# douban/dpark

Hardware: NVIDIA H100
Metric: shuffled rows/sec (reduceByKey end-to-end) (higher is better)
Workload: dtype int64

## Files before the change

### dpark_b200/_native.py

```python
import ctypes as C
import os

import torch

_HERE = os.path.dirname(os.path.abspath(__file__))
LIB_PATH = os.path.join(_HERE, "libdpark_b200.so")

OK, ERR_INVALID, ERR_UNSUPPORTED, ERR_WORKSPACE, ERR_CUDA = 0, -1, -2, -3, -4
K_HASHED = -1
K_I64, K_I32, K_F64, K_U64, K_F32, K_ROWID = 0, 1, 2, 3, 4, 5
V_I64, V_F64, V_I32, V_F32 = 0, 1, 2, 3
OPS = {"sum": 0, "min": 1, "max": 2, "prod": 3, "and": 4, "or": 5, "xor": 6}
BYTES_SIGNED, STR_UTF8 = 0, 1
MAX_PARTITIONS = 4096

_KEY_KIND = {torch.int64: K_I64, torch.int32: K_I32, torch.float64: K_F64, torch.float32: K_F32}
if hasattr(torch, "uint64"):
    _KEY_KIND[torch.uint64] = K_U64
_VAL_KIND = {torch.int64: V_I64, torch.float64: V_F64, torch.int32: V_I32, torch.float32: V_F32}

EXPORTS = [
    "dpk_abi_version", "dpk_last_error", "dpk_device_info", "dpk_hash_keys", "dpk_hash_bytes",
    "dpk_partition_ids", "dpk_partition_workspace_bytes", "dpk_partition_count",
    "dpk_partition_scatter", "dpk_partition", "dpk_combine_workspace_bytes", "dpk_combine",
# ... 99 lines not shown
def _stream():
    return C.c_void_p(torch.cuda.current_stream().cuda_stream)


def _need_cuda(*ts):
    for t in ts:
        if t is not None and not t.is_cuda:
            raise NativeError("dpark_b200 shuffle kernels need CUDA tensors (no CPU fallback); got %s" % t.device)
        if t is not None and not t.is_contiguous():
            raise ValueError("columns must be contiguous")


def key_kind(t, prehashed=False):
    if prehashed:
        if t.dtype != torch.int64:
            raise TypeError("prehashed keys must be int64")
        return K_HASHED
    try:
        return _KEY_KIND[t.dtype]
    except KeyError:
        raise TypeError("%s is unhashable by portable_hash" % t.dtype)


def val_kind(t):
    try:
        return _VAL_KIND[t.dtype]
    except KeyError:
        raise TypeError("unsupported value dtype %s" % t.dtype)


def _thr(thresholds, device):
    if thresholds is None:
        return None, 0
    if not torch.is_tensor(thresholds):
        thresholds = torch.tensor(list(thresholds), dtype=torch.int64, device=device)
    thresholds = thresholds.to(device=device, dtype=torch.int64).contiguous()
    return thresholds, int(thresholds.numel())


def device_info():
    import numpy as np
    info = np.zeros(4, dtype=np.int32)
    _check(lib().dpk_device_info(info.ctypes.data_as(C.c_void_p)))
    return {"sm_count": int(info[0]), "cc": (int(info[1]), int(info[2])), "l2_mb": int(info[3])}


def hash_keys(keys):
    _need_cuda(keys)
    out = torch.empty(keys.numel(), dtype=torch.int64, device=keys.device)
    _check(lib().dpk_hash_keys(_ptr(keys), key_kind(keys), keys.numel(), _ptr(out), _stream()))
    return out


def hash_bytes(data, offsets, mode):
    _need_cuda(data, offsets)
    n = offsets.numel() - 1
    out = torch.empty(n, dtype=torch.int64, device=offsets.device)
    _check(lib().dpk_hash_bytes(_ptr(data), _ptr(offsets), n, mode, _ptr(out), _stream()))
    return out


def hash_tuple(item_hashes):
    _need_cuda(item_hashes)
    arity, n = int(item_hashes.shape[0]), int(item_hashes.shape[1])
    out = torch.empty(n, dtype=torch.int64, device=item_hashes.device)
    _check(lib().dpk_hash_tuple(_ptr(item_hashes), n, arity, _ptr(out), _stream()))
    return out


def partition_ids(hashes, P, thresholds=None):
    _need_cuda(hashes)
    thr, nthr = _thr(thresholds, hashes.device)
    out = torch.empty(hashes.numel(), dtype=torch.int32, device=hashes.device)
    _check(lib().dpk_partition_ids(_ptr(hashes), hashes.numel(), P, _ptr(thr), nthr, _ptr(out), _stream()))
    return out


def partition_workspace(nbuckets, device):
    nbytes = lib().dpk_partition_workspace_bytes(0, nbuckets)
    return torch.empty(nbytes, dtype=torch.uint8, device=device)


K_UNORDERED = 0x100


def _kk(keys, prehashed, row_hash, unordered=False):
    kk = K_ROWID if row_hash is not None else key_kind(keys, prehashed)
    return kk | K_UNORDERED if (unordered and kk >= 0) else kk


def partition_count(keys, P, thresholds=None, prehashed=False, sub_bits=0, ws=None, row_hash=None, unordered=False):
    _need_cuda(keys, row_hash)
    F = P << sub_bits
    thr, nthr = _thr(thresholds, keys.device)
    if ws is None:
        ws = partition_workspace(F, keys.device)
    counts = torch.empty(F, dtype=torch.int64, device=keys.device)
    _check(lib().dpk_partition_count(_ptr(keys), _kk(keys, prehashed, row_hash, unordered), _ptr(row_hash), keys.numel(), P,
                                     _ptr(thr), nthr,
                                     sub_bits, _ptr(counts), _ptr(ws), ws.numel(), _stream()))
    return counts, ws


def partition_scatter(keys, vals, P, bucket_base, out_keys, out_vals, ws, thresholds=None, prehashed=False,
                      sub_bits=0, row_hash=None, unordered=False):
    _need_cuda(keys, vals, bucket_base, out_keys, out_vals, ws, row_hash)
    thr, nthr = _thr(thresholds, keys.device)
    vb = 0 if vals is None else vals.element_size()
    _check(lib().dpk_partition_scatter(_ptr(keys), _kk(keys, prehashed, row_hash, unordered), _ptr(row_hash), _ptr(vals), vb,
                                       keys.numel(), P,
                                       _ptr(thr), nthr, sub_bits, _ptr(bucket_base), _ptr(out_keys),
                                       _ptr(out_vals), _ptr(ws), ws.numel(), _stream()))


def partition_scatter_ptrs(keys, vals, P, key_ptrs, val_ptrs, ws, thresholds=None, prehashed=False, sub_bits=0,
                           row_hash=None, unordered=False):
    _need_cuda(keys, vals, key_ptrs, val_ptrs, ws, row_hash)
    thr, nthr = _thr(thresholds, keys.device)
    vb = 0 if vals is None else vals.element_size()
    _check(lib().dpk_partition_scatter_ptrs(_ptr(keys), _kk(keys, prehashed, row_hash, unordered), _ptr(row_hash), _ptr(vals),
                                            vb, keys.numel(), P, _ptr(thr), nthr, sub_bits, _ptr(key_ptrs),
                                            _ptr(val_ptrs), _ptr(ws), ws.numel(), _stream()))


def copy_segments(src_ptrs, dst_ptrs, nbytes, sms=0):
    _need_cuda(src_ptrs, dst_ptrs, nbytes)
    if not (src_ptrs.numel() == dst_ptrs.numel() == nbytes.numel()):
        raise ValueError("segment table columns differ in length")
    if sms:
        set_option("copy_sms", int(sms))
    try:
        _check(lib().dpk_copy_segments(_ptr(src_ptrs), _ptr(dst_ptrs), _ptr(nbytes), nbytes.numel(), _stream()))
    finally:
        if sms:
            set_option("copy_sms", 0)


def memcpy_batch(dst_ptrs, src_ptrs, nbytes):
    n = len(nbytes)
    if not (len(dst_ptrs) == len(src_ptrs) == n):
        raise ValueError("segment table columns differ in length")
    if n == 0:
        return
    U, I = C.c_uint64 * n, C.c_int64 * n
    _check(lib().dpk_memcpy_batch(U(*dst_ptrs), U(*src_ptrs), I(*nbytes), n, _stream()))


def push_plan(all_counts, nranks, per_block, my_src, my_rank, keys, vals, dst_base, capacity, need_over, want_seg=True,
              part=None, dst_row0=0):
    _need_cuda(all_counts, dst_base, need_over)
    nsrc, F = int(all_counts.shape[0]), int(all_counts.shape[1])
    ncols = 1 if vals is None else 2
    dev = all_counts.device
    lo, hi = (0, per_block) if part is None else part
    src = torch.empty(ncols * nranks, dtype=torch.int64, device=dev)
    dst = torch.empty(ncols * nranks, dtype=torch.int64, device=dev)
    nby = torch.empty(ncols * nranks, dtype=torch.int64, device=dev)
    b0, b1 = min(F, my_rank * per_block + lo), min(F, (my_rank + 1) * per_block, my_rank * per_block + hi)
    seg = torch.empty((nsrc, max(0, b1 - b0)), dtype=torch.int64, device=dev) if want_seg else None
    _check(lib().dpk_push_plan_part(_ptr(all_counts), nsrc, nranks, F, per_block, lo, hi, dst_row0, my_src, my_rank, ncols,
                                    C.c_uint64(keys.data_ptr()), C.c_uint64(0 if vals is None else vals.data_ptr()),
                                    _ptr(dst_base), keys.element_size(), 0 if vals is None else vals.element_size(),
                                    capacity, _ptr(src), _ptr(dst), _ptr(nby), _ptr(need_over), _ptr(seg), _stream()))
    return src, dst, nby, seg


def pipe_plan(all_counts, nranks, per_block, nparts, region_rows, my_src, my_rank, keys, vals, dst_base, need_over,
              want_seg=True):
    _need_cuda(all_counts, dst_base, need_over, keys, vals)
    nsrc, F = int(all_counts.shape[0]), int(all_counts.shape[1])
    ncols = 1 if vals is None else 2
    dev = all_counts.device
    base = torch.empty(F, dtype=torch.int64, device=dev)
    src = torch.empty((nparts, ncols * nranks), dtype=torch.int64, device=dev)
    dst = torch.empty((nparts, ncols * nranks), dtype=torch.int64, device=dev)
    nby = torch.empty((nparts, ncols * nranks), dtype=torch.int64, device=dev)
    seg = torch.empty((nparts, nsrc, per_block // nparts), dtype=torch.int64, device=dev) if want_seg else None
    _check(lib().dpk_pipe_plan(_ptr(all_counts), nsrc, nranks, F, per_block, nparts, region_rows, my_src, my_rank, ncols,
                               C.c_uint64(keys.data_ptr()), C.c_uint64(0 if vals is None else vals.data_ptr()),
                               _ptr(dst_base), keys.element_size(), 0 if vals is None else vals.element_size(),
                               _ptr(base), _ptr(src), _ptr(dst), _ptr(nby), _ptr(need_over), _ptr(seg), _stream()))
    return base, src, dst, nby, seg


def pipe_pad_rows(nranks, nparts, key_bytes, val_bytes=None):
    return nranks * nparts * (16 // min(key_bytes, val_bytes or key_bytes))


def fused_plan(all_counts, nranks, per_block, my_rank, dst_base, key_bytes, val_bytes, capacity, dump_keys, dump_vals,
               need_over, want_seg=True):
    _need_cuda(all_counts, dst_base, need_over, dump_keys, dump_vals)
    G, F = int(all_counts.shape[0]), int(all_counts.shape[1])
    if G != nranks:
        raise ValueError("all_counts has %d source rows for %d ranks" % (G, nranks))
    ncols = 1 if dump_vals is None else 2
    dev = all_counts.device
    kp = torch.empty(F, dtype=torch.int64, device=dev)
    vp_ = torch.empty(F, dtype=torch.int64, device=dev) if ncols == 2 else None
    b0, b1 = min(F, my_rank * per_block), min(F, (my_rank + 1) * per_block)
    seg = torch.empty((G, b1 - b0), dtype=torch.int64, device=dev) if want_seg else None
    _check(lib().dpk_fused_plan(_ptr(all_counts), nranks, F, per_block, my_rank, ncols, _ptr(dst_base), key_bytes,
                                val_bytes if ncols == 2 else 0, capacity, C.c_uint64(dump_keys.data_ptr()),
                                C.c_uint64(0 if dump_vals is None else dump_vals.data_ptr()), _ptr(kp), _ptr(vp_),
                                _ptr(need_over), _ptr(seg), _stream()))
    return kp, vp_, seg


def partition(keys, vals, P, thresholds=None, prehashed=False, sub_bits=0, row_hash=None, unordered=False):
    _need_cuda(keys, vals, row_hash)
    if vals is not None and vals.numel() != keys.numel():
        from .errors import DparkUserFatalError
        raise DparkUserFatalError("ragged pair columns: %d keys, %d values" % (keys.numel(), vals.numel()))
    F = P << sub_bits
    thr, nthr = _thr(thresholds, keys.device)
    ws = partition_workspace(F, keys.device)
    out_keys = torch.empty_like(keys)
    out_vals = None if vals is None else torch.empty_like(vals)
    offsets = torch.empty(F + 1, dtype=torch.int64, device=keys.device)
    vb = 0 if vals is None else vals.element_size()
    _check(lib().dpk_partition(_ptr(keys), _kk(keys, prehashed, row_hash, unordered), _ptr(row_hash), _ptr(vals), vb,
                               keys.numel(), P,
                               _ptr(thr), nthr, sub_bits, _ptr(out_keys), _ptr(out_vals), _ptr(offsets),
                               _ptr(ws), ws.numel(), _stream()))
    return out_keys, out_vals, offsets


def acc_dtype(vals_dtype):
    return torch.float64 if vals_dtype in (torch.float32, torch.float64) else torch.int64


def combine(keys, vals, op, P, seg_rows, part_first=0, nparts=None, thresholds=None, sub_bits=0,
            row_hash=None):
    _need_cuda(keys, vals, seg_rows, row_hash)
    if nparts is None:
        nparts = P
    n = keys.numel()
    F = nparts << sub_bits
    if seg_rows.dim() == 1:
        seg_rows = seg_rows.unsqueeze(0)
    nsrc = int(seg_rows.shape[0])
    if seg_rows.shape[1] != F or seg_rows.dtype != torch.int64:
        raise ValueError("seg_rows must be int64[nsrc, %d]" % F)
    bucket_rows = seg_rows
    thr, nthr = _thr(thresholds, keys.device)
    ws_bytes = lib().dpk_combine_workspace_bytes(n, F, nsrc)
    ws = torch.empty(ws_bytes, dtype=torch.uint8, device=keys.device)
    out_keys = torch.empty_like(keys)
    out_vals = torch.empty(n, dtype=acc_dtype(vals.dtype), device=keys.device)
    out_offsets = torch.empty(nparts + 1, dtype=torch.int64, device=keys.device)
    out_counts = torch.empty(nparts, dtype=torch.int64, device=keys.device)
    kk = key_kind(keys) if row_hash is None else K_ROWID
    _check(lib().dpk_combine(_ptr(keys), kk, _ptr(row_hash), _ptr(vals), val_kind(vals), n, OPS[op], P,
                             _ptr(thr), nthr, sub_bits, part_first, nparts, nsrc, _ptr(bucket_rows), _ptr(out_keys),
                             _ptr(out_vals), _ptr(out_offsets), _ptr(out_counts), _ptr(ws), ws_bytes,
                             _stream()))
    return out_keys, out_vals, out_offsets, out_counts


def dict_encode(data, offsets, hashes):
    _need_cuda(data, offsets, hashes)
    n = offsets.numel() - 1
    ws_bytes = lib().dpk_dict_encode_workspace_bytes(n)
    ws = torch.empty(ws_bytes, dtype=torch.uint8, device=offsets.device)
    rep = torch.empty(n, dtype=torch.int64, device=offsets.device)
    _check(lib().dpk_dict_encode(_ptr(data), _ptr(offsets), _ptr(hashes), n, _ptr(rep), _ptr(ws), ws_bytes,
                                 _stream()))
    return rep


def tokenize(data):
    _need_cuda(data)
    n = int(data.numel())
    dev = data.device
    if n == 0:
        z = torch.zeros(0, dtype=torch.int64, device=dev)
        return z, z.clone(), True
    nb = int(lib().dpk_tokenize_blocks(n))
    counts = torch.empty(nb + 1, dtype=torch.int64, device=dev)
    counts[nb] = 0
    _check(lib().dpk_tokenize_count(_ptr(data), n, _ptr(counts), C.c_void_p(counts.data_ptr() + 8 * nb), _stream()))
    incl = torch.cumsum(counts[:nb], 0)
    total, flag = int(incl[-1].item()), int(counts[nb].item())
    if flag & 1:
        return None, None, False
    base = (incl - counts[:nb]).contiguous()
    starts = torch.empty(total, dtype=torch.int64, device=dev)
    lens = torch.empty(total, dtype=torch.int64, device=dev)
    if total:
        _check(lib().dpk_tokenize_emit(_ptr(data), n, _ptr(base), _ptr(starts), _ptr(lens), _stream()))
    return starts, lens, True


def gather_bytes(data, starts, lens, idx=None):
    _need_cuda(data, starts, lens, idx)
    sel = lens if idx is None else lens[idx]
    m = int(sel.numel())
    off = torch.zeros(m + 1, dtype=torch.int64, device=data.device)
    if m:
        torch.cumsum(sel, 0, out=off[1:])
    out = torch.empty(int(off[-1].item()) if m else 0, dtype=torch.uint8, device=data.device)
    if m and out.numel():
        _check(lib().dpk_gather_bytes(_ptr(data), _ptr(starts), _ptr(lens), _ptr(idx), m, _ptr(off), _ptr(out), _stream()))
    return out, off


def key_or(keys):
    _need_cuda(keys)
    out = torch.empty(1, dtype=torch.int64, device=keys.device)
    _check(lib().dpk_key_or(_ptr(keys), keys.numel(), _ptr(out), _stream()))
    return out


def gather_i64(src, idx):
    _need_cuda(src, idx)
    out = torch.empty(idx.numel(), dtype=torch.int64, device=idx.device)
    _check(lib().dpk_gather_i64(_ptr(src), _ptr(idx), idx.numel(), _ptr(out), _stream()))
    return out


def radix_pass(keys, vals, shift, bits, out_keys=None, out_vals=None, ws=None):
    _need_cuda(keys, vals)
    if keys.dtype != torch.int64:
        raise TypeError("radix_pass sorts int64 key bits")
    if out_keys is None:
        out_keys = torch.empty_like(keys)
    if out_vals is None and vals is not None:
        out_vals = torch.empty_like(vals)
    if ws is None:
        ws = partition_workspace(1 << bits, keys.device)
    vb = 0 if vals is None else vals.element_size()
    _check(lib().dpk_radix_pass(_ptr(keys), _ptr(vals), vb, keys.numel(), shift, bits, _ptr(out_keys),
                                _ptr(out_vals), _ptr(ws), ws.numel(), _stream()))
    return out_keys, out_vals


# ... 96 lines not shown
```

### dpark_b200/csrc/dpk_aggregate2.cuh

```cuda
#pragma once

constexpr int AG2_THREADS = 256;
constexpr int AG2_WARPS = AG2_THREADS / 32;
constexpr int AG2_TAGS = 4096;
constexpr int AG2_CAP = 2048;
constexpr int AG2_ITEMS = AG2_CAP / AG2_THREADS;
constexpr int AG2_GEN_ITEMS = 4;
constexpr uint32_t AG2_IDX_MASK = 0xfffu;
constexpr int AG2_MINW = 256;
constexpr int AG2_MAX_M = 1 << 16;
constexpr int AG2_STACK = 40;

struct Ag2Shared {
    int fb, sp, overflow, nres;
    unsigned long long excl;
    int next_fb[2];
    long long next_r0[2], next_r1[2];
    int wcnt[AG2_ITEMS * AG2_WARPS];
    int total;
    int stack_m[AG2_STACK], stack_r[AG2_STACK];
};

__device__ __forceinline__ uint32_t sm_ld_u32(uint32_t a) {
    uint32_t v;
// ... 74 lines not shown
    unsigned mine = 0;
    const int lane = threadIdx.x & 31;
    const unsigned lt = (1u << lane) - 1u;
    offs[0] = offs[1] = 0;
    int lc = 0;
#pragma unroll
    for (int g = 0; g < NI; g += 4) {
        long long k[4];
        uint32_t h[4], t[4];
        bool claimed[4];
#pragma unroll
        for (int u = 0; u < 4; u++) {
            const int idx = (g + u) * AG2_THREADS + (int)threadIdx.x;
            k[u] = idx < n ? sm_ld_s64(key_base + (uint32_t)idx * 8u) : 0ll;
        }
        uint32_t fpb[4];
#pragma unroll
        for (int u = 0; u < 4; u++) {
            const uint32_t hs = slot_hash32((uint64_t)k[u]);
            h[u] = hs & (AG2_TAGS - 1);
            fpb[u] = hs & ~(uint32_t)AG2_IDX_MASK;
        }
#pragma unroll
        for (int u = 0; u < 4; u++) {
            const int idx = (g + u) * AG2_THREADS + (int)threadIdx.x;
            t[u] = idx < n ? sm_ld_u32(tag_base + h[u] * 4u) : 0xffffffffu;
        }
#pragma unroll
        for (int u = 0; u < 4; u++) {
            const int idx = (g + u) * AG2_THREADS + (int)threadIdx.x;
            claimed[u] = false;
            if (t[u] == 0u) {
                t[u] = sm_cas_u32(tag_base + h[u] * 4u, 0u, fpb[u] | ((uint32_t)idx + 1u));
                claimed[u] = t[u] == 0u;
            }
        }
#pragma unroll
        for (int u = 0; u < 4; u++) {
            const int idx = (g + u) * AG2_THREADS + (int)threadIdx.x;
            if (idx < n && !claimed[u]) {
                uint32_t hh = h[u], tt = t[u];
                for (;;) {
                    if (tt == 0u) {
                        tt = sm_cas_u32(tag_base + hh * 4u, 0u, fpb[u] | ((uint32_t)idx + 1u));
                        if (tt == 0u) { claimed[u] = true; break; }
                    }
                    if ((tt & ~(uint32_t)AG2_IDX_MASK) == fpb[u]) {
                        const uint32_t o = (tt & AG2_IDX_MASK) - 1u;
                        if (sm_ld_s64(key_base + o * 8u) == k[u]) {
                            const long long mv = sm_ld_s64(acc_base + (uint32_t)idx * 8u);
                            if constexpr (std::is_same<AccT, double>::value)
                                sm_apply<double>(op, acc_base + o * 8u, s_acc + o, __longlong_as_double(mv));
                            else
                                sm_apply<int64_t>(op, acc_base + o * 8u, s_acc + o, (int64_t)mv);
                            break;
                        }
                    }
                    hh = (hh + 1u) & (AG2_TAGS - 1);
                    tt = sm_ld_u32(tag_base + hh * 4u);
                }
            }
        }
#pragma unroll
        for (int u = 0; u < 4; u++) {
            const int j = g + u;
            const unsigned cmj = __ballot_sync(0xffffffffu, claimed[u]);
            if (lane == j) lc = __popc(cmj);
            offs[j >> 2] |= (uint32_t)__popc(cmj & lt) << (8 * (j & 3));
            if (claimed[u]) mine |= 1u << j;
        }
    }
    *lane_cnt = lc;
    return mine;
}

__device__ __forceinline__ int ag2_off(const uint32_t (&offs)[2], int j) { return (int)((offs[j >> 2] >> (8 * (j & 3))) & 0xffu); }
__device__ __forceinline__ uint32_t ag2_slot(const uint32_t (&slots)[3], int j) {
    const int bit = 12 * j;
    uint32_t v = slots[bit >> 5] >> (bit & 31);
    if ((bit & 31) > 20) v |= slots[(bit >> 5) + 1] << (32 - (bit & 31));
    return v & 0xfffu;
}

template <typename KeyT, typename ValT, typename AccT, int MINB, bool CURSOR, bool BATCHED, bool FAST_ONLY = false>
__global__ void __launch_bounds__(AG2_THREADS, MINB)
k_smem_aggregate2(const KeyT *__restrict__ keys, const ValT *__restrict__ vals, int op,
                  const int64_t *__restrict__ fine_off, int32_t nfine, int32_t fine_per_part,
                  const int64_t *__restrict__ part_offsets, KeyT *__restrict__ out_keys,
                  int64_t *__restrict__ out_vals, long long *__restrict__ out_counts,
                  unsigned long long *__restrict__ fb_state, int *__restrict__ work_counter,
                  int *__restrict__ part_err, const int *__restrict__ bucket_list, const int *__restrict__ bucket_count,
                  long long *__restrict__ phase_cycles, int *__restrict__ big_list = nullptr, int *__restrict__ big_count = nullptr) {
    long long tstamp = 0;
    auto stamp = [&](int k) {
        if (phase_cycles != nullptr && threadIdx.x == 0) {
            const long long now = clock64();
            if (k >= 0) atomicAdd(reinterpret_cast<unsigned long long *>(&phase_cycles[k]), (unsigned long long)(now - tstamp));
            tstamp = now;
        }
    };
    const int nwork = bucket_list ? *bucket_count : nfine;
    auto bucket_of_ticket = [&](int t) { return bucket_list ? bucket_list[t] : t; };
    extern __shared__ __align__(16) long long s_dyn2[];
    uint32_t *s_tag = reinterpret_cast<uint32_t *>(s_dyn2);
    long long *s_key = s_dyn2 + AG2_TAGS / 2;
    long long *s_acc = s_key + AG2_CAP;
    const uint32_t tag_base = (uint32_t)__cvta_generic_to_shared(s_tag);
    const uint32_t key_base = (uint32_t)__cvta_generic_to_shared(s_key);
    const uint32_t acc_base = (uint32_t)__cvta_generic_to_shared(s_acc);
    __shared__ Ag2Shared sh;
    const int lane = threadIdx.x & 31, warp = threadIdx.x >> 5;
    auto clear_tags = [&]() {
        uint4 *t4 = reinterpret_cast<uint4 *>(s_tag);
#pragma unroll
        for (int i = 0; i < AG2_TAGS / 4 / AG2_THREADS; i++) t4[i * AG2_THREADS + threadIdx.x] = make_uint4(0, 0, 0, 0);
    };
    auto stage = [&](int64_t g0, int w, int at, auto ni_tag, auto between) {
        constexpr int NI = decltype(ni_tag)::value;
        KeyT kr[NI];
        ValT vr[NI];
#pragma unroll
        for (int j = 0; j < NI; j++) {
            const int i = j * AG2_THREADS + (int)threadIdx.x;
            if (i < w) { kr[j] = keys[g0 + i]; vr[j] = vals[g0 + i]; }
        }
        between();
#pragma unroll
        for (int j = 0; j < NI; j++) {
            const int i = j * AG2_THREADS + (int)threadIdx.x;
            if (i < w) {
                s_key[at + i] = key_bits<KeyT>(kr[j]);
                if constexpr (std::is_same<AccT, double>::value) s_acc[at + i] = __double_as_longlong((double)vr[j]);
                else s_acc[at + i] = (long long)vr[j];
            }
        }
    };
    auto nothing = []() {};
    auto scan_claims = [&]() {
        constexpr int N = AG2_ITEMS * AG2_WARPS;
        int a = sh.wcnt[lane], b = sh.wcnt[lane + 32];
        int ia = a, ib = b;
#pragma unroll
        for (int d = 1; d < 32; d <<= 1) {
            int ta = __shfl_up_sync(0xffffffffu, ia, d), tb = __shfl_up_sync(0xffffffffu, ib, d);
            if (lane >= d) { ia += ta; ib += tb; }
        }
        const int suma = __shfl_sync(0xffffffffu, ia, 31);
        sh.wcnt[lane] = ia - a;
        sh.wcnt[lane + 32] = suma + ib - b;
        if (lane == 31) sh.total = suma + ib;
        static_assert(N == 64, "scan_claims handles 64 counters");
    };

    clear_tags();
    if (threadIdx.x == 0) {
        const int t = atomicAdd(work_counter, 1);
        sh.next_fb[0] = t < nwork ? bucket_of_ticket(t) : nfine;
        if (t < nwork) { const int b = bucket_of_ticket(t); sh.next_r0[0] = fine_off[b]; sh.next_r1[0] = fine_off[b + 1]; }
    }
    for (int it = 0;; it++) {
        __syncthreads();
        stamp(it ? 4 : -1);
        const int fb = sh.next_fb[it & 1];
        if (fb >= nfine) break;
        const int64_t r0 = sh.next_r0[it & 1], r1 = sh.next_r1[it & 1];
        const int p = fb / fine_per_part;
        const int first_fb = p * fine_per_part;
        const bool last_fb = fb == first_fb + fine_per_part - 1;
        const int64_t pbase = part_offsets[p];
        uint32_t offs[2], slots[3];
        int lane_cnt;
        int nt = 0;
        long long nr0 = 0, nr1 = 0;
        auto prefetch_ticket = [&]() {
            if (CURSOR && threadIdx.x == 0) nt = atomicAdd(work_counter, 1);
        };
        auto prefetch_range = [&]() {
            if (CURSOR && threadIdx.x == 0) {
                const int b = nt < nwork ? bucket_of_ticket(nt) : nfine;
                sh.next_fb[(it + 1) & 1] = b;
                if (b < nfine) { nr0 = fine_off[b]; nr1 = fine_off[b + 1]; }
            }
        };
        auto publish_range = [&]() {
            if (threadIdx.x == 0) {
                if (!CURSOR) {
                    nt = atomicAdd(work_counter, 1);
                    sh.next_fb[(it + 1) & 1] = nt;
                    if (nt < nfine) { nr0 = fine_off[nt]; nr1 = fine_off[nt + 1]; }
                }
                sh.next_r0[(it + 1) & 1] = nr0;
                sh.next_r1[(it + 1) & 1] = nr1;
            }
        };

        if (r1 - r0 <= AG2_CAP) {
            const int n = (int)(r1 - r0);
            stage(r0, n, 0, std::integral_constant<int, AG2_ITEMS>(), prefetch_ticket);
            prefetch_range();
            __syncthreads();
            stamp(0);
            const unsigned mine = BATCHED ? ag2_insert_batched<AccT, AG2_ITEMS>(n, op, tag_base, key_base, acc_base, s_acc, offs, &lane_cnt)
                                          : ag2_insert<AccT, false, AG2_ITEMS>(0, n, 1, 0, op, tag_base, key_base, acc_base, s_acc, offs, &lane_cnt, slots);
            if (lane < AG2_ITEMS) sh.wcnt[lane * AG2_WARPS + warp] = lane_cnt;
            if (CURSOR) publish_range();
            __syncthreads();
            stamp(1);
// ... 148 lines not shown
```

### dpark_b200/csrc/dpk_combine.cu

```cuda
#include "dpk_common.cuh"
#include <cooperative_groups.h>
#include <type_traits>

namespace cg = cooperative_groups;

namespace dpk {

constexpr int CB_THREADS = 256;
constexpr int64_t kEmpty = INT64_MIN;

struct __align__(16) Slot {
    int64_t key;
    int64_t acc;
};

template <typename KeyT> __device__ __forceinline__ int64_t key_bits(KeyT k);
template <> __device__ __forceinline__ int64_t key_bits<int64_t>(int64_t k) { return k; }
template <> __device__ __forceinline__ int64_t key_bits<int32_t>(int32_t k) { return (int64_t)k; }
template <> __device__ __forceinline__ int64_t key_bits<uint64_t>(uint64_t k) { return (int64_t)k; }
template <> __device__ __forceinline__ int64_t key_bits<double>(double k) {
    if (k == 0.0) k = 0.0;
    return __double_as_longlong(k);
}
template <> __device__ __forceinline__ int64_t key_bits<float>(float k) {
// ... 79 lines not shown

__global__ void __launch_bounds__(CB_THREADS)
k_tbl_plan(const int64_t *__restrict__ seg_rows, int32_t nsrc, int32_t F, int32_t sub_bits, int32_t nparts,
           int64_t *__restrict__ tbl_off, int64_t *__restrict__ part_off, int64_t *__restrict__ seg_start) {
    __shared__ long long s_slots[CB_THREADS], s_rows[CB_THREADS], s_carry;
    const int E = (F + CB_THREADS - 1) / CB_THREADS;
    const int b0 = threadIdx.x * E, b1 = min(b0 + E, F);
    long long slots = 0, rows = 0;
    for (int b = b0; b < b1; b++) {
        long long r = 0;
        for (int s = 0; s < nsrc; s++) r += seg_rows[(int64_t)s * F + b];
        slots += ((r + (r >> 1) + 32 + 7) >> 3) << 3;
        rows += r;
    }
    s_slots[threadIdx.x] = slots;
    s_rows[threadIdx.x] = rows;
    __syncthreads();
    long long sbase = 0, rbase = 0;
    for (int t = 0; t < (int)threadIdx.x; t++) { sbase += s_slots[t]; rbase += s_rows[t]; }
    const int S = 1 << sub_bits;
    for (int b = b0; b < b1; b++) {
        long long r = 0;
        for (int s = 0; s < nsrc; s++) r += seg_rows[(int64_t)s * F + b];
        tbl_off[b] = sbase;
        if ((b & (S - 1)) == 0) part_off[b >> sub_bits] = rbase;
        sbase += ((r + (r >> 1) + 32 + 7) >> 3) << 3;
        rbase += r;
    }
    if (b0 < F && b1 == F) { tbl_off[F] = sbase; part_off[nparts] = rbase; }
    if (F == 0 && threadIdx.x == 0) { tbl_off[0] = 0; part_off[0] = 0; }
    if (threadIdx.x == 0) s_carry = 0;
    __syncthreads();
    for (int s = 0; s < nsrc; s++) {
        long long mine = 0;
        for (int b = b0; b < b1; b++) mine += seg_rows[(int64_t)s * F + b];
        s_rows[threadIdx.x] = mine;
        __syncthreads();
        long long base = s_carry;
        for (int t = 0; t < (int)threadIdx.x; t++) base += s_rows[t];
        for (int b = b0; b < b1; b++) {
            seg_start[(int64_t)s * F + b] = base;
            base += seg_rows[(int64_t)s * F + b];
        }
        __syncthreads();
        if (threadIdx.x == CB_THREADS - 1) s_carry = base;
        __syncthreads();
    }
}

__device__ __forceinline__ int4 slot_fill(int64_t ident) {
    return make_int4((int)(uint32_t)((uint64_t)kEmpty & 0xffffffffu), (int)(uint32_t)((uint64_t)kEmpty >> 32),
                     (int)(uint32_t)((uint64_t)ident & 0xffffffffu), (int)(uint32_t)((uint64_t)ident >> 32));
}

__device__ __forceinline__ Slot *probe_slot(Slot *region, uint32_t size, int64_t kb) {
    uint32_t h = (uint32_t)(((mix64((uint64_t)kb) & 0xffffffffull) * (uint64_t)size) >> 32);
    for (;;) {
        int64_t cur = __ldcg(&region[h].key);
        if (cur == kb) break;
        if (cur == kEmpty) {
            unsigned long long prev = atomicCAS((unsigned long long *)&region[h].key, (unsigned long long)kEmpty,
                                                (unsigned long long)kb);
            if (prev == (unsigned long long)kEmpty || prev == (unsigned long long)kb) break;
        }
        h = h + 1 == size ? 0 : h + 1;
    }
    return &region[h];
}

__global__ void __launch_bounds__(CB_THREADS)
k_tbl_init(Slot *__restrict__ table, const int64_t *__restrict__ tbl_total, int64_t ident) {
    const int64_t slots = *tbl_total;
    int64_t i = (int64_t)blockIdx.x * blockDim.x + threadIdx.x;
    int64_t stride = (int64_t)gridDim.x * blockDim.x;
    const int4 fill = slot_fill(ident);
    for (; i < slots; i += stride) reinterpret_cast<int4 *>(table)[i] = fill;
}

template <typename KeyT, typename ValT, typename AccT>
__global__ void __launch_bounds__(CB_THREADS)
k_tbl_insert(const KeyT *__restrict__ keys, const int64_t *__restrict__ aux, const ValT *__restrict__ vals,
             int64_t n, const int64_t *__restrict__ rows_total, int op, PartFn f, int32_t bucket_first, int32_t F,
             const int64_t *__restrict__ tbl_off, Slot *__restrict__ table, Slot *__restrict__ side,
             int32_t *__restrict__ side_used) {
    int64_t i = (int64_t)blockIdx.x * blockDim.x + threadIdx.x;
    int64_t stride = (int64_t)gridDim.x * blockDim.x;
    const int64_t rows = min(n, *rows_total);
    for (; i < rows; i += stride) {
        const KeyT key = keys[i];
        const int64_t kb = key_bits<KeyT>(key);
        const AccT v = (AccT)vals[i];
        Slot *s;
        if (kb == kEmpty) {
            s = side;
            *side_used = 1;
        } else {
            int b = f.bucket(hash_of<KeyT>(key, aux)) - bucket_first;
            b = min(max(b, 0), F - 1);
            const int64_t base = __ldg(&tbl_off[b]);
            s = probe_slot(table + base, (uint32_t)(__ldg(&tbl_off[b + 1]) - base), kb);
        }
        Acc<AccT>::apply(op, &s->acc, v);
    }
}

template <typename KeyT>
__global__ void __launch_bounds__(CB_THREADS)
k_tbl_compact(const Slot *__restrict__ table, const int64_t *__restrict__ tbl_total,
              const int64_t *__restrict__ aux, PartFn f, int32_t part_first, int32_t nparts,
              const int64_t *__restrict__ part_offsets, KeyT *__restrict__ out_keys,
              int64_t *__restrict__ out_vals, unsigned long long *__restrict__ out_counts) {
    extern __shared__ __align__(16) int32_t s_mem[];
    int32_t *s_cnt = s_mem;
    long long *s_base = reinterpret_cast<long long *>(s_mem + ((nparts + 1) & ~1));
    const int lane = threadIdx.x & 31;
    constexpr int ITEMS = 4;
    const int64_t total = *tbl_total;
    const int64_t tile = (int64_t)CB_THREADS * ITEMS;
    for (int64_t t0 = (int64_t)blockIdx.x * tile; t0 < total; t0 += (int64_t)gridDim.x * tile) {
        for (int p = threadIdx.x; p < nparts; p += CB_THREADS) s_cnt[p] = 0;
        __syncthreads();
        int64_t kb[ITEMS], acc[ITEMS];
        int lp[ITEMS], rk[ITEMS];
#pragma unroll
        for (int j = 0; j < ITEMS; j++) {
            int64_t i = t0 + (int64_t)j * CB_THREADS + threadIdx.x;
            lp[j] = -1;
            if (i < total) {
                int4 raw = __ldcs(reinterpret_cast<const int4 *>(table) + i);
                kb[j] = (int64_t)(((uint64_t)(uint32_t)raw.y << 32) | (uint32_t)raw.x);
                acc[j] = (int64_t)(((uint64_t)(uint32_t)raw.w << 32) | (uint32_t)raw.z);
                if (kb[j] != kEmpty) lp[j] = f(hash_of<KeyT>(key_from_bits<KeyT>(kb[j]), aux)) - part_first;
            }
        }
#pragma unroll
        for (int j = 0; j < ITEMS; j++) {
            unsigned m = __match_any_sync(0xffffffffu, lp[j]);
            int base = 0;
            const bool ok = lp[j] >= 0 && lp[j] < nparts;
            if (ok && lane == __ffs(m) - 1) base = atomicAdd(&s_cnt[lp[j]], __popc(m));
            base = __shfl_sync(0xffffffffu, base, __ffs(m) - 1);
            rk[j] = base + __popc(m & ((1u << lane) - 1u));
        }
        __syncthreads();
        for (int p = threadIdx.x; p < nparts; p += CB_THREADS) {
            int c = s_cnt[p];
            s_base[p] = c ? (long long)atomicAdd(&out_counts[p], (unsigned long long)c) : 0;
        }
        __syncthreads();
#pragma unroll
        for (int j = 0; j < ITEMS; j++) {
            if (lp[j] >= 0 && lp[j] < nparts) {
                int64_t dst = part_offsets[lp[j]] + s_base[lp[j]] + rk[j];
                out_keys[dst] = key_from_bits<KeyT>(kb[j]);
                out_vals[dst] = acc[j];
            }
        }
        __syncthreads();
    }
}

constexpr int BR_THREADS = 1024;
constexpr int BR_CLUSTER = 8;

template <typename KeyT, typename ValT, typename AccT>
__global__ void __cluster_dims__(BR_CLUSTER, 1, 1) __launch_bounds__(BR_THREADS, 1)
k_bucket_reduce(const KeyT *__restrict__ keys, const int64_t *__restrict__ aux, const ValT *__restrict__ vals,
                int op, int64_t ident, int32_t sub_bits, int32_t F, int32_t nsrc,
                const int64_t *__restrict__ seg_start, const int64_t *__restrict__ seg_rows,
                const int64_t *__restrict__ tbl_off, Slot *__restrict__ table, Slot *__restrict__ side,
                int32_t *__restrict__ side_used, const int64_t *__restrict__ part_offsets,
                KeyT *__restrict__ out_keys, int64_t *__restrict__ out_vals,
                unsigned long long *__restrict__ out_counts, int *__restrict__ bucket_counter) {
    cg::cluster_group cluster = cg::this_cluster();
    const unsigned crank = cluster.block_rank();
    __shared__ int s_bucket;
    __shared__ int s_wsum[BR_THREADS / 32];
    __shared__ long long s_base;
    const int lane = threadIdx.x & 31, warp = threadIdx.x >> 5;
    const int64_t tid_c = (int64_t)crank * BR_THREADS + threadIdx.x;
    const int64_t nth_c = (int64_t)BR_CLUSTER * BR_THREADS;
    const int4 fill = slot_fill(ident);
    for (;;) {
        if (crank == 0 && threadIdx.x == 0) s_bucket = atomicAdd(bucket_counter, 1);
        cluster.sync();
        const int b = *cluster.map_shared_rank(&s_bucket, 0);
        cluster.sync();
        if (b >= F) break;
        const int64_t base = tbl_off[b];
        const uint32_t size = (uint32_t)(tbl_off[b + 1] - base);
        Slot *region = table + base;
        for (int64_t i = tid_c; i < size; i += nth_c) reinterpret_cast<int4 *>(region)[i] = fill;
        cluster.sync();
        for (int s = 0; s < nsrc; s++) {
            const int64_t r0 = seg_start[(int64_t)s * F + b];
            const int64_t rn = seg_rows[(int64_t)s * F + b];
            for (int64_t i = tid_c; i < rn; i += nth_c) {
                const int64_t kb = key_bits<KeyT>(keys[r0 + i]);
                const AccT v = (AccT)vals[r0 + i];
                Slot *sl;
                if (kb == kEmpty) {
                    sl = side;
                    *side_used = 1;
                } else {
                    sl = probe_slot(region, size, kb);
                }
                Acc<AccT>::apply(op, &sl->acc, v);
            }
        }
        cluster.sync();
        const int p = b >> sub_bits;
        const int64_t pbase = part_offsets[p];
        constexpr int ITEMS = 4;
        const int64_t tile = (int64_t)BR_THREADS * ITEMS;
        for (int64_t t0 = (int64_t)crank * tile; t0 < size; t0 += (int64_t)BR_CLUSTER * tile) {
            int64_t kb[ITEMS], acc[ITEMS];
            int c = 0;
#pragma unroll
            for (int j = 0; j < ITEMS; j++) {
                const int64_t i = t0 + (int64_t)threadIdx.x * ITEMS + j;
                kb[j] = kEmpty;
                if (i < size) {
                    int4 raw = __ldcg(reinterpret_cast<const int4 *>(region) + i);
                    kb[j] = (int64_t)(((uint64_t)(uint32_t)raw.y << 32) | (uint32_t)raw.x);
                    acc[j] = (int64_t)(((uint64_t)(uint32_t)raw.w << 32) | (uint32_t)raw.z);
                }
                c += kb[j] != kEmpty;
            }
            int inc = c;
#pragma unroll
            for (int d = 1; d < 32; d <<= 1) {
                int t = __shfl_up_sync(0xffffffffu, inc, d);
                if (lane >= d) inc += t;
            }
            if (lane == 31) s_wsum[warp] = inc;
            __syncthreads();
            if (warp == 0) {
                int w = s_wsum[lane];
                int winc = w;
#pragma unroll
                for (int d = 1; d < 32; d <<= 1) {
                    int t = __shfl_up_sync(0xffffffffu, winc, d);
                    if (lane >= d) winc += t;
                }
                s_wsum[lane] = winc - w;
                if (lane == 31) s_base = winc ? (long long)atomicAdd(&out_counts[p], (unsigned long long)winc) : 0;
            }
            __syncthreads();
            int64_t dst = pbase + s_base + s_wsum[warp] + (inc - c);
#pragma unroll
            for (int j = 0; j < ITEMS; j++) {
                if (kb[j] != kEmpty) {
                    out_keys[dst] = key_from_bits<KeyT>(kb[j]);
                    out_vals[dst] = acc[j];
                    dst++;
                }
            }
            __syncthreads();
        }
    }
}

#include "dpk_aggregate.cuh"
#include "dpk_aggregate2.cuh"
#include "dpk_aggregate3.cuh"

template <typename KeyT>
__global__ void k_side_flush(const Slot *__restrict__ side, const int32_t *__restrict__ side_used,
                             const int64_t *__restrict__ aux, PartFn f, int32_t part_first, int32_t nparts,
                             const int64_t *__restrict__ part_offsets, KeyT *__restrict__ out_keys,
                             int64_t *__restrict__ out_vals, unsigned long long *__restrict__ out_counts) {
    if (threadIdx.x != 0 || blockIdx.x != 0 || *side_used == 0) return;
    const KeyT key = key_from_bits<KeyT>(kEmpty);
    const int p = f(hash_of<KeyT>(key, aux)) - part_first;
    if (p < 0 || p >= nparts) return;
    const int64_t dst = part_offsets[p] + (int64_t)atomicAdd(&out_counts[p], 1ull);
    out_keys[dst] = key;
    out_vals[dst] = side->acc;
}

static inline int64_t max_slots_for(int64_t n, int32_t F) { return n + (n >> 1) + (int64_t)F * 40 + 64; }

static inline int grid_cap(int64_t items, int per_cta, int waves) {
    int64_t g = (items + per_cta - 1) / per_cta;
    int64_t cap = (int64_t)sm_count() * waves;
    if (g > cap) g = cap;
    if (g < 1) g = 1;
    return (int)g;
}

int g_reduce_impl = 2;

int g_agg_wide = 1;
int g_agg_ctas = 4;
int g_agg_timing = 0;
int g_agg_split = 1;
int g_agg_cursor = 1;
int g_agg_pipe = 0;
int g_agg_batched = 0;
int g_agg_impl = 1;
int g_agg_target_rows = 2048;

struct Ctx {
    int key_kind, val_bytes;
    int64_t *fine_off;
    unsigned long long *fb_state;
    int *part_err;
    void *seg_ws;
    int64_t seg_ws_bytes;
    const void *keys, *vals;
    const int64_t *aux;
    int64_t n;
    int op;
    PartFn f;
    int32_t part_first, nparts, F, nsrc;
    const int64_t *seg_rows, *seg_start, *tbl_off, *part_off;
    Slot *table, *side;
    int64_t max_slots;
    int32_t *side_used;
    int *bucket_counter;
    void *out_keys;
    int64_t *out_vals;
    unsigned long long *out_counts;
    cudaStream_t st;
};

template <typename KeyT, typename ValT, typename AccT>
static int dispatch_op(const Ctx &c) {
    if (!Acc<AccT>::supports(c.op)) return fail(DPK_ERR_UNSUPPORTED, "op %d unsupported for this value kind", c.op);
    const int64_t ident = Acc<AccT>::identity(c.op);
    if (g_reduce_impl == 2) {
        const int sb2 = choose_sb2(c.n, c.F, g_agg_target_rows);
        const int32_t S2 = 1 << sb2;
        PartFn fine = fine_partfn(c.f, sb2);
        fine.row_hash = c.aux;
        KeyT *rekeys = (KeyT *)c.table;
        ValT *revals = (ValT *)((char *)c.table + (size_t)c.n * 8);
        int rc = seg_multisplit(c.keys, c.key_kind, c.vals, (int32_t)sizeof(ValT), c.n, fine, c.F, c.nsrc, c.seg_start,
                                c.seg_rows, rekeys, revals, c.fine_off, c.seg_ws, c.seg_ws_bytes, c.st);
        if (rc) return rc;
        const int32_t nfine = c.F * S2;
        int grid = sm_count() * 8;
        if (grid > nfine) grid = nfine;
        auto agg = g_agg_wide ? k_smem_aggregate<KeyT, ValT, AccT, true> : k_smem_aggregate<KeyT, ValT, AccT, false>;
        const int agg_smem = AG_CAP * 16 + AG_CAP * 2;
        DPK_CUDA_TRY(cudaFuncSetAttribute(agg, cudaFuncAttributeMaxDynamicSharedMemorySize, agg_smem));
        DPK_CUDA_TRY(cudaMemsetAsync(c.fb_state, 0, (size_t)nfine * 8, c.st));
        if (g_agg_impl == 1) {
            auto agg2 = k_smem_aggregate2<KeyT, ValT, AccT, 3, true, true>;
            if (g_agg_cursor && g_agg_batched) agg2 = g_agg_ctas == 4 ? k_smem_aggregate2<KeyT, ValT, AccT, 4, true, true> : k_smem_aggregate2<KeyT, ValT, AccT, 3, true, true>;
            else if (g_agg_cursor) agg2 = g_agg_ctas == 4 ? k_smem_aggregate2<KeyT, ValT, AccT, 4, true, false> : k_smem_aggregate2<KeyT, ValT, AccT, 3, true, false>;
            else agg2 = k_smem_aggregate2<KeyT, ValT, AccT, 3, false, false>;
            const int smem2 = AG2_TAGS * 4 + AG2_CAP * 16;
            DPK_CUDA_TRY(cudaFuncSetAttribute(agg2, cudaFuncAttributeMaxDynamicSharedMemorySize, smem2));
            DPK_CUDA_TRY(cudaMemsetAsync(c.part_err, 0, (size_t)(c.nparts + 2) * 4, c.st));
            long long *timing = nullptr;
            if (g_agg_timing) {
                static long long *d_timing = nullptr;
                if (!d_timing) DPK_CUDA_TRY(cudaMalloc(&d_timing, 64));
                DPK_CUDA_TRY(cudaMemsetAsync(d_timing, 0, 64, c.st));
                timing = d_timing;
            }
            if (g_agg_pipe && g_agg_cursor) {
                auto agg3 = g_agg_pipe == 2 ? k_smem_aggregate3<KeyT, ValT, AccT, 2, false>
                          : (g_agg_batched ? k_smem_aggregate3<KeyT, ValT, AccT, 3, true> : k_smem_aggregate3<KeyT, ValT, AccT, 3, false>);
                const int smem3 = AG2_TAGS * 4 + AG2_CAP * 8;
                DPK_CUDA_TRY(cudaFuncSetAttribute(agg3, cudaFuncAttributeMaxDynamicSharedMemorySize, smem3));
                int *big_count = c.part_err + c.nparts, *list_counter = c.part_err + c.nparts + 1;
                int *big_list = reinterpret_cast<int *>(c.fb_state);
                int g3 = sm_count() * (g_agg_pipe == 2 ? 2 : 3);
                if (g3 > nfine) g3 = nfine;
                DPK_LAUNCH("smem_aggregate", c.st, agg3<<<g3, AG2_THREADS, smem3, c.st>>>(
                    rekeys, revals, c.op, ident, c.fine_off, nfine, (1 << c.f.sub_bits) * S2, c.part_off,
                    (KeyT *)c.out_keys, c.out_vals, (long long *)c.out_counts, c.bucket_counter, big_list, big_count));
                auto aggb = k_smem_aggregate2<KeyT, ValT, AccT, 3, true, false>;
                DPK_CUDA_TRY(cudaFuncSetAttribute(aggb, cudaFuncAttributeMaxDynamicSharedMemorySize, smem2));
                DPK_LAUNCH("smem_aggregate_big", c.st, aggb<<<sm_count(), AG2_THREADS, smem2, c.st>>>(
                    rekeys, revals, c.op, c.fine_off, nfine, (1 << c.f.sub_bits) * S2, c.part_off,
                    (KeyT *)c.out_keys, c.out_vals, (long long *)c.out_counts, c.fb_state, list_counter, c.part_err,
                    big_list, big_count, nullptr, nullptr, nullptr));
            } else if (g_agg_cursor && !g_agg_batched && g_agg_split) {
                auto fast = g_agg_ctas == 4 ? k_smem_aggregate2<KeyT, ValT, AccT, 4, true, false, true>
                                            : k_smem_aggregate2<KeyT, ValT, AccT, 3, true, false, true>;
                DPK_CUDA_TRY(cudaFuncSetAttribute(fast, cudaFuncAttributeMaxDynamicSharedMemorySize, smem2));
                int *big_count = c.part_err + c.nparts, *list_counter = c.part_err + c.nparts + 1;
                int *big_list = reinterpret_cast<int *>(c.fb_state);
                DPK_LAUNCH("smem_aggregate", c.st, fast<<<grid, AG2_THREADS, smem2, c.st>>>(
                    rekeys, revals, c.op, c.fine_off, nfine, (1 << c.f.sub_bits) * S2, c.part_off,
                    (KeyT *)c.out_keys, c.out_vals, (long long *)c.out_counts, c.fb_state, c.bucket_counter, c.part_err,
                    nullptr, nullptr, timing, big_list, big_count));
                auto aggb = k_smem_aggregate2<KeyT, ValT, AccT, 3, true, false>;
                DPK_CUDA_TRY(cudaFuncSetAttribute(aggb, cudaFuncAttributeMaxDynamicSharedMemorySize, smem2));
                DPK_LAUNCH("smem_aggregate_big", c.st, aggb<<<sm_count() * 2, AG2_THREADS, smem2, c.st>>>(
                    rekeys, revals, c.op, c.fine_off, nfine, (1 << c.f.sub_bits) * S2, c.part_off,
                    (KeyT *)c.out_keys, c.out_vals, (long long *)c.out_counts, c.fb_state, list_counter, c.part_err,
                    big_list, big_count, nullptr, nullptr, nullptr));
            } else {
            DPK_LAUNCH("smem_aggregate", c.st, agg2<<<grid, AG2_THREADS, smem2, c.st>>>(
                rekeys, revals, c.op, c.fine_off, nfine, (1 << c.f.sub_bits) * S2, c.part_off,
                (KeyT *)c.out_keys, c.out_vals, (long long *)c.out_counts, c.fb_state, c.bucket_counter, c.part_err,
                nullptr, nullptr, timing, nullptr, nullptr));
            if (timing) {
                long long h[8];
                DPK_CUDA_TRY(cudaMemcpyAsync(h, timing, sizeof(h), cudaMemcpyDeviceToHost, c.st));
                DPK_CUDA_TRY(cudaStreamSynchronize(c.st));
                const double nb = h[5] ? (double)h[5] : 1.0;
                fprintf(stderr, "agg_timing: %lld buckets; cycles per bucket: load+stage %.0f | insert %.0f | reserve %.0f | write-out %.0f | "
                        "to next top %.0f | total %.0f\n", h[5], h[0] / nb, h[1] / nb, h[2] / nb, h[3] / nb, h[4] / nb,
                        (h[0] + h[1] + h[2] + h[3] + h[4]) / nb);
            }
            }
            if (g_agg_cursor)
                DPK_LAUNCH("agg_finalize", c.st, k_agg_finalize<<<1, 256, 0, c.st>>>(c.part_err, (long long *)c.out_counts, c.nparts));
            return DPK_OK;
        }
        DPK_LAUNCH("smem_aggregate", c.st, agg<<<grid, AG_THREADS, agg_smem, c.st>>>(
            rekeys, revals, c.op, ident, c.fine_off, nfine, (1 << c.f.sub_bits) * S2, c.part_off,
            (KeyT *)c.out_keys, c.out_vals, c.out_counts, c.fb_state, c.bucket_counter));
        return DPK_OK;
    }
    if (g_reduce_impl == 1) {
        auto kern = k_bucket_reduce<KeyT, ValT, AccT>;
        int nclusters = sm_count() / BR_CLUSTER;
        if (nclusters > c.F) nclusters = c.F;
        if (nclusters < 1) nclusters = 1;
        DPK_LAUNCH("bucket_reduce", c.st, kern<<<nclusters * BR_CLUSTER, BR_THREADS, 0, c.st>>>(
            (const KeyT *)c.keys, c.aux, (const ValT *)c.vals, c.op, ident, c.f.sub_bits, c.F, c.nsrc,
            c.seg_start, c.seg_rows, c.tbl_off, c.table, c.side, c.side_used, c.part_off, (KeyT *)c.out_keys,
            c.out_vals, c.out_counts, c.bucket_counter));
    } else {
        DPK_LAUNCH("tbl_init", c.st, k_tbl_init<<<grid_cap(c.max_slots, CB_THREADS, 16), CB_THREADS, 0, c.st>>>(
            c.table, c.tbl_off + c.F, ident));
        if (c.n > 0) {
            DPK_LAUNCH("tbl_insert", c.st, k_tbl_insert<KeyT, ValT, AccT><<<grid_cap(c.n, CB_THREADS, 16), CB_THREADS, 0, c.st>>>(
                (const KeyT *)c.keys, c.aux, (const ValT *)c.vals, c.n, c.part_off + c.nparts, c.op, c.f,
                c.part_first << c.f.sub_bits,
                c.F, c.tbl_off, c.table, c.side, c.side_used));
        }
        size_t sh = (size_t)((c.nparts + 1) & ~1) * 4 + (size_t)c.nparts * 8;
        DPK_LAUNCH("tbl_compact", c.st, k_tbl_compact<KeyT><<<grid_cap(c.max_slots, CB_THREADS * 4, 8), CB_THREADS, sh, c.st>>>(
            c.table, c.tbl_off + c.F, c.aux, c.f, c.part_first, c.nparts, c.part_off, (KeyT *)c.out_keys,
            c.out_vals, c.out_counts));
    }
    DPK_LAUNCH("side_flush", c.st, k_side_flush<KeyT><<<1, 32, 0, c.st>>>(
        c.side, c.side_used, c.aux, c.f, c.part_first, c.nparts, c.part_off, (KeyT *)c.out_keys, c.out_vals,
        c.out_counts));
    return DPK_OK;
}

template <typename KeyT>
static int dispatch_valkind(int val_kind, const Ctx &c) {
    switch (val_kind) {
    case DPK_V_I64: return dispatch_op<KeyT, int64_t, int64_t>(c);
    case DPK_V_I32: return dispatch_op<KeyT, int32_t, int64_t>(c);
    case DPK_V_F64: return dispatch_op<KeyT, double, double>(c);
    case DPK_V_F32: return dispatch_op<KeyT, float, double>(c);
    }
    return fail(DPK_ERR_UNSUPPORTED, "value kind %d unsupported", val_kind);
}

template <typename KeyT>
static int run_combine(Ctx &c, int val_kind, int64_t *out_offsets, void *ws) {
    c.table = (Slot *)ws;
    c.side = c.table + c.max_slots;
    c.side_used = (int32_t *)(c.side + 1);
    c.bucket_counter = (int *)(c.side_used + 2);
    int64_t *tbl_off = (int64_t *)(c.side_used + 4);
    int64_t *seg_start = tbl_off + c.F + 2;
    c.tbl_off = tbl_off;
    c.seg_start = seg_start;
    c.part_off = out_offsets;
    c.fine_off = seg_start + (int64_t)c.nsrc * c.F + 2;
    const int sb2 = choose_sb2(c.n, c.F, g_agg_target_rows);
    c.fb_state = (unsigned long long *)(c.fine_off + ((int64_t)c.F << sb2) + 2);
    c.part_err = (int *)(c.fb_state + ((int64_t)c.F << sb2) + 2);
    c.seg_ws = (void *)(((uintptr_t)(c.part_err + c.F + 2) + 255) & ~(uintptr_t)255);
    c.seg_ws_bytes = seg_multisplit_ws_bytes(c.n, c.F, 1 << sb2, c.nsrc);
    DPK_CUDA_TRY(cudaMemsetAsync(c.side_used, 0, 16, c.st));
    DPK_CUDA_TRY(cudaMemsetAsync(c.out_counts, 0, (size_t)c.nparts * 8, c.st));
    DPK_LAUNCH("tbl_plan", c.st, k_tbl_plan<<<1, CB_THREADS, 0, c.st>>>(c.seg_rows, c.nsrc, c.F, c.f.sub_bits, c.nparts,
                                                                       tbl_off, out_offsets, seg_start));
    return dispatch_valkind<KeyT>(val_kind, c);
}

__global__ void k_side_init(Slot *side, int64_t ident) {
    if (threadIdx.x == 0 && blockIdx.x == 0) { side->key = kEmpty; side->acc = ident; }
}

}

using namespace dpk;

extern "C" {

int dpk_set_option(const char *name, int64_t value) {
    if (!name) return fail(DPK_ERR_INVALID, "name is NULL");
    if (strcmp(name, "reduce_impl") == 0) {
        if (value < 0 || value > 2) return fail(DPK_ERR_INVALID, "reduce_impl must be 0, 1 or 2");
        g_reduce_impl = (int)value;
        return DPK_OK;
    }
    if (strcmp(name, "agg_impl") == 0) {
        if (value != 0 && value != 1) return fail(DPK_ERR_INVALID, "agg_impl must be 0 or 1");
        g_agg_impl = (int)value;
        return DPK_OK;
    }
    if (strcmp(name, "agg_batched") == 0) {
        if (value != 0 && value != 1) return fail(DPK_ERR_INVALID, "agg_batched must be 0 or 1");
        g_agg_batched = (int)value;
        return DPK_OK;
    }
    if (strcmp(name, "agg_split") == 0) {
        g_agg_split = value != 0;
        return DPK_OK;
    }
    if (strcmp(name, "agg_timing") == 0) {
        g_agg_timing = value != 0;
        return DPK_OK;
    }
    if (strcmp(name, "agg_pipe") == 0) {
// ... 12 lines not shown
        return DPK_OK;
    }
    if (strcmp(name, "agg_wide") == 0) {
        if (value != 0 && value != 1) return fail(DPK_ERR_INVALID, "agg_wide must be 0 or 1");
        g_agg_wide = (int)value;
        return DPK_OK;
    }
    if (strcmp(name, "scatter_items") == 0) {
        if (value != 8 && value != 16) return fail(DPK_ERR_INVALID, "scatter_items must be 8 or 16");
        g_scatter_items = (int)value;
        return DPK_OK;
    }
    if (strcmp(name, "scatter_threads") == 0) {
        if (value != 256 && value != 512 && value != 1024) return fail(DPK_ERR_INVALID, "scatter_threads must be 256, 512 or 1024");
        g_scatter_threads = (int)value;
        return DPK_OK;
    }
    if (strcmp(name, "scatter_seg_wide") == 0) {
        g_scatter_seg_wide = value != 0;
        return DPK_OK;
    }
    if (strcmp(name, "scatter_wide_from") == 0) {
        if (value < 0 || value > DPK_MAX_PARTITIONS) return fail(DPK_ERR_INVALID, "scatter_wide_from out of range");
        g_scatter_wide_from = (int)value;
        return DPK_OK;
    }
    if (strcmp(name, "copy_tma") == 0) {
        if (value != 0 && value != 1) return fail(DPK_ERR_INVALID, "copy_tma must be 0 or 1");
        g_copy_tma = (int)value;
        return DPK_OK;
    }
    if (strcmp(name, "copy_sms") == 0) {
        if (value < 0 || value > 1024) return fail(DPK_ERR_INVALID, "copy_sms out of range");
        g_copy_sms = (int)value;
        return DPK_OK;
    }
    if (strcmp(name, "scatter_ptr_bulk") == 0) {
        if (value != 0 && value != 1) return fail(DPK_ERR_INVALID, "scatter_ptr_bulk must be 0 or 1");
        g_scatter_ptr_bulk = (int)value;
        return DPK_OK;
    }
    if (strcmp(name, "scatter_ptr_threads") == 0) {
        if (value != 512 && value != 1024) return fail(DPK_ERR_INVALID, "scatter_ptr_threads must be 512 or 1024");
        g_scatter_ptr_threads = (int)value;
        return DPK_OK;
    }
    if (strcmp(name, "scatter_bulk") == 0) {
        if (value != 0 && value != 1) return fail(DPK_ERR_INVALID, "scatter_bulk must be 0 or 1");
        g_scatter_bulk = (int)value;
        return DPK_OK;
    }
    if (strcmp(name, "count_mode") == 0) {
        if (value != 0 && value != 1) return fail(DPK_ERR_INVALID, "count_mode must be 0 or 1");
        g_count_mode = (int)value;
        return DPK_OK;
    }
    if (strcmp(name, "agg_target_rows") == 0) {
        if (value < 64 || value > AG_LIMIT) return fail(DPK_ERR_INVALID, "agg_target_rows must be in [64, %d]", AG_LIMIT);
        g_agg_target_rows = (int)value;
        return DPK_OK;
    }
    return fail(DPK_ERR_INVALID, "unknown option %s", name);
}

int64_t dpk_combine_workspace_bytes(int64_t n, int32_t nbuckets, int32_t nsrc) {
    if (n < 0) n = 0;
    if (nbuckets < 1) nbuckets = 1;
    if (nsrc < 1) nsrc = 1;
    return (max_slots_for(n, nbuckets) + 2) * (int64_t)sizeof(Slot) +
           ((int64_t)nbuckets + 4 + (int64_t)nbuckets * nsrc) * 8 + 64 +
           (((int64_t)nbuckets << choose_sb2(n, nbuckets, g_agg_target_rows)) + 4) * 16 + 512 + ((int64_t)nbuckets + 2) * 4 +
           seg_multisplit_ws_bytes(n, nbuckets, 1 << choose_sb2(n, nbuckets, g_agg_target_rows), nsrc);
}

int dpk_combine(const void *keys, int key_kind, const int64_t *key_aux, const void *vals, int val_kind, int64_t n,
                int op, int32_t P, const int64_t *thresholds, int32_t nthr, int32_t sub_bits, int32_t part_first,
                int32_t nparts, int32_t nsrc, const int64_t *seg_rows, void *out_keys, void *out_vals,
                int64_t *out_offsets, int64_t *out_counts, void *ws, int64_t ws_bytes, dpk_stream_t stream) {
    if (n < 0 || n >= ((int64_t)1 << 31)) return fail(DPK_ERR_INVALID, "n=%lld out of range [0, 2^31)", (long long)n);
    if (nparts < 1 || part_first < 0 || part_first + nparts > P)
        return fail(DPK_ERR_INVALID, "bad partition range first=%d n=%d P=%d", part_first, nparts, P);
    if (nsrc < 1) return fail(DPK_ERR_INVALID, "nsrc must be >= 1");
    if (!seg_rows || !out_counts || !out_offsets || !ws) return fail(DPK_ERR_INVALID, "NULL pointer");
    if (n > 0 && (!keys || !vals || !out_keys || !out_vals)) return fail(DPK_ERR_INVALID, "NULL pointer");
    Ctx c;
    int rc = make_partfn(P, thresholds, nthr, sub_bits, &c.f);
    if (rc) return rc;
    c.F = nparts << sub_bits;
    if (c.F > DPK_MAX_PARTITIONS)
        return fail(DPK_ERR_UNSUPPORTED, "%d local buckets exceed %d", c.F, DPK_MAX_PARTITIONS);
    if (ws_bytes < dpk_combine_workspace_bytes(n, c.F, nsrc))
        return fail(DPK_ERR_WORKSPACE, "workspace needs %lld B, got %lld", (long long)dpk_combine_workspace_bytes(n, c.F, nsrc), (long long)ws_bytes);
    c.keys = keys; c.vals = vals; c.n = n; c.op = op; c.aux = key_aux; c.key_kind = key_kind; c.val_bytes = 0;
    if (key_kind == DPK_K_ROWID && n > 0 && !key_aux) return fail(DPK_ERR_INVALID, "DPK_K_ROWID needs key_aux (the per-row hash column)");
    c.part_first = part_first; c.nparts = nparts; c.nsrc = nsrc; c.seg_rows = seg_rows;
    c.max_slots = max_slots_for(n, c.F);
    c.out_keys = out_keys; c.out_vals = (int64_t *)out_vals; c.out_counts = (unsigned long long *)out_counts;
    c.st = (cudaStream_t)stream;
    {
        int64_t ident = (val_kind == DPK_V_F64 || val_kind == DPK_V_F32) ? Acc<double>::identity(op) : Acc<int64_t>::identity(op);
        Slot *side = (Slot *)ws + c.max_slots;
        DPK_LAUNCH("side_init", c.st, k_side_init<<<1, 32, 0, c.st>>>(side, ident));
    }
    switch (key_kind) {
    case DPK_K_I64: return run_combine<int64_t>(c, val_kind, out_offsets, ws);
    case DPK_K_I32: return run_combine<int32_t>(c, val_kind, out_offsets, ws);
    case DPK_K_F64: return run_combine<double>(c, val_kind, out_offsets, ws);
    case DPK_K_U64: return run_combine<uint64_t>(c, val_kind, out_offsets, ws);
    case DPK_K_F32: return run_combine<float>(c, val_kind, out_offsets, ws);
    case DPK_K_ROWID: return run_combine<RowId>(c, val_kind, out_offsets, ws);
    }
    return fail(DPK_ERR_UNSUPPORTED, "key kind %d is unhashable by portable_hash", key_kind);
}

}
```

### dpark_b200/csrc/dpk_common.cuh

```cuda
#pragma once
#include <cuda_runtime.h>
#include <stdint.h>
#include <stdio.h>
#include <stdarg.h>
#include <string.h>
#include <math.h>

#include "dpark_b200.h"

#define DPK_HD __host__ __device__ __forceinline__

namespace dpk {

extern thread_local char g_err[512];
int fail(int code, const char *fmt, ...);
#define DPK_CUDA_TRY(expr)                                                        \
    do {                                                                          \
        cudaError_t _e = (expr);                                                  \
        if (_e != cudaSuccess)                                                    \
            return dpk::fail(DPK_ERR_CUDA, "%s failed: %s (%s:%d)", #expr,        \
                             cudaGetErrorString(_e), __FILE__, __LINE__);         \
    } while (0)
#define DPK_LAUNCH_CHECK() DPK_CUDA_TRY(cudaGetLastError())

// ... 84 lines not shown
        if (c < 0x80) { cp = c; extra = 0; }
        else if (c < 0xE0) { cp = c & 0x1F; extra = 1; }
        else if (c < 0xF0) { cp = c & 0x0F; extra = 2; }
        else { cp = c & 0x07; extra = 3; }
        for (int j = 1; j <= extra && i + j < nbytes; j++) cp = (cp << 6) | (s[i + j] & 0x3F);
        i += extra + 1;
        if (ncp == 0) value = (uint64_t)cp << 7;
        value = (1000003ull * value) ^ (uint64_t)cp;
        ncp++;
    }
    value ^= (uint64_t)ncp;
    return (int64_t)value == -1 ? -2 : (int64_t)value;
}

DPK_HD int64_t hash_tuple_items(const int64_t *item_hash, int64_t stride, int64_t i, int32_t arity) {
    uint64_t mul = 1000003ull, value = 0x345678ull;
    int64_t l = arity;
    for (int32_t a = 0; a < arity; a++) {
        l -= 1;
        value = (value ^ (uint64_t)item_hash[(int64_t)a * stride + i]) * mul;
        mul += (uint64_t)(82520 + l * 2);
    }
    value += 97531ull;
    return (int64_t)value == -1 ? -2 : (int64_t)value;
}

struct PartFn {
    int32_t P;
    int32_t mode;
    uint64_t magic;
    int32_t shift;
    int32_t nthr;
    const int64_t *thresholds;
    int32_t sub_bits;
    const int64_t *row_hash;

    DPK_HD int32_t nbuckets() const { return P << sub_bits; }
    DPK_HD int32_t bucket(int64_t h) const {
        if (mode == 4) return (int32_t)(((uint64_t)h >> shift) & (uint64_t)(P - 1));
        if (mode == 5) return P == 1 ? 0 : (int32_t)((mixed(h) >> shift) & (uint32_t)(P - 1));
        int32_t p = (*this)(h);
        if (sub_bits == 0) return p;
        return (p << sub_bits) | (int32_t)(mixed(h) >> (32 - sub_bits));
    }
    static DPK_HD uint32_t mixed(int64_t h) {
        uint32_t x = (uint32_t)(uint64_t)h * 0x9E3779B1u + (uint32_t)((uint64_t)h >> 32) * 0x85EBCA77u;
        x ^= x >> 16; x *= 0x21F0AAADu;
        x ^= x >> 15; x *= 0x735A2D97u;
        x ^= x >> 15;
        return x;
    }

    DPK_HD int32_t operator()(int64_t h) const {
        if (mode == 1) return (int32_t)((uint64_t)h & (uint64_t)(P - 1));
        if (mode == 2) {
            uint64_t a = h < 0 ? 0ull - (uint64_t)h : (uint64_t)h;
#ifdef __CUDA_ARCH__
            uint64_t q = __umul64hi(magic, a);
#else
            uint64_t q = (uint64_t)(((unsigned __int128)magic * a) >> 64);
#endif
            uint64_t t = ((a - q) >> 1) + q;
            q = t >> shift;
            uint32_t r = (uint32_t)(a - q * (uint64_t)P);
            return h < 0 ? (r ? P - (int32_t)r : 0) : (int32_t)r;
        }
        if (mode == 3) {
            int32_t lo = 0, hi = nthr;
            while (lo < hi) {
                int32_t mid = (lo + hi) >> 1;
                if (h < thresholds[mid]) hi = mid; else lo = mid + 1;
            }
            return lo;
        }
        return 0;
    }
};
int make_partfn(int32_t P, const int64_t *thresholds, int32_t nthr, int32_t sub_bits, PartFn *out);

int64_t seg_multisplit_ws_bytes(int64_t n, int32_t F1, int32_t S2, int32_t nsrc);
int seg_multisplit(const void *keys, int key_kind, const void *vals, int32_t val_bytes, int64_t n,
                   const PartFn &fine, int32_t F1, int32_t nsrc, const int64_t *seg_start,
                   const int64_t *seg_rows, void *out_keys, void *out_vals, int64_t *fine_off, void *ws,
                   int64_t ws_bytes, cudaStream_t st, bool stable = false);

DPK_HD uint64_t mix64(uint64_t x) {
    x ^= x >> 33; x *= 0xff51afd7ed558ccdull; x ^= x >> 33; x *= 0xc4ceb9fe1a85ec53ull;
    return x ^ (x >> 33);
}
DPK_HD uint32_t slot_hash32(uint64_t kb) {
    uint32_t x = (uint32_t)kb * 0xCC9E2D51u + (uint32_t)(kb >> 32) * 0x1B873593u + 0x7F4A7C15u;
    x ^= x >> 16; x *= 0x85EBCA6Bu;
    x ^= x >> 13; x *= 0xC2B2AE35u;
    x ^= x >> 16;
    return x;
}

constexpr int AG_MAX_SB2 = 10;
DPK_HD int choose_sb2(int64_t n, int32_t F, int target_rows) {
    int sb2 = 0;
    while (sb2 < AG_MAX_SB2 && n / ((int64_t)F << sb2) > target_rows) sb2++;
    return sb2;
}
DPK_HD PartFn fine_partfn(const PartFn &first, int sb2) {
    PartFn fine = first;
    fine.mode = 5; fine.P = 1 << sb2; fine.shift = 32 - first.sub_bits - sb2; fine.sub_bits = 0;
    return fine;
}

DPK_HD int64_t join_left_rows(const int64_t *run, int64_t len, int64_t nL) {
    int64_t lo = 0, hi = len;
    while (lo < hi) {
        const int64_t mid = (lo + hi) >> 1;
        if (run[mid] < nL) lo = mid + 1; else hi = mid;
    }
    return lo;
}
DPK_HD int64_t join_side(int64_t n, bool keep_other) { return n > 0 ? n : (keep_other ? 1 : 0); }
DPK_HD int64_t join_count(int64_t nl, int64_t nr, bool keep_left, bool keep_right) {
    return join_side(nl, keep_right) * join_side(nr, keep_left);
}
DPK_HD void join_pair(int64_t i, int64_t nr, bool keep_left, int64_t *a, int64_t *b) {
    const int64_t R = join_side(nr, keep_left);
    *a = i / R;
    *b = i - *a * R;
}
DPK_HD int64_t group_of(const int64_t *off, int64_t lo, int64_t hi, int64_t i) {
    while (hi - lo > 1) {
        const int64_t mid = (lo + hi) >> 1;
        if (off[mid] <= i) lo = mid; else hi = mid;
    }
    return lo;
}

DPK_HD void cogroup_split(const int64_t *ids, int64_t s, int64_t len, const int64_t *bounds, int32_t ninputs,
                          int64_t *first, int64_t *count, int64_t stride) {
    int64_t lo = join_left_rows(ids + s, len, bounds[0]);
    for (int32_t t = 0; t < ninputs; t++) {
        const int64_t hi = join_left_rows(ids + s, len, bounds[t + 1]);
        first[t * stride] = s + lo;
        count[t * stride] = hi - lo;
        lo = hi;
    }
}
DPK_HD int64_t cogroup_source(const int64_t *ids, int64_t first, int64_t base, int64_t r, int64_t id_base) {
    return ids[first + r - base] - id_base;
}

constexpr int TK_BYTES = 16;
__host__ __device__ __forceinline__ bool tok_ws(uint8_t c) { return c == 0x20 || (c >= 0x09 && c <= 0x0d) || (c >= 0x1c && c <= 0x1f); }

__host__ __device__ __forceinline__ uint32_t tok_starts16(const uint8_t *__restrict__ data, int64_t n, int64_t i0, bool *hi) {
    uint8_t c[TK_BYTES];
    if (i0 + TK_BYTES <= n && (((uintptr_t)(data + i0)) & 15u) == 0) {
        const uint4 q = *reinterpret_cast<const uint4 *>(data + i0);
        const uint32_t w[4] = {q.x, q.y, q.z, q.w};
#pragma unroll
        for (int j = 0; j < TK_BYTES; j++) c[j] = (uint8_t)(w[j >> 2] >> ((j & 3) * 8));
    } else {
#pragma unroll
        for (int j = 0; j < TK_BYTES; j++) c[j] = i0 + j < n ? data[i0 + j] : (uint8_t)0x20;
    }
    bool prev_ws = i0 == 0 ? true : tok_ws(data[i0 - 1]);
    uint32_t m = 0;
    bool h = false;
#pragma unroll
    for (int j = 0; j < TK_BYTES; j++) {
// ... 12 lines not shown
```

### dpark_b200/csrc/dpk_partition.cu

```cuda
#include "dpk_common.cuh"

namespace dpk {

constexpr int PT_THREADS = 256;
constexpr int PT_WARPS = PT_THREADS / 32;
constexpr int PT_ITEMS = 16;
constexpr int PT_TILE = PT_THREADS * PT_ITEMS;
constexpr int PT_COUNT_PRIV = 1024;

struct NoVal {};

int g_count_mode = 1;
int g_scatter_items = 16;
int g_scatter_bulk = 1;
int g_scatter_threads = 512;
int g_scatter_seg_wide = 1;
int g_scatter_wide_from = 512;
int g_scatter_ptr_bulk = 1;
int g_scatter_ptr_threads = 1024;

struct SegTab {
    const int64_t *cbeg, *cend;
    const int32_t *ctotal;
    int32_t *chunk_counts;
    const int64_t *chunk_off;
    const uint64_t *key_ptrs, *val_ptrs;
    int unordered;
};

struct Plan {
    int32_t T;
    int64_t L;
    SegTab seg;
    const char *label_count = nullptr, *label_scatter = nullptr;
};

static Plan make_plan(int64_t n) {
    Plan pl;
    pl.seg = SegTab{nullptr, nullptr, nullptr, nullptr, nullptr, nullptr, nullptr, 0};
    int64_t tiles = (n + PT_TILE - 1) / PT_TILE;
    if (tiles < 1) tiles = 1;
    int64_t maxT = (int64_t)sm_count() * 8;
    pl.T = (int32_t)(tiles < maxT ? tiles : maxT);
    pl.L = tiles;
    return pl;
}

static inline int64_t align_up(int64_t x, int64_t a) { return (x + a - 1) / a * a; }

static int64_t ws_counts_bytes(int32_t P) { return align_up((int64_t)P * sm_count() * 8 * 4, 256); }
static int64_t ws_total_bytes(int32_t P) {
    return ws_counts_bytes(P) + align_up((int64_t)P * 8, 256) + align_up((int64_t)(P + 1) * 8, 256);
}

template <typename KeyT, int PRE>
__device__ __forceinline__ int64_t key_hash(KeyT k, const PartFn &f) {
    if constexpr (PRE == 1) return (int64_t)k;
    else if constexpr (PRE == 2) return __ldg(&f.row_hash[(int64_t)k]);
    else return KeyHash<KeyT>::of(k);
}

__device__ __forceinline__ unsigned warp_peers(int id, int nbits) {
    unsigned peers = 0xffffffffu;
#pragma unroll
    for (int b = 0; b < 13; b++) {
        if (b < nbits) {
            const unsigned set = __ballot_sync(0xffffffffu, (id >> b) & 1);
            peers &= ((id >> b) & 1) ? set : ~set;
        }
    }
    return peers;
}

template <int NW = PT_WARPS>
__device__ __forceinline__ int block_excl_scan(int v, int *s_warp, int *total) {
    const int lane = threadIdx.x & 31, warp = threadIdx.x >> 5;
    int inc = v;
#pragma unroll
    for (int d = 1; d < 32; d <<= 1) {
        int t = __shfl_up_sync(0xffffffffu, inc, d);
        if (lane >= d) inc += t;
    }
    if (lane == 31) s_warp[warp] = inc;
    __syncthreads();
    int base = 0, tot = 0;
#pragma unroll
    for (int w = 0; w < NW; w++) {
        int t = s_warp[w];
        if (w < warp) base += t;
        tot += t;
    }
    __syncthreads();
    *total = tot;
    return base + inc - v;
}

template <typename KeyT, int PRE>
__global__ void __launch_bounds__(PT_THREADS)
k_part_count(const KeyT *__restrict__ keys, int64_t n, int64_t L, PartFn f,
             int32_t *__restrict__ tile_counts, int32_t T, SegTab seg, int count_mode) {
    extern __shared__ int32_t s_cnt[];
    const int P = f.nbuckets();
    if (seg.cbeg != nullptr && (int)blockIdx.x >= *seg.ctotal) return;
    const bool priv = P <= PT_COUNT_PRIV;
    const int nhist = priv ? PT_WARPS * P : P;
    for (int p = threadIdx.x; p < nhist; p += PT_THREADS) s_cnt[p] = 0;
    __syncthreads();
    const int64_t beg = seg.cbeg ? seg.cbeg[blockIdx.x] : ((int64_t)blockIdx.x * L / T) * PT_TILE;
    const int64_t end = seg.cbeg ? seg.cend[blockIdx.x] : min(n, ((int64_t)(blockIdx.x + 1) * L / T) * PT_TILE);
    const int lane = threadIdx.x & 31;
    int32_t *wh = s_cnt + (priv ? (threadIdx.x >> 5) * P : 0);
    constexpr int U = 8;
    int64_t i0 = beg;
    if (count_mode == 1) {
        for (; i0 + (int64_t)PT_THREADS * U <= end; i0 += (int64_t)PT_THREADS * U) {
            KeyT k[U];
#pragma unroll
            for (int u = 0; u < U; u++) k[u] = keys[i0 + (int64_t)u * PT_THREADS + threadIdx.x];
#pragma unroll
            for (int u = 0; u < U; u++) atomicAdd(&wh[f.bucket(key_hash<KeyT, PRE>(k[u], f))], 1);
        }
    }
    for (; i0 < end; i0 += (int64_t)PT_THREADS * U) {
        KeyT k[U];
        bool ok[U];
#pragma unroll
        for (int u = 0; u < U; u++) {
            int64_t i = i0 + (int64_t)u * PT_THREADS + threadIdx.x;
            ok[u] = i < end;
            k[u] = ok[u] ? keys[i] : KeyT(0);
        }
#pragma unroll
        for (int u = 0; u < U; u++) {
            int pid = ok[u] ? f.bucket(key_hash<KeyT, PRE>(k[u], f)) : -1;
            if (count_mode == 1) {
                if (ok[u]) atomicAdd(&wh[pid], 1);
                continue;
            }
            unsigned m = warp_peers(pid, 32 - __clz(P));
            if (priv) {
                if (ok[u] && lane == __ffs(m) - 1) wh[pid] += __popc(m);
                __syncwarp();
            } else {
                if (ok[u] && lane == __ffs(m) - 1) atomicAdd(&s_cnt[pid], __popc(m));
            }
        }
    }
    __syncthreads();
    if (priv) {
        for (int p = threadIdx.x; p < P; p += PT_THREADS) {
            int t = 0;
#pragma unroll
            for (int w = 0; w < PT_WARPS; w++) t += s_cnt[w * P + p];
            s_cnt[p] = t;
        }
        __syncthreads();
    }
    if (seg.cbeg) {
        for (int p = threadIdx.x; p < P; p += PT_THREADS) seg.chunk_counts[(int64_t)blockIdx.x * P + p] = s_cnt[p];
    } else {
        for (int p = threadIdx.x; p < P; p += PT_THREADS) tile_counts[(int64_t)p * T + blockIdx.x] = s_cnt[p];
    }
}

__global__ void __launch_bounds__(PT_THREADS)
k_part_scan(int32_t *__restrict__ tile_counts, int32_t T, int64_t *__restrict__ totals) {
    __shared__ int s_warp[PT_WARPS];
    int32_t *row = tile_counts + (int64_t)blockIdx.x * T;
    const int E = (T + PT_THREADS - 1) / PT_THREADS;
    const int b = threadIdx.x * E;
    int sum = 0;
    for (int i = b; i < min(b + E, T); i++) sum += row[i];
    int tot;
    int run = block_excl_scan(sum, s_warp, &tot);
    for (int i = b; i < min(b + E, T); i++) {
        int t = row[i];
        row[i] = run;
        run += t;
    }
    if (threadIdx.x == 0) totals[blockIdx.x] = (int64_t)tot;
}

__global__ void __launch_bounds__(PT_THREADS)
k_part_offsets(const int64_t *__restrict__ totals, int32_t P, int64_t *__restrict__ offsets) {
    __shared__ long long s_part[PT_THREADS];
    const int E = (P + PT_THREADS - 1) / PT_THREADS;
    const int b = threadIdx.x * E;
    long long sum = 0;
    for (int i = b; i < min(b + E, P); i++) sum += totals[i];
    s_part[threadIdx.x] = sum;
    __syncthreads();
    long long base = 0;
    for (int t = 0; t < (int)threadIdx.x; t++) base += s_part[t];
    for (int i = b; i < min(b + E, P); i++) {
        offsets[i] = base;
        base += totals[i];
    }
    if (b < P && min(b + E, P) == P) offsets[P] = base;
    if (P == 0 && threadIdx.x == 0) offsets[0] = 0;
}

struct ScatterSmem {
    int64_t key_off, val_off, pid_off, gpos_off, tstart_off, tcount_off, whist_off, kptr_off, vptr_off, total;
};
static ScatterSmem scatter_smem(int kb, int vb, int32_t P, bool ptr_mode, int tile) {
    ScatterSmem s;
    int64_t o = 0;
    s.key_off = o; o += align_up((int64_t)tile * kb, 16);
    s.val_off = o; o += align_up((int64_t)tile * vb, 16);
    s.gpos_off = o; o += align_up((int64_t)P * 8, 16);
    s.tstart_off = o; o += align_up((int64_t)P * 4, 16);
    s.tcount_off = o; o += align_up((int64_t)P * 4, 16);
    s.pid_off = o; o += align_up((int64_t)tile * 2, 16);
    s.whist_off = o; o += align_up((int64_t)PT_WARPS * P * 2, 16);
    s.kptr_off = o; if (ptr_mode) o += align_up((int64_t)P * 8, 16);
    s.vptr_off = o; if (ptr_mode) o += align_up((int64_t)P * 8, 16);
    s.total = o;
    return s;
}

template <typename KeyT, typename ValT, int PRE, int ITEMS>
__global__ void __launch_bounds__(PT_THREADS, ITEMS == 16 ? 2 : 4)
k_part_scatter(const KeyT *__restrict__ keys, const ValT *__restrict__ vals, int64_t n, int64_t L,
               PartFn f, const int32_t *__restrict__ tile_off, int32_t T,
               const int64_t *__restrict__ bucket_base, KeyT *__restrict__ out_keys,
               ValT *__restrict__ out_vals, ScatterSmem lay, SegTab seg) {
    constexpr bool HAS_VAL = !std::is_same<ValT, NoVal>::value;
    constexpr int TILE = PT_THREADS * ITEMS;
    extern __shared__ __align__(16) unsigned char smem[];
    __shared__ int s_warp[PT_WARPS];
    KeyT *s_key = reinterpret_cast<KeyT *>(smem + lay.key_off);
    ValT *s_val = reinterpret_cast<ValT *>(smem + lay.val_off);
    int64_t *s_gpos = reinterpret_cast<int64_t *>(smem + lay.gpos_off);
    int32_t *s_tstart = reinterpret_cast<int32_t *>(smem + lay.tstart_off);
    int32_t *s_tcount = reinterpret_cast<int32_t *>(smem + lay.tcount_off);
    uint16_t *s_pid = reinterpret_cast<uint16_t *>(smem + lay.pid_off);
    uint16_t *s_whist = reinterpret_cast<uint16_t *>(smem + lay.whist_off);

    const int P = f.nbuckets();
    const int lane = threadIdx.x & 31, warp = threadIdx.x >> 5;
    const unsigned lt_mask = (1u << lane) - 1u;
    if (seg.cbeg != nullptr && (int)blockIdx.x >= *seg.ctotal) return;
    const int64_t beg = seg.cbeg ? seg.cbeg[blockIdx.x] : ((int64_t)blockIdx.x * L / T) * PT_TILE;
    const int64_t end = seg.cbeg ? seg.cend[blockIdx.x] : min(n, ((int64_t)(blockIdx.x + 1) * L / T) * PT_TILE);

    uint64_t *s_kptr = reinterpret_cast<uint64_t *>(smem + lay.kptr_off);
    uint64_t *s_vptr = reinterpret_cast<uint64_t *>(smem + lay.vptr_off);
    if (seg.key_ptrs) {
        for (int p = threadIdx.x; p < P; p += PT_THREADS) {
            s_gpos[p] = (int64_t)tile_off[(int64_t)p * T + blockIdx.x];
            s_kptr[p] = seg.key_ptrs[p];
            if constexpr (HAS_VAL) s_vptr[p] = seg.val_ptrs[p];
        }
    } else if (seg.cbeg) {
        for (int p = threadIdx.x; p < P; p += PT_THREADS) s_gpos[p] = seg.chunk_off[(int64_t)blockIdx.x * P + p];
    } else {
        for (int p = threadIdx.x; p < P; p += PT_THREADS)
            s_gpos[p] = bucket_base[p] + (int64_t)tile_off[(int64_t)p * T + blockIdx.x];
    }

    const int E = (P + PT_THREADS - 1) / PT_THREADS;

    for (int64_t tile = beg; tile < end; tile += TILE) {
        const int rows = (int)min((int64_t)TILE, end - tile);
        for (int i = threadIdx.x; i < PT_WARPS * P; i += PT_THREADS) s_whist[i] = 0;

        KeyT k[ITEMS];
        ValT v[ITEMS];
        const int64_t wbase = tile + (int64_t)warp * (32 * ITEMS) + lane;
#pragma unroll
        for (int j = 0; j < ITEMS; j++) {
            int64_t idx = wbase + j * 32;
            k[j] = idx < end ? keys[idx] : KeyT(0);
        }
        if constexpr (HAS_VAL) {
#pragma unroll
            for (int j = 0; j < ITEMS; j++) {
                int64_t idx = wbase + j * 32;
                if (idx < end) v[j] = vals[idx];
            }
        }
        __syncthreads();

        uint16_t pid[ITEMS], rank[ITEMS];
        uint16_t *wh = s_whist + warp * P;
#pragma unroll
        for (int j = 0; j < ITEMS; j++) {
            const bool ok = (wbase + j * 32) < end;
            const int p = ok ? f.bucket(key_hash<KeyT, PRE>(k[j], f)) : P;
            if (seg.unordered) {
                pid[j] = (uint16_t)p;
                if (ok) {
                    const unsigned old = atomicAdd(reinterpret_cast<unsigned *>(wh) + (p >> 1), (p & 1) ? 0x10000u : 1u);
                    rank[j] = (uint16_t)((p & 1) ? (old >> 16) : (old & 0xffffu));
                }
                continue;
            }
            const unsigned m = __match_any_sync(0xffffffffu, p);
            int base = 0;
            if (ok) base = wh[p];
            __syncwarp();
            pid[j] = (uint16_t)p;
            rank[j] = (uint16_t)(base + __popc(m & lt_mask));
            if (ok && lane == __ffs(m) - 1) wh[p] = (uint16_t)(base + __popc(m));
            __syncwarp();
        }
        __syncthreads();

        for (int p = threadIdx.x; p < P; p += PT_THREADS) {
            int run = 0;
#pragma unroll
            for (int w = 0; w < PT_WARPS; w++) {
                int t = s_whist[w * P + p];
                s_whist[w * P + p] = (uint16_t)run;
                run += t;
            }
            s_tcount[p] = run;
        }
        __syncthreads();
        {
            const int b = threadIdx.x * E;
            int sum = 0;
            for (int i = b; i < min(b + E, P); i++) sum += s_tcount[i];
            int tot;
            int run = block_excl_scan(sum, s_warp, &tot);
            for (int i = b; i < min(b + E, P); i++) {
                s_tstart[i] = run;
                run += s_tcount[i];
            }
        }
        __syncthreads();

#pragma unroll
        for (int j = 0; j < ITEMS; j++) {
            const int p = pid[j];
            if (p < P) {
                const int pos = s_tstart[p] + s_whist[warp * P + p] + rank[j];
                s_key[pos] = k[j];
                if constexpr (HAS_VAL) s_val[pos] = v[j];
                s_pid[pos] = (uint16_t)p;
            }
        }
        __syncthreads();

        for (int i = threadIdx.x; i < rows; i += PT_THREADS) {
            const int p = s_pid[i];
            const int64_t dst = s_gpos[p] + (int64_t)(i - s_tstart[p]);
            if (seg.key_ptrs) {
                reinterpret_cast<KeyT *>(s_kptr[p])[dst] = s_key[i];
                if constexpr (HAS_VAL) reinterpret_cast<ValT *>(s_vptr[p])[dst] = s_val[i];
            } else {
                out_keys[dst] = s_key[i];
                if constexpr (HAS_VAL) out_vals[dst] = s_val[i];
            }
        }
        __syncthreads();
        for (int p = threadIdx.x; p < P; p += PT_THREADS) s_gpos[p] += s_tcount[p];
    }
}


struct BulkSmem {
    int64_t key_off, val_off, gpos_off, cnt_off, sk_off, sv_off, vd_off, total;
    int32_t key_slots, val_slots;
};
static BulkSmem bulk_smem(int kb, int vb, int32_t P, int tile, bool ptr_mode = false) {
    BulkSmem s;
    int64_t o = 0;
    const int padk = 16 / kb - 1, padv = vb ? 16 / vb - 1 : 0;
    s.key_slots = tile + P * padk;
    s.val_slots = vb ? tile + P * padv : 0;
    s.key_off = o; o += align_up((int64_t)s.key_slots * kb, 128);
    s.val_off = o; o += align_up((int64_t)s.val_slots * vb, 128);
    s.gpos_off = o; o += align_up((int64_t)P * 8, 16);
    s.cnt_off = o; o += align_up((int64_t)P * 4 * 2, 16);
    s.sk_off = o; o += align_up((int64_t)P * 4, 16);
    s.sv_off = o; o += align_up((int64_t)P * 4, 16);
    s.vd_off = o; if (ptr_mode && vb) o += align_up((int64_t)P * 8, 16);
    s.total = o;
    return s;
}

__device__ __forceinline__ void bulk_store_s2g(void *gdst, uint32_t ssrc, uint32_t bytes) {
    asm volatile("cp.async.bulk.global.shared::cta.bulk_group [%0], [%1], %2;" ::"l"(gdst), "r"(ssrc), "r"(bytes) : "memory");
}

template <typename T>
__device__ __forceinline__ void flush_run(T *__restrict__ out, int64_t g, const T *s_col, uint32_t s_col_addr, int s0, int cnt) {
    constexpr int A = 16 / (int)sizeof(T);
    T *dst = out + g;
    int head = (int)(((16u - (uint32_t)((uintptr_t)dst & 15u)) & 15u) / (uint32_t)sizeof(T));
    if (head > cnt) head = cnt;
    const int mid = ((cnt - head) / A) * A;
    for (int i = 0; i < head; i++) dst[i] = s_col[s0 + i];
    if (mid) bulk_store_s2g(dst + head, s_col_addr + (uint32_t)(s0 + head) * (uint32_t)sizeof(T), (uint32_t)mid * (uint32_t)sizeof(T));
    for (int i = head + mid; i < cnt; i++) dst[i] = s_col[s0 + i];
}

template <int FMODE>
__device__ __forceinline__ int bucket_of(const PartFn &f, int64_t h) {
    if constexpr (FMODE == 1) {
        const uint32_t sub = (uint32_t)(((uint64_t)PartFn::mixed(h) << f.sub_bits) >> 32);
        return (int)((((uint32_t)h & (uint32_t)(f.P - 1)) << f.sub_bits) | sub);
    } else if constexpr (FMODE == 2) {
        return (int)((PartFn::mixed(h) >> f.shift) & (uint32_t)(f.P - 1));
    } else {
        return f.bucket(h);
    }
}

template <typename KeyT, typename ValT, int PRE, int NT, int FMODE, bool PTRS = false>
__global__ void __launch_bounds__(NT, NT == 1024 ? 1 : 2)
k_part_scatter_bulk(const KeyT *__restrict__ keys, const ValT *__restrict__ vals, int64_t n, int64_t L,
                    PartFn f, const int32_t *__restrict__ tile_off, int32_t T,
                    const int64_t *__restrict__ bucket_base, KeyT *__restrict__ out_keys,
                    ValT *__restrict__ out_vals, BulkSmem lay, SegTab seg) {
    constexpr bool HAS_VAL = !std::is_same<ValT, NoVal>::value;
    constexpr int ITEMS = NT == 256 ? 16 : 8;
    constexpr int TILE = NT * ITEMS;
    constexpr int NW = NT / 32;
    constexpr int AK = 16 / (int)sizeof(KeyT);
    constexpr int AV = HAS_VAL ? 16 / (int)sizeof(typename std::conditional<HAS_VAL, ValT, int64_t>::type) : 1;
    extern __shared__ __align__(128) unsigned char smem_bulk[];
    unsigned char *smem = smem_bulk;
    __shared__ int s_warp[NW];
    KeyT *s_key = reinterpret_cast<KeyT *>(smem + lay.key_off);
    ValT *s_val = reinterpret_cast<ValT *>(smem + lay.val_off);
    int64_t *s_gpos = reinterpret_cast<int64_t *>(smem + lay.gpos_off);
    uint32_t *s_cnt = reinterpret_cast<uint32_t *>(smem + lay.cnt_off);
    int32_t *s_sk = reinterpret_cast<int32_t *>(smem + lay.sk_off);
    int32_t *s_sv = reinterpret_cast<int32_t *>(smem + lay.sv_off);
    constexpr bool ptrs = PTRS;
    int64_t *s_vd = reinterpret_cast<int64_t *>(smem + lay.vd_off);
    const uint32_t key_addr = (uint32_t)__cvta_generic_to_shared(s_key);
    const uint32_t val_addr = (uint32_t)__cvta_generic_to_shared(s_val);

    const int P = f.nbuckets();
    const int lane = threadIdx.x & 31, warp = threadIdx.x >> 5;
    if (seg.cbeg != nullptr && (int)blockIdx.x >= *seg.ctotal) return;
    const int64_t beg = seg.cbeg ? seg.cbeg[blockIdx.x] : ((int64_t)blockIdx.x * L / T) * PT_TILE;
    const int64_t end = seg.cbeg ? seg.cend[blockIdx.x] : min(n, ((int64_t)(blockIdx.x + 1) * L / T) * PT_TILE);
    if (seg.cbeg) {
        for (int p = threadIdx.x; p < P; p += NT) s_gpos[p] = seg.chunk_off[(int64_t)blockIdx.x * P + p];
    } else if constexpr (PTRS) {
        for (int p = threadIdx.x; p < P; p += NT) {
            const int64_t ke = (int64_t)(seg.key_ptrs[p] / sizeof(KeyT));
            s_gpos[p] = ke + (int64_t)tile_off[(int64_t)p * T + blockIdx.x];
            if constexpr (HAS_VAL) s_vd[p] = (int64_t)(seg.val_ptrs[p] / sizeof(ValT)) - ke;
        }
    } else {
        for (int p = threadIdx.x; p < P; p += NT)
            s_gpos[p] = bucket_base[p] + (int64_t)tile_off[(int64_t)p * T + blockIdx.x];
    }
    for (int p = threadIdx.x; p < 2 * P; p += NT) s_cnt[p] = 0;
    const int E = (P + NT - 1) / NT;

    KeyT k[ITEMS];
    ValT v[ITEMS];
    auto load_tile = [&](int64_t tile) {
        const KeyT *kp = keys + tile + warp * (32 * ITEMS) + lane;
        if (tile + TILE <= end) {
#pragma unroll
            for (int j = 0; j < ITEMS; j++) k[j] = kp[j * 32];
            if constexpr (HAS_VAL) {
                const ValT *vp = vals + tile + warp * (32 * ITEMS) + lane;
#pragma unroll
                for (int j = 0; j < ITEMS; j++) v[j] = vp[j * 32];
            }
        } else {
            const int left = (int)(end - tile) - warp * (32 * ITEMS) - lane;
#pragma unroll
            for (int j = 0; j < ITEMS; j++) k[j] = j * 32 < left ? kp[j * 32] : KeyT(0);
            if constexpr (HAS_VAL) {
                const ValT *vp = vals + tile + warp * (32 * ITEMS) + lane;
#pragma unroll
                for (int j = 0; j < ITEMS; j++)
                    if (j * 32 < left) v[j] = vp[j * 32];
            }
        }
    };
    if (beg < end) load_tile(beg);
    __syncthreads();

    int par = 0;
    for (int64_t tile = beg; tile < end; tile += TILE, par ^= 1) {
        uint32_t *cnt = s_cnt + par * P;
        uint32_t pr[ITEMS];
        if (tile + TILE <= end) {
#pragma unroll
            for (int j = 0; j < ITEMS; j++) {
                const int p = bucket_of<FMODE>(f, key_hash<KeyT, PRE>(k[j], f));
                pr[j] = ((uint32_t)p << 16) | atomicAdd(&cnt[p], 1u);
            }
        } else {
            const int left = (int)(end - tile) - warp * (32 * ITEMS) - lane;
#pragma unroll
            for (int j = 0; j < ITEMS; j++) {
                pr[j] = 0xffffffffu;
                if (j * 32 < left) {
                    const int p = bucket_of<FMODE>(f, key_hash<KeyT, PRE>(k[j], f));
                    pr[j] = ((uint32_t)p << 16) | atomicAdd(&cnt[p], 1u);
                }
            }
        }
        asm volatile("cp.async.bulk.wait_group.read 0;" ::: "memory");
        __syncthreads();

        {
            const int b = threadIdx.x * E;
            int sum = 0;
            for (int i = b; i < min(b + E, P); i++) sum += (int)cnt[i];
            int tot;
            int run = block_excl_scan<NW>(sum, s_warp, &tot);
            for (int i = b; i < min(b + E, P); i++) {
                const int64_t g = s_gpos[i];
                const uint32_t gk = (uint32_t)(((uintptr_t)(out_keys + g)) / sizeof(KeyT));
                const int basek = run + i * (AK - 1);
                s_sk[i] = basek + (int)((gk - (uint32_t)basek) & (uint32_t)(AK - 1));
                if constexpr (HAS_VAL) {
                    const uint32_t gv = (uint32_t)(((uintptr_t)(out_vals + (ptrs ? g + s_vd[i] : g))) / sizeof(ValT));
                    const int basev = run + i * (AV - 1);
                    s_sv[i] = basev + (int)((gv - (uint32_t)basev) & (uint32_t)(AV - 1));
                }
                run += (int)cnt[i];
            }
        }
        __syncthreads();

#pragma unroll
        for (int j = 0; j < ITEMS; j++) {
            const int p = (int)(pr[j] >> 16), r = (int)(pr[j] & 0xffffu);
            if (p != 0xffff) {
                s_key[s_sk[p] + r] = k[j];
                if constexpr (HAS_VAL) s_val[s_sv[p] + r] = v[j];
            }
        }
        if (tile + TILE < end) load_tile(tile + TILE);
        asm volatile("fence.proxy.async.shared::cta;" ::: "memory");
        __syncthreads();

        if constexpr (HAS_VAL) {
            for (int q0 = 0; q0 < 2 * P; q0 += NT) {
                const int q = q0 + (int)threadIdx.x;
                const int p = q >> 1;
                const bool on = q < 2 * P;
                const int c = on ? (int)cnt[p] : 0;
                const int64_t g = on ? s_gpos[p] : 0;
                if (c) {
                    if (q & 1) flush_run<ValT>(out_vals, ptrs ? g + s_vd[p] : g, s_val, val_addr, s_sv[p], c);
                    else flush_run<KeyT>(out_keys, g, s_key, key_addr, s_sk[p], c);
                }
                __syncwarp();
                if (c && !(q & 1)) {
                    s_gpos[p] = g + c;
                    cnt[p] = 0;
                }
            }
        } else {
            for (int p = threadIdx.x; p < P; p += NT) {
                const int c = (int)cnt[p];
                if (c) {
                    const int64_t g = s_gpos[p];
                    flush_run<KeyT>(out_keys, g, s_key, key_addr, s_sk[p], c);
                    s_gpos[p] = g + c;
                    cnt[p] = 0;
                }
            }
        }
        asm volatile("cp.async.bulk.commit_group;" ::: "memory");
    }
    asm volatile("cp.async.bulk.wait_group 0;" ::: "memory");
}

template <typename KeyT, int PRE>
static int launch_count(const void *keys, int64_t n, const Plan &pl, const PartFn &f,
                        int32_t *tile_counts, cudaStream_t st) {
    size_t sh = (size_t)f.nbuckets() * sizeof(int32_t) * (f.nbuckets() <= PT_COUNT_PRIV ? PT_WARPS : 1);
    DPK_LAUNCH(pl.label_count ? pl.label_count : (pl.seg.cbeg ? "seg_count" : "part_count"), st, k_part_count<KeyT, PRE><<<pl.T, PT_THREADS, sh, st>>>((const KeyT *)keys, n, pl.L, f, tile_counts, pl.T, pl.seg, g_count_mode));
    return DPK_OK;
}

static int dispatch_count(const void *keys, int key_kind, int64_t n, const Plan &pl, const PartFn &f,
                          int32_t *tile_counts, cudaStream_t st) {
    if (key_kind >= DPK_K_UNORDERED) key_kind -= DPK_K_UNORDERED;
    switch (key_kind) {
    case -1: return launch_count<int64_t, true>(keys, n, pl, f, tile_counts, st);
    case DPK_K_I64: return launch_count<int64_t, false>(keys, n, pl, f, tile_counts, st);
    case DPK_K_I32: return launch_count<int32_t, false>(keys, n, pl, f, tile_counts, st);
    case DPK_K_F64: return launch_count<double, false>(keys, n, pl, f, tile_counts, st);
    case DPK_K_U64: return launch_count<uint64_t, false>(keys, n, pl, f, tile_counts, st);
    case DPK_K_F32: return launch_count<float, false>(keys, n, pl, f, tile_counts, st);
    case DPK_K_ROWID:
        if (!f.row_hash) return fail(DPK_ERR_INVALID, "DPK_K_ROWID needs key_aux (the per-row hash column)");
        return launch_count<int64_t, 2>(keys, n, pl, f, tile_counts, st);
    }
    return fail(DPK_ERR_UNSUPPORTED, "key kind %d is unhashable by portable_hash", key_kind);
}

template <typename KeyT, typename ValT, int PRE, int ITEMS>
static int launch_scatter_items(const void *keys, const void *vals, int64_t n, const Plan &pl, const PartFn &f,
                                const int32_t *tile_off, const int64_t *bucket_base, void *out_keys,
                                void *out_vals, cudaStream_t st) {
    constexpr int vb = std::is_same<ValT, NoVal>::value ? 0 : (int)sizeof(ValT);
    ScatterSmem lay = scatter_smem((int)sizeof(KeyT), vb, f.nbuckets(), pl.seg.key_ptrs != nullptr, PT_THREADS * ITEMS);
    auto kern = k_part_scatter<KeyT, ValT, PRE, ITEMS>;
    if (lay.total > 227 * 1024)
        return fail(DPK_ERR_UNSUPPORTED, "%d buckets need %lld B of shared memory", f.nbuckets(), (long long)lay.total);
    DPK_CUDA_TRY(cudaFuncSetAttribute(kern, cudaFuncAttributeMaxDynamicSharedMemorySize, (int)lay.total));
    DPK_LAUNCH(pl.label_scatter ? pl.label_scatter : (pl.seg.cbeg ? "seg_scatter" : "part_scatter"), st,
               kern<<<pl.T, PT_THREADS, (size_t)lay.total, st>>>((const KeyT *)keys, (const ValT *)vals, n, pl.L, f,
                                                                tile_off, pl.T, bucket_base, (KeyT *)out_keys,
                                                                (ValT *)out_vals, lay, pl.seg));
    return DPK_OK;
}

template <typename KeyT, typename ValT, int PRE>
static int launch_scatter_bulk(const void *keys, const void *vals, int64_t n, const Plan &pl, const PartFn &f,
                               const int32_t *tile_off, const int64_t *bucket_base, void *out_keys,
                               void *out_vals, cudaStream_t st) {
    constexpr int vb = std::is_same<ValT, NoVal>::value ? 0 : (int)sizeof(ValT);
    int nt = g_scatter_threads;
    if (nt == 512 && pl.seg.cbeg != nullptr && g_scatter_seg_wide) nt = 1024;
    if (nt == 512 && g_scatter_seg_wide && sizeof(KeyT) <= 4 && (vb == 0 || vb <= 4)) nt = 1024;
    if (nt == 512 && g_scatter_wide_from > 0 && f.nbuckets() >= g_scatter_wide_from) nt = 1024;
    const bool ptr_mode = pl.seg.key_ptrs != nullptr;
    if (ptr_mode && nt == 512 && g_scatter_ptr_threads == 1024) nt = 1024;
    if (nt == 1024 && bulk_smem((int)sizeof(KeyT), vb, f.nbuckets(), 8192, ptr_mode).total > 220 * 1024) nt = 512;
    BulkSmem lay = bulk_smem((int)sizeof(KeyT), vb, f.nbuckets(), nt == 1024 ? 8192 : PT_TILE, ptr_mode);
    const int fmode = f.mode == 5 ? 2 : ((f.mode == 0 || f.mode == 1) ? 1 : 0);
    if (ptr_mode) {
        auto kp = nt == 1024 ? (fmode == 1 ? k_part_scatter_bulk<KeyT, ValT, PRE, 1024, 1, true> : k_part_scatter_bulk<KeyT, ValT, PRE, 1024, 0, true>)
                             : (fmode == 1 ? k_part_scatter_bulk<KeyT, ValT, PRE, 512, 1, true> : k_part_scatter_bulk<KeyT, ValT, PRE, 512, 0, true>);
        if (nt != 512 && nt != 1024) return fail(DPK_ERR_UNSUPPORTED, "pointer mode needs 512- or 1024-thread CTAs");
        DPK_CUDA_TRY(cudaFuncSetAttribute(kp, cudaFuncAttributeMaxDynamicSharedMemorySize, (int)lay.total));
        DPK_LAUNCH(pl.label_scatter ? pl.label_scatter : "part_scatter", st,
                   kp<<<pl.T, nt, (size_t)lay.total, st>>>((const KeyT *)keys, (const ValT *)vals, n, pl.L, f, tile_off, pl.T,
                                                          bucket_base, (KeyT *)out_keys, (ValT *)out_vals, lay, pl.seg));
        return DPK_OK;
    }
    auto kern = nt == 1024 ? (fmode == 2 ? k_part_scatter_bulk<KeyT, ValT, PRE, 1024, 2> :
                              fmode == 1 ? k_part_scatter_bulk<KeyT, ValT, PRE, 1024, 1> : k_part_scatter_bulk<KeyT, ValT, PRE, 1024, 0>)
              : nt == 512 ? (fmode == 2 ? k_part_scatter_bulk<KeyT, ValT, PRE, 512, 2> :
                             fmode == 1 ? k_part_scatter_bulk<KeyT, ValT, PRE, 512, 1> : k_part_scatter_bulk<KeyT, ValT, PRE, 512, 0>)
                          : k_part_scatter_bulk<KeyT, ValT, PRE, 256, 0>;
    DPK_CUDA_TRY(cudaFuncSetAttribute(kern, cudaFuncAttributeMaxDynamicSharedMemorySize, (int)lay.total));
    DPK_LAUNCH(pl.label_scatter ? pl.label_scatter : (pl.seg.cbeg ? "seg_scatter" : "part_scatter"), st,
               kern<<<pl.T, nt, (size_t)lay.total, st>>>((const KeyT *)keys, (const ValT *)vals, n, pl.L, f,
                                                                tile_off, pl.T, bucket_base, (KeyT *)out_keys,
                                                                (ValT *)out_vals, lay, pl.seg));
    return DPK_OK;
}

template <typename KeyT, typename ValT, int PRE>
static int launch_scatter(const void *keys, const void *vals, int64_t n, const Plan &pl_in, const PartFn &f,
                          const int32_t *tile_off, const int64_t *bucket_base, void *out_keys,
                          void *out_vals, cudaStream_t st) {
    Plan pl = pl_in;
    if (pl.seg.unordered == 2) {
        constexpr int vb = std::is_same<ValT, NoVal>::value ? 0 : (int)sizeof(ValT);
        if (bulk_smem((int)sizeof(KeyT), vb, f.nbuckets(), PT_TILE, pl.seg.key_ptrs != nullptr).total <= 110 * 1024)
            return launch_scatter_bulk<KeyT, ValT, PRE>(keys, vals, n, pl, f, tile_off, bucket_base, out_keys, out_vals, st);
        pl.seg.unordered = (f.nbuckets() % 2 == 0) ? 1 : 0;
    }
    if (g_scatter_items == 8)
        return launch_scatter_items<KeyT, ValT, PRE, 8>(keys, vals, n, pl, f, tile_off, bucket_base, out_keys, out_vals, st);
    return launch_scatter_items<KeyT, ValT, PRE, 16>(keys, vals, n, pl, f, tile_off, bucket_base, out_keys, out_vals, st);
}

template <typename KeyT, int PRE>
static int dispatch_val(const void *keys, const void *vals, int32_t val_bytes, int64_t n, const Plan &pl,
                        const PartFn &f, const int32_t *tile_off, const int64_t *bucket_base,
                        void *out_keys, void *out_vals, cudaStream_t st) {
    if (vals == nullptr || val_bytes == 0)
        return launch_scatter<KeyT, NoVal, PRE>(keys, nullptr, n, pl, f, tile_off, bucket_base, out_keys, nullptr, st);
    if (val_bytes == 8)
        return launch_scatter<KeyT, int64_t, PRE>(keys, vals, n, pl, f, tile_off, bucket_base, out_keys, out_vals, st);
    if (val_bytes == 4)
        return launch_scatter<KeyT, int32_t, PRE>(keys, vals, n, pl, f, tile_off, bucket_base, out_keys, out_vals, st);
    return fail(DPK_ERR_UNSUPPORTED, "val_bytes must be 0, 4 or 8, got %d", val_bytes);
}

static int dispatch_scatter(const void *keys, int key_kind, const void *vals, int32_t val_bytes, int64_t n,
                            const Plan &pl_in, const PartFn &f, const int32_t *tile_off,
                            const int64_t *bucket_base, void *out_keys, void *out_vals, cudaStream_t st) {
    Plan pl = pl_in;
    if (key_kind >= DPK_K_UNORDERED) {
        key_kind -= DPK_K_UNORDERED;
        if (f.nbuckets() % 2 == 0) pl.seg.unordered = 1;
        if (g_scatter_bulk && (pl.seg.key_ptrs == nullptr || g_scatter_ptr_bulk)) pl.seg.unordered = 2;
    } else if (pl.seg.unordered && g_scatter_bulk && pl.seg.key_ptrs == nullptr) {
        pl.seg.unordered = 2;
    }
    switch (key_kind) {
    case -1: return dispatch_val<int64_t, true>(keys, vals, val_bytes, n, pl, f, tile_off, bucket_base, out_keys, out_vals, st);
    case DPK_K_I64: return dispatch_val<int64_t, false>(keys, vals, val_bytes, n, pl, f, tile_off, bucket_base, out_keys, out_vals, st);
    case DPK_K_I32: return dispatch_val<int32_t, false>(keys, vals, val_bytes, n, pl, f, tile_off, bucket_base, out_keys, out_vals, st);
    case DPK_K_F64: return dispatch_val<double, false>(keys, vals, val_bytes, n, pl, f, tile_off, bucket_base, out_keys, out_vals, st);
    case DPK_K_U64: return dispatch_val<uint64_t, false>(keys, vals, val_bytes, n, pl, f, tile_off, bucket_base, out_keys, out_vals, st);
    case DPK_K_F32: return dispatch_val<float, false>(keys, vals, val_bytes, n, pl, f, tile_off, bucket_base, out_keys, out_vals, st);
    case DPK_K_ROWID:
        if (!f.row_hash) return fail(DPK_ERR_INVALID, "DPK_K_ROWID needs key_aux (the per-row hash column)");
        return dispatch_val<int64_t, 2>(keys, vals, val_bytes, n, pl, f, tile_off, bucket_base, out_keys, out_vals, st);
    }
    return fail(DPK_ERR_UNSUPPORTED, "key kind %d is unhashable by portable_hash", key_kind);
}

static int check_common(const void *keys, int64_t n, int32_t P, int32_t sub_bits, void *ws, int64_t ws_bytes) {
    if (n < 0 || n >= ((int64_t)1 << 31)) return fail(DPK_ERR_INVALID, "n=%lld out of range [0, 2^31)", (long long)n);
    if (P < 1 || sub_bits < 0 || sub_bits > 12 || ((int64_t)P << sub_bits) > DPK_MAX_PARTITIONS)
        return fail(DPK_ERR_UNSUPPORTED, "P=%d (x 2^%d sub-buckets) out of range [1, %d]", P, sub_bits, DPK_MAX_PARTITIONS);
    P <<= sub_bits;
    if (n > 0 && !keys) return fail(DPK_ERR_INVALID, "keys is NULL");
    if (!ws || ws_bytes < ws_total_bytes(P)) return fail(DPK_ERR_WORKSPACE, "workspace needs %lld B, got %lld", (long long)ws_total_bytes(P), (long long)ws_bytes);
    return DPK_OK;
}

constexpr int SEG_CHUNK_TILES = 4;
constexpr int64_t SEG_CHUNK = (int64_t)SEG_CHUNK_TILES * PT_TILE;

static inline int64_t seg_max_chunks(int64_t n, int32_t F1, int32_t nsrc) {
    return n / SEG_CHUNK + (int64_t)F1 * nsrc + 1;
}

__global__ void __launch_bounds__(PT_THREADS)
k_seg_plan(const int64_t *__restrict__ seg_start, const int64_t *__restrict__ seg_rows, int32_t nsrc, int32_t F1,
           int64_t *__restrict__ brow_off, int64_t *__restrict__ cfirst, int64_t *__restrict__ cbeg,
           int64_t *__restrict__ cend, int32_t *__restrict__ ctotal) {
    __shared__ long long s_rows[PT_THREADS], s_chunks[PT_THREADS];
    const int E = (F1 + PT_THREADS - 1) / PT_THREADS;
    const int b0 = threadIdx.x * E, b1 = min(b0 + E, F1);
    long long rows = 0, chunks = 0;
    for (int b = b0; b < b1; b++)
        for (int s = 0; s < nsrc; s++) {
            long long r = seg_rows[(int64_t)s * F1 + b];
            rows += r;
            chunks += (r + SEG_CHUNK - 1) / SEG_CHUNK;
        }
    s_rows[threadIdx.x] = rows;
    s_chunks[threadIdx.x] = chunks;
    __syncthreads();
    long long rbase = 0, cbase = 0;
    for (int t = 0; t < (int)threadIdx.x; t++) { rbase += s_rows[t]; cbase += s_chunks[t]; }
    for (int b = b0; b < b1; b++) {
        brow_off[b] = rbase;
        cfirst[b] = cbase;
        for (int s = 0; s < nsrc; s++) {
            const long long r0 = seg_start[(int64_t)s * F1 + b], r = seg_rows[(int64_t)s * F1 + b];
            for (long long o = 0; o < r; o += SEG_CHUNK) {
                cbeg[cbase] = r0 + o;
                cend[cbase] = r0 + min(r, o + SEG_CHUNK);
                cbase++;
            }
            rbase += r;
        }
    }
    if (b0 < F1 && b1 == F1) { brow_off[F1] = rbase; cfirst[F1] = cbase; *ctotal = (int32_t)cbase; }
    if (F1 == 0 && threadIdx.x == 0) { brow_off[0] = 0; cfirst[0] = 0; *ctotal = 0; }
}

__global__ void __launch_bounds__(PT_THREADS)
k_seg_scan(const int32_t *__restrict__ chunk_counts, const int64_t *__restrict__ cfirst,
           const int64_t *__restrict__ brow_off, int32_t F1, int32_t S2, int64_t *__restrict__ chunk_off,
           int64_t *__restrict__ fine_off) {
    extern __shared__ int32_t s_tot[];
    __shared__ int s_warp[PT_WARPS];
    const int b = blockIdx.x;
    const int64_t c0 = cfirst[b], c1 = cfirst[b + 1];
    for (int p = threadIdx.x; p < S2; p += PT_THREADS) {
        int t = 0;
        for (int64_t c = c0; c < c1; c++) t += chunk_counts[c * S2 + p];
        s_tot[p] = t;
    }
    __syncthreads();
    const int E = (S2 + PT_THREADS - 1) / PT_THREADS;
    const int p0 = threadIdx.x * E, p1 = min(p0 + E, S2);
    int sum = 0;
    for (int p = p0; p < p1; p++) sum += s_tot[p];
    int tot;
    int run = block_excl_scan(sum, s_warp, &tot);
    for (int p = p0; p < p1; p++) {
        int t = s_tot[p];
        s_tot[p] = run;
        run += t;
    }
    __syncthreads();
    const int64_t base = brow_off[b];
    for (int p = threadIdx.x; p < S2; p += PT_THREADS) {
        int64_t pos = base + s_tot[p];
        fine_off[(int64_t)b * S2 + p] = pos;
        for (int64_t c = c0; c < c1; c++) {
            chunk_off[c * S2 + p] = pos;
            pos += chunk_counts[c * S2 + p];
        }
    }
    if (b == F1 - 1 && threadIdx.x == 0) fine_off[(int64_t)F1 * S2] = brow_off[F1];
}

int64_t seg_multisplit_ws_bytes(int64_t n, int32_t F1, int32_t S2, int32_t nsrc) {
    const int64_t maxc = seg_max_chunks(n, F1, nsrc);
    return align_up((int64_t)(F1 + 1) * 8, 256) * 2 + 256 + align_up(maxc * 8, 256) * 2 +
           align_up(maxc * S2 * 4, 256) + align_up(maxc * S2 * 8, 256);
}

int seg_multisplit(const void *keys, int key_kind, const void *vals, int32_t val_bytes, int64_t n,
                   const PartFn &fine, int32_t F1, int32_t nsrc, const int64_t *seg_start,
                   const int64_t *seg_rows, void *out_keys, void *out_vals, int64_t *fine_off, void *ws,
                   int64_t ws_bytes, cudaStream_t st, bool stable) {
    const int32_t S2 = fine.nbuckets();
    if (ws_bytes < seg_multisplit_ws_bytes(n, F1, S2, nsrc)) return fail(DPK_ERR_WORKSPACE, "segmented multisplit workspace too small");
    const int64_t maxc = seg_max_chunks(n, F1, nsrc);
    char *w = (char *)ws;
    int64_t *brow_off = (int64_t *)w; w += align_up((int64_t)(F1 + 1) * 8, 256);
    int64_t *cfirst = (int64_t *)w; w += align_up((int64_t)(F1 + 1) * 8, 256);
    int32_t *ctotal = (int32_t *)w; w += 256;
    int64_t *cbeg = (int64_t *)w; w += align_up(maxc * 8, 256);
    int64_t *cend = (int64_t *)w; w += align_up(maxc * 8, 256);
    int32_t *chunk_counts = (int32_t *)w; w += align_up(maxc * S2 * 4, 256);
    int64_t *chunk_off = (int64_t *)w;
    DPK_LAUNCH("seg_plan", st, k_seg_plan<<<1, PT_THREADS, 0, st>>>(seg_start, seg_rows, nsrc, F1, brow_off, cfirst, cbeg, cend, ctotal));
    Plan pl;
    pl.T = (int32_t)maxc;
    pl.L = 0;
    pl.seg = SegTab{cbeg, cend, ctotal, chunk_counts, chunk_off, nullptr, nullptr, (S2 % 2 == 0) ? 1 : (g_scatter_bulk ? 2 : 0)};
    if (stable) {
        pl.seg.unordered = 0;
        pl.label_count = "radix_count";
        pl.label_scatter = "radix_scatter";
    }
    int rc = DPK_OK;
    if (n > 0) {
        rc = dispatch_count(keys, key_kind, n, pl, fine, nullptr, st);
        if (rc) return rc;
    }
    DPK_LAUNCH("seg_scan", st, k_seg_scan<<<F1, PT_THREADS, (size_t)S2 * 4, st>>>(chunk_counts, cfirst, brow_off, F1, S2, chunk_off, fine_off));
    if (n > 0) rc = dispatch_scatter(keys, key_kind, vals, val_bytes, n, pl, fine, nullptr, nullptr, out_keys, out_vals, st);
    return rc;
}

}

using namespace dpk;

extern "C" {

int64_t dpk_partition_workspace_bytes(int64_t n, int32_t nbuckets) {
    (void)n;
    if (nbuckets < 1) nbuckets = 1;
    return ws_total_bytes(nbuckets);
}

int dpk_partition_count(const void *keys, int key_kind, const int64_t *key_aux, int64_t n, int32_t P,
                        const int64_t *thresholds, int32_t nthr, int32_t sub_bits, int64_t *out_counts,
                        void *ws, int64_t ws_bytes, dpk_stream_t stream) {
    int rc = check_common(keys, n, P, sub_bits, ws, ws_bytes);
    if (rc) return rc;
    if (!out_counts) return fail(DPK_ERR_INVALID, "out_counts is NULL");
    PartFn f;
    rc = make_partfn(P, thresholds, nthr, sub_bits, &f);
    if (rc) return rc;
    f.row_hash = key_aux;
    const int32_t F = f.nbuckets();
    cudaStream_t st = (cudaStream_t)stream;
    int32_t *tile_counts = (int32_t *)ws;
    Plan pl = make_plan(n);
    if (n == 0) {
        DPK_CUDA_TRY(cudaMemsetAsync(tile_counts, 0, (size_t)F * pl.T * 4, st));
    } else {
        rc = dispatch_count(keys, key_kind, n, pl, f, tile_counts, st);
        if (rc) return rc;
    }
    DPK_LAUNCH("part_scan", st, k_part_scan<<<F, PT_THREADS, 0, st>>>(tile_counts, pl.T, out_counts));
    return DPK_OK;
}

int dpk_partition_scatter(const void *keys, int key_kind, const int64_t *key_aux, const void *vals,
                          int32_t val_bytes, int64_t n, int32_t P, const int64_t *thresholds, int32_t nthr,
                          int32_t sub_bits,
                          const int64_t *bucket_base, void *out_keys, void *out_vals, void *ws,
                          int64_t ws_bytes, dpk_stream_t stream) {
    int rc = check_common(keys, n, P, sub_bits, ws, ws_bytes);
    if (rc) return rc;
    if (n == 0) return DPK_OK;
    if (!bucket_base || !out_keys) return fail(DPK_ERR_INVALID, "NULL pointer");
    PartFn f;
    rc = make_partfn(P, thresholds, nthr, sub_bits, &f);
    if (rc) return rc;
    f.row_hash = key_aux;
    Plan pl = make_plan(n);
    return dispatch_scatter(keys, key_kind, vals, val_bytes, n, pl, f, (const int32_t *)ws, bucket_base,
                            out_keys, out_vals, (cudaStream_t)stream);
}

int dpk_partition(const void *keys, int key_kind, const int64_t *key_aux, const void *vals, int32_t val_bytes,
                  int64_t n, int32_t P, const int64_t *thresholds, int32_t nthr, int32_t sub_bits, void *out_keys, void *out_vals,
                  int64_t *out_offsets, void *ws, int64_t ws_bytes, dpk_stream_t stream) {
    int rc = check_common(keys, n, P, sub_bits, ws, ws_bytes);
    if (rc) return rc;
    if (!out_offsets) return fail(DPK_ERR_INVALID, "out_offsets is NULL");
    const int32_t F = P << sub_bits;
    int64_t *totals = (int64_t *)((char *)ws + ws_counts_bytes(F));
    rc = dpk_partition_count(keys, key_kind, key_aux, n, P, thresholds, nthr, sub_bits, totals, ws, ws_bytes, stream);
    if (rc) return rc;
    cudaStream_t st = (cudaStream_t)stream;
    DPK_LAUNCH("part_offsets", st, k_part_offsets<<<1, PT_THREADS, 0, st>>>(totals, F, out_offsets));
    return dpk_partition_scatter(keys, key_kind, key_aux, vals, val_bytes, n, P, thresholds, nthr, sub_bits, out_offsets,
                                 out_keys, out_vals, ws, ws_bytes, stream);
// ... 104 lines not shown
```

### dpark_b200/peer.py

```python
import torch
import torch.distributed as dist

from . import _native as nv
from .shuffle import Received, owner_blocks


class PeerExchange(object):

    def __init__(self, capacity, key_dtype, val_dtype, device=None, group=None, mode="push", buffers=2):
        import torch.distributed._symmetric_memory as symm
        if mode not in ("push", "fused"):
            raise ValueError("mode must be 'push' (scatter locally, then block pushes) or 'fused' "
                             "(the scatter kernel stores into peer memory)")
        self.mode = mode
        self.group = group or dist.group.WORLD
        self.rank = dist.get_rank(self.group)
        self.world = dist.get_world_size(self.group)
        self.device = device or torch.device("cuda", torch.cuda.current_device())
        self.capacity = int(capacity)
        self.nbuf = max(1, int(buffers))
        name = self.group.group_name
        self._keys, self._vals, self._hk, self._hv, self._kb, self._vb, self._db = [], [], [], [], [], [], []
        self._pk, self._pv, self._kp, self._vp = [], [], [], []
        for _ in range(self.nbuf):
# ... 9 lines not shown
            self._db.append(torch.cat([self._kb[-1], self._vb[-1]]).contiguous())
            self._pk.append([hk.get_buffer(r, (self.capacity,), key_dtype) for r in range(self.world)])
            self._pv.append([hv.get_buffer(r, (self.capacity,), val_dtype) for r in range(self.world)])
            self._kp.append([int(p) for p in hk.buffer_ptrs])
            self._vp.append([int(p) for p in hv.buffer_ptrs])
        self.step = 0
        self.side = torch.cuda.Stream(device=self.device, priority=-1)
        self.err = torch.zeros(1, dtype=torch.int64, device=self.device)
        self._closed = False
        self._dump = None
        self.copy_sms = 16
        self.copy_engine = 2
        self.side2 = torch.cuda.Stream(device=self.device, priority=-1)
        self._tab_host = None

    @property
    def keys(self):
        return self._keys[self.step % self.nbuf]

    @property
    def vals(self):
        return self._vals[self.step % self.nbuf]

    @property
    def key_base(self):
        return self._kb[self.step % self.nbuf]

    @property
    def val_base(self):
        return self._vb[self.step % self.nbuf]

    @property
    def dst_base(self):
        return self._db[self.step % self.nbuf]

    def barrier(self):
        self._hk[self.step % self.nbuf].barrier()

    def advance(self):
        self.step += 1

    def note_need(self, need_rows):
        torch.maximum(self.err, (need_rows - self.capacity).reshape(1), out=self.err)

    def check(self):
        over = int(self.err.item())
        if over > 0:
            self.err.zero_()
            raise RuntimeError("peer receive buffer too small: a step needed %d rows, capacity %d (results of that "
                               "step are invalid)" % (self.capacity + over, self.capacity))

    def dump(self, rows, with_vals=True):
        if self._dump is None or self._dump[0].numel() < rows:
            self._dump = (torch.empty(max(rows, 1), dtype=self._keys[0].dtype, device=self.device),
                          torch.empty(max(rows, 1), dtype=self._vals[0].dtype, device=self.device))
        return self._dump[0], (self._dump[1] if with_vals else None)

    def close(self):
        if not self._closed:
            self._closed = True
            self._keys, self._vals, self._hk, self._hv, self._kb, self._vb, self._db = [], [], [], [], [], [], []
            self._pk, self._pv = [], []


def push_plan(all_counts, blocks, rank):
    G, F = all_counts.shape
    csum = torch.zeros(G, F + 1, dtype=torch.int64, device=all_counts.device)
    csum[:, 1:] = torch.cumsum(all_counts, 1)
    bidx = torch.tensor(blocks, dtype=torch.int64, device=all_counts.device)
    edge = csum[:, bidx]
    R = edge[:, 1:] - edge[:, :-1]
    src_base = torch.cumsum(R, 0) - R
    return edge[rank, :-1].contiguous(), src_base[rank].contiguous(), R[rank].contiguous(), R.sum(0)


def _landed(seg, capacity):
    flat = seg.reshape(-1)
    start = torch.cumsum(flat, 0) - flat
    return torch.minimum(flat, (capacity - start).clamp(min=0)).view(seg.shape).contiguous()


def exchange_push(px, mo, need_host_count=False):
    G, rank, dev = px.world, px.rank, px.device
    P, sb = mo.P, mo.sub_bits
    F = P << sb
    if mo.keys.dtype != px.keys.dtype or (mo.vals is not None and mo.vals.dtype != px.vals.dtype):
        raise TypeError("receive buffers are (%s, %s) but the map output is (%s, %s): allocate the PeerExchange "
                        "with the column dtypes that are exchanged (after a map-side combine the value column "
                        "is the accumulator type)" % (px.keys.dtype, px.vals.dtype, mo.keys.dtype,
                                                      None if mo.vals is None else mo.vals.dtype))
    counts = (mo.offsets[1:] - mo.offsets[:-1]).contiguous()
    all_counts = torch.empty(G * F, dtype=torch.int64, device=dev)
    dist.all_gather_into_tensor(all_counts, counts, group=px.group)
    all_counts = all_counts.view(G, F)
    blocks = [b << sb for b in owner_blocks(P, G)]
    per_block = ((P + G - 1) // G) << sb
    src, dst, nby, seg = nv.push_plan(all_counts, G, per_block, rank, rank, mo.keys, mo.vals,
                                      px.dst_base if mo.vals is not None else px.key_base, px.capacity, px.err)
    nv.copy_segments(src, dst, nby)
    px.barrier()
    b0, b1 = blocks[rank], blocks[rank + 1]
    keys, vals = px.keys, (px.vals if mo.vals is not None else None)
    px.advance()
    if need_host_count:
        nrecv = min(int(seg.sum().item()), px.capacity)
        return Received(keys[:nrecv], None if vals is None else vals[:nrecv], seg, b0 >> sb, (b1 - b0) >> sb, sb)
    return Received(keys, vals, seg, b0 >> sb, (b1 - b0) >> sb, sb, bound=True)


def map_exchange_overlapped(px, key_chunks, val_chunks, P, thresholds=None, sub_bits=0, unordered=True, halves=2):
    from . import shuffle as sh
    G, rank, dev = px.world, px.rank, px.device
    F = P << sub_bits
    M = len(key_chunks)
    H = max(1, min(halves, M))
    has_v = val_chunks[0] is not None
    bounds = [(M * h) // H for h in range(H + 1)]
    gk, gv = [], []
    for h in range(H):
        sel = slice(bounds[h], bounds[h + 1])
        k1 = sh._as_one(key_chunks[sel])
        v1 = sh._as_one(val_chunks[sel]) if has_v else None
        if k1 is None or (has_v and v1 is None) or k1.numel() >= (1 << 31):
            return _map_exchange_overlapped_splits(px, key_chunks, val_chunks, P, thresholds, sub_bits, unordered, H)
        gk.append(k1)
        gv.append(v1)
    counts, wss = [], []
    for k in gk:
        c, ws = nv.partition_count(k, P, thresholds, False, sub_bits, None, None, unordered)
        counts.append(c)
        wss.append(ws)
    gc = torch.stack(counts)
    all_counts = torch.empty(G * H * F, dtype=torch.int64, device=dev)
    dist.all_gather_into_tensor(all_counts, gc.reshape(-1), group=px.group)
    all_counts = all_counts.view(G * H, F)
    per_block = ((P + G - 1) // G) << sub_bits
    main = torch.cuda.current_stream()
    seg = None
    for h in range(H):
        offsets = torch.zeros(F + 1, dtype=torch.int64, device=dev)
        torch.cumsum(gc[h], 0, out=offsets[1:])
        out_k = torch.empty_like(gk[h])
        out_v = torch.empty_like(gv[h]) if has_v else None
        nv.partition_scatter(gk[h], gv[h], P, offsets, out_k, out_v, wss[h], thresholds, False, sub_bits, None, unordered)
        src, dst, nby, sg = nv.push_plan(all_counts, G, per_block, rank * H + h, rank, out_k, out_v,
                                         px.dst_base if has_v else px.key_base, px.capacity, px.err, want_seg=(h == 0))
        if h == 0:
            seg = sg
        ready = torch.cuda.Event()
        ready.record(main)
        with torch.cuda.stream(px.side):
            px.side.wait_event(ready)
            nv.copy_segments(src, dst, nby, sms=px.copy_sms if h + 1 < H else 0)
            for t in (out_k, out_v, src, dst, nby):
                if t is not None:
                    t.record_stream(px.side)
    main.wait_stream(px.side)
    px.barrier()
    blocks = [b << sub_bits for b in owner_blocks(P, G)]
    b0, b1 = blocks[rank], blocks[rank + 1]
    keys, vals = px.keys, (px.vals if has_v else None)
    px.advance()
    return Received(keys, vals, seg, b0 >> sub_bits, (b1 - b0) >> sub_bits, sub_bits, bound=True)


def shuffle_pipelined(px, key_chunks, val_chunks, P, op, thresholds=None, sub_bits=0, groups=2, parts=2):
# ... 257 lines not shown
```

### dpark_b200/shuffle.py

```python
import torch

from . import _native as nv

FINE_BUCKET_ROWS = 1536
MAX_SECOND_LEVEL = 1024
TARGET_BUCKET_ROWS = FINE_BUCKET_ROWS * MAX_SECOND_LEVEL
MAX_FIRST_LEVEL = 512


def owner_blocks(P, G):
    per = (P + G - 1) // G
    return [min(P, g * per) for g in range(G + 1)]


def choose_sub_bits(rows, P, world=1):
    total = float(rows) * max(1, world)
    nf = total / FINE_BUCKET_ROWS
    if nf <= P:
        return 0
    want = min(float(MAX_FIRST_LEVEL), 2.0 * nf ** 0.5)
    sb = 0
    while sb < 12 and (P << (sb + 1)) <= min(nv.MAX_PARTITIONS, MAX_FIRST_LEVEL) and (P << sb) < want:
        sb += 1
    while sb < 12 and (P << (sb + 1)) <= min(nv.MAX_PARTITIONS, 1024) and total / float(P << sb) > TARGET_BUCKET_ROWS:
        sb += 1
    return sb


def bind_to_gpu_numa_node(local_rank):
    import os
    try:
        props = torch.cuda.get_device_properties(local_rank)
        bus = "%04x:%02x:%02x.0" % (props.pci_domain_id, props.pci_bus_id, props.pci_device_id)
        with open("/sys/bus/pci/devices/%s/numa_node" % bus) as f:
            node = int(f.read().strip())
        if node < 0:
            return None
        with open("/sys/devices/system/node/node%d/cpulist" % node) as f:
            spec = f.read().strip()
        cpus = set()
        for part in spec.split(","):
            if "-" in part:
                lo, hi = part.split("-")
                cpus.update(range(int(lo), int(hi) + 1))
            elif part:
                cpus.add(int(part))
        allowed = cpus & set(os.sched_getaffinity(0))
        if not allowed:
            return None
        os.sched_setaffinity(0, allowed)
        return node
    except Exception:
        return None


class MapOutput(object):
    __slots__ = ("keys", "vals", "offsets", "P", "sub_bits")

    def __init__(self, keys, vals, offsets, P, sub_bits):
        self.keys, self.vals, self.offsets, self.P, self.sub_bits = keys, vals, offsets, P, sub_bits


def _as_one(chunks):
    first = chunks[0]
    if first is None or not first.is_contiguous():
        return None
    base = first.untyped_storage().data_ptr()
    at, total = first.storage_offset(), 0
    for c in chunks:
        if (c is None or c.dtype != first.dtype or c.dim() != 1 or not c.is_contiguous() or c.storage_offset() != at
                or c.untyped_storage().data_ptr() != base):
            return None
        at += c.numel()
        total += c.numel()
    return torch.empty(0, dtype=first.dtype, device=first.device).set_(first.untyped_storage(), first.storage_offset(), (total,))


def map_side(key_chunks, val_chunks, P, thresholds=None, prehashed=False, sub_bits=0, row_hash=None,
             unordered=False):
    F = P << sub_bits
    if len(key_chunks) > 1:
        whole_k, whole_v = _as_one(key_chunks), (_as_one(val_chunks) if val_chunks[0] is not None else None)
        if whole_k is not None and (val_chunks[0] is None or whole_v is not None) and whole_k.numel() < (1 << 31):
            key_chunks, val_chunks = [whole_k], [whole_v]
    if len(key_chunks) == 1:
        k, v, off = nv.partition(key_chunks[0], val_chunks[0], P, thresholds, prehashed, sub_bits, row_hash, unordered)
        return MapOutput(k, v, off, P, sub_bits)
    dev = key_chunks[0].device
    counts, wss = [], []
    for k in key_chunks:
        c, ws = nv.partition_count(k, P, thresholds, prehashed, sub_bits, None, row_hash, unordered)
        counts.append(c)
        wss.append(ws)
    cm = torch.stack(counts)
    tot = cm.sum(0)
    offsets = torch.zeros(F + 1, dtype=torch.int64, device=dev)
    torch.cumsum(tot, 0, out=offsets[1:])
    base = offsets[:-1].unsqueeze(0) + (torch.cumsum(cm, 0) - cm)
    n = sum(int(k.numel()) for k in key_chunks)
    out_k = torch.empty(n, dtype=key_chunks[0].dtype, device=dev)
    has_v = val_chunks[0] is not None
    out_v = torch.empty(n, dtype=val_chunks[0].dtype, device=dev) if has_v else None
    for m, (k, v) in enumerate(zip(key_chunks, val_chunks)):
        nv.partition_scatter(k, v, P, base[m].contiguous(), out_k, out_v, wss[m], thresholds, prehashed, sub_bits,
                             row_hash, unordered)
    return MapOutput(out_k, out_v, offsets, P, sub_bits)


class Received(object):
    __slots__ = ("keys", "vals", "seg", "part_first", "nparts", "sub_bits", "bound")

    def __init__(self, keys, vals, seg, part_first, nparts, sub_bits, bound=False):
        self.keys, self.vals, self.seg = keys, vals, seg
        self.part_first, self.nparts, self.sub_bits = part_first, nparts, sub_bits
        self.bound = bound


_LOCAL_ONLY = [0]


class local_only(object):

    def __enter__(self):
        _LOCAL_ONLY[0] += 1

    def __exit__(self, *a):
        _LOCAL_ONLY[0] -= 1


def exchange(mo, group=None):
    import torch.distributed as dist
    G = dist.get_world_size(group) if (dist.is_available() and dist.is_initialized() and not _LOCAL_ONLY[0]) else 1
    P, sb = mo.P, mo.sub_bits
    if G == 1:
        seg = (mo.offsets[1:] - mo.offsets[:-1]).unsqueeze(0)
        return Received(mo.keys, mo.vals, seg, 0, P, sb)
    rank = dist.get_rank(group)
    F = P << sb
    blocks = [b << sb for b in owner_blocks(P, G)]
    counts = (mo.offsets[1:] - mo.offsets[:-1]).contiguous()
    all_counts = torch.empty(G * F, dtype=torch.int64, device=counts.device)
    dist.all_gather_into_tensor(all_counts, counts, group=group)
    all_counts = all_counts.view(G, F)
    host_counts = all_counts.cpu()
    send_splits = [int(host_counts[rank, blocks[d]:blocks[d + 1]].sum()) for d in range(G)]
    b0, b1 = blocks[rank], blocks[rank + 1]
    recv_splits = [int(host_counts[s, b0:b1].sum()) for s in range(G)]
    nrecv = sum(recv_splits)
    rk = torch.empty(nrecv, dtype=mo.keys.dtype, device=mo.keys.device)
    dist.all_to_all_single(rk, mo.keys, recv_splits, send_splits, group=group)
    rv = None
    if mo.vals is not None:
        rv = torch.empty(nrecv, dtype=mo.vals.dtype, device=mo.vals.device)
        dist.all_to_all_single(rv, mo.vals, recv_splits, send_splits, group=group)
    seg = all_counts[:, b0:b1].contiguous()
    return Received(rk, rv, seg, b0 >> sb, (b1 - b0) >> sb, sb)


def reduce_side(rx, op, P, thresholds=None):
    dev = rx.keys.device
    if rx.nparts == 0:
        z = torch.zeros(1, dtype=torch.int64, device=dev)
        return rx.keys[:0], (rx.vals[:0] if rx.vals is not None else None), z, z[:0]
    return nv.combine(rx.keys, rx.vals, op, P, rx.seg.contiguous(), rx.part_first, rx.nparts, thresholds,
                      rx.sub_bits)


RADIX_BITS = 8


def sort_by_key_bits(keys, vals, bits=None):
    bits = bits or RADIX_BITS
    n = int(keys.numel())
    if n <= 1:
        return keys, vals
    ormask = int(nv.key_or(keys).item()) & 0xFFFFFFFFFFFFFFFF
    ws = nv.partition_workspace(1 << bits, keys.device)
    src_k, src_v = keys, vals
    dst_k, dst_v = torch.empty_like(keys), (None if vals is None else torch.empty_like(vals))
    spare_k = spare_v = None
    shift = 0
    while shift < 64:
        width = min(bits, 64 - shift)
        if (ormask >> shift) & ((1 << width) - 1):
            nv.radix_pass(src_k, src_v, shift, width, dst_k, dst_v, ws)
            if src_k is keys:
                spare_k, spare_v = torch.empty_like(keys), (None if vals is None else torch.empty_like(vals))
                src_k, src_v, dst_k, dst_v = dst_k, dst_v, spare_k, spare_v
            else:
                src_k, src_v, dst_k, dst_v = dst_k, dst_v, src_k, src_v
        shift += width
    return src_k, src_v


def group_side(rx, P, thresholds=None, key_view=None, row_hash=None):
    if row_hash is not None:
        raise NotImplementedError("row-id keys are handled by dpark_b200.grouping")
    dev = rx.keys.device
    seg = rx.seg.contiguous()
    if rx.bound:
        nrecv = int(seg.sum().item())
        rx = Received(rx.keys[:nrecv], None if rx.vals is None else rx.vals[:nrecv], seg, rx.part_first, rx.nparts,
                      rx.sub_bits)
    k, v = rx.keys.view(torch.int64), rx.vals
    n = int(k.numel())
    nsrc, F = int(seg.shape[0]), int(seg.shape[1])
    bucket_rows = seg.sum(0, keepdim=True).contiguous()
    if n > 1:
        ormask = int(nv.key_or(k).item()) & 0xFFFFFFFFFFFFFFFF
        cur = seg
        for shift in range(0, 64, RADIX_BITS):
            if (ormask >> shift) & ((1 << RADIX_BITS) - 1):
                k, v = nv.radix_pass_seg(k, v, shift, RADIX_BITS, cur)
                cur = bucket_rows
        if cur is seg and nsrc > 1:
            k, v = nv.radix_pass_seg(k, v, 0, 1, cur)
    gk, gs, ng = nv.group_heads(k)
    off = torch.zeros(rx.nparts + 1, dtype=torch.int64, device=dev)
    if rx.nparts:
        torch.cumsum(bucket_rows.view(rx.nparts, -1).sum(1), 0, out=off[1:])
    return gk, gs, ng, v, off


def _world(group=None):
    import torch.distributed as dist
    return dist.get_world_size(group) if (dist.is_available() and dist.is_initialized() and not _LOCAL_ONLY[0]) else 1


def check_counts(cnt_h):
    if any(c < 0 for c in cnt_h):
        raise nv.NativeError("reduce side: a fine bucket overflowed its shared-memory table beyond the splittable hash "
                             "bits; the partition's result is invalid (dpk_combine out_counts = -1)")


class HostShuffle(object):

    def __init__(self, n_rows, key_dtype, val_dtype, P, op="sum", splits=8, thresholds=None, group=None,
                 device=None, sub_bits=None, world=1, peer_exchange=None, map_combine=False):
        self.P, self.op, self.splits, self.thresholds, self.group = P, op, splits, thresholds, group
        self.map_combine = map_combine
        self.peer_exchange = peer_exchange
        self.device = device or torch.device("cuda", torch.cuda.current_device())
        self.n = n_rows
        self.sub_bits = choose_sub_bits(n_rows, P, world) if sub_bits is None else sub_bits
        self.h_keys = torch.empty(n_rows, dtype=key_dtype).pin_memory()
        self.h_vals = torch.empty(n_rows, dtype=val_dtype).pin_memory()
        self.d_keys = torch.empty(n_rows, dtype=key_dtype, device=self.device)
        self.d_vals = torch.empty(n_rows, dtype=val_dtype, device=self.device)
# ... 91 lines not shown
        if s.busy:
            raise RuntimeError("all %d slots are in flight: collect() first" % len(self.slots))
        self.next_submit += 1
        per = (self.n + self.splits - 1) // self.splits
        with torch.cuda.stream(s.stream):
            kc, vc = [], []
            for i in range(self.splits):
                a, b = min(self.n, i * per), min(self.n, (i + 1) * per)
                s.d_keys[a:b].copy_(h_keys[a:b], non_blocking=True)
                s.d_vals[a:b].copy_(h_vals[a:b], non_blocking=True)
                kc.append(s.d_keys[a:b])
                vc.append(s.d_vals[a:b])
            mo = map_side(kc, vc, self.P, self.thresholds, False, self.sub_bits, unordered=self.kind == "reduce")
            if s.px is not None:
                from . import peer
                rx = peer.exchange_push(s.px, mo, need_host_count=self.kind == "group")
            else:
                rx = exchange(mo, self.group)
            if self.kind == "reduce":
                s.result = reduce_side(rx, self.op, self.P, self.thresholds)
            else:
                s.result = group_side(rx, self.P, self.thresholds)
            s.nparts, s.part_first = rx.nparts, rx.part_first
        s.busy = True

    def collect(self):
        s = self.slots[self.next_collect % len(self.slots)]
        if not s.busy:
            raise RuntimeError("nothing in flight")
        self.next_collect += 1
        with torch.cuda.stream(s.stream):
            res = self._collect_reduce(s) if self.kind == "reduce" else self._collect_group(s)
            s.stream.synchronize()
            if s.px is not None:
                s.px.check()
        s.result = None
        s.busy = False
        return res

    def _collect_reduce(self, s):
        ok, ov, po, cnt = s.result
        po_h, cnt_h = po.cpu().tolist(), cnt.cpu().tolist()
        check_counts(cnt_h)
        res, at = [], 0
        for j in range(s.nparts):
            a, c = po_h[j], cnt_h[j]
            s.out_keys[at:at + c].copy_(ok[a:a + c], non_blocking=True)
            s.out_vals[at:at + c].copy_(ov[a:a + c], non_blocking=True)
            res.append((s.part_first + j, s.out_keys[at:at + c], s.out_vals[at:at + c]))
            at += c
        self.d2h_bytes = at * (ok.element_size() + ov.element_size())
        return res

    def _collect_group(self, s):
        gk, gs, ng, ov, off = s.result
        G = int(ng.item())
        off_h = off.cpu().tolist()
        nval = int(ov.numel())
        s.out_keys[:G].copy_(gk[:G], non_blocking=True)
        s.out_starts[:G + 1].copy_(gs[:G + 1], non_blocking=True)
        s.out_vals[:nval].copy_(ov, non_blocking=True)
        s.stream.synchronize()
        starts = s.out_starts[:G + 1]
        first = torch.searchsorted(starts[:-1].contiguous(), torch.tensor(off_h, dtype=torch.int64)).tolist() if G else \
            [0] * len(off_h)
        res = []
        for j in range(s.nparts):
            g0, g1 = first[j], first[j + 1]
            res.append((s.part_first + j, s.out_keys[g0:g1], s.out_starts[g0:g1 + 1], s.out_vals))
        self.d2h_bytes = G * 8 + (G + 1) * 8 + nval * ov.element_size()
        return res

    def close(self):
        for s in self.slots:
            if s.px is not None:
                s.px.close()
                s.px = None
        self.slots = []


def combine_map_output(mo, op, thresholds=None):
    P, sb = mo.P, mo.sub_bits
    seg = (mo.offsets[1:] - mo.offsets[:-1]).unsqueeze(0)
    ok, ov, po, cnt = reduce_side(Received(mo.keys, mo.vals, seg, 0, P, sb), op, P, thresholds)
    po_h, cnt_h = po.cpu().tolist(), cnt.cpu().tolist()
    check_counts(cnt_h)
    keys = torch.cat([ok[a:a + c] for a, c in zip(po_h, cnt_h)])
    vals = torch.cat([ov[a:a + c] for a, c in zip(po_h, cnt_h)])
    return map_side([keys], [vals], P, thresholds, False, sb, unordered=True)


def reduce_by_key(key_chunks, val_chunks, P, op="sum", thresholds=None, group=None, sub_bits=None,
                  map_combine=False):
    if sub_bits is None:
        sub_bits = choose_sub_bits(sum(int(k.numel()) for k in key_chunks), P, _world(group))
    mo = map_side(key_chunks, val_chunks, P, thresholds, False, sub_bits, unordered=True)
    if map_combine:
        mo = combine_map_output(mo, op, thresholds)
    rx = exchange(mo, group)
    ok, ov, po, cnt = reduce_side(rx, op, P, thresholds)
    po_h, cnt_h = po.cpu().tolist(), cnt.cpu().tolist()
    check_counts(cnt_h)
    return [(rx.part_first + j, ok[po_h[j]:po_h[j] + cnt_h[j]], ov[po_h[j]:po_h[j] + cnt_h[j]])
            for j in range(rx.nparts)]
```

### dpark_b200/strings.py

```python
import numpy as np
import torch

from . import _native as nv
from . import columnar, shuffle


def _concat(splits):
    datas, offs, vals, base, rows = [], [np.zeros(1, np.int64)], [], 0, 0
    for c in splits:
        if c.n == 0:
            continue
        datas.append(c.keys)
        offs.append(c.key_offsets[1:] + base)
        base += int(c.key_offsets[-1])
        vals.append(c.vals)
        rows += c.n
    data = np.concatenate(datas) if datas else np.zeros(0, np.uint8)
    offsets = np.concatenate(offs)
    v = np.concatenate(vals) if vals else np.zeros(0, np.int64)
    return data, offsets, v, rows


def reduce_by_key_bytes(splits, key_kind, P, thresholds, op, dev, res):
    if shuffle._world() > 1:
        raise NotImplementedError("this is the one-GPU stage; under torch.distributed the rows are first routed to the "
                                  "rank owning their partition (dpark_b200.engine._routed_shuffle)")
    data, offsets, vals, n = _concat(splits)
    if n == 0:
        for p in range(P):
            res.parts[p] = ([], [])
        return res
    d_data = torch.from_numpy(data if data.size else np.zeros(1, np.uint8)).to(dev)
    d_off = torch.from_numpy(offsets).to(dev)
    d_vals = torch.from_numpy(vals).to(dev)
    key_objs = None
    if key_kind == columnar.KEY_TUPLE:
        key_objs = [k for c in splits if c.n for k in c.key_objs]
        h = columnar.tuple_hashes_on_device(key_objs, dev)
    else:
        h = nv.hash_bytes(d_data, d_off, nv.STR_UTF8 if key_kind == columnar.KEY_STR else nv.BYTES_SIGNED)
    rep = nv.dict_encode(d_data, d_off, h)
    sb = shuffle.choose_sub_bits(n, P)
    mo = shuffle.map_side([rep], [d_vals], P, thresholds, False, sb, row_hash=h, unordered=True)
    rx = shuffle.exchange(mo)
    ok, ov, off, cnt = nv.combine(rx.keys, rx.vals, op, P, rx.seg.contiguous(), rx.part_first, rx.nparts,
                                  thresholds, sb, row_hash=h)
    off_h, cnt_h = off.cpu().tolist(), cnt.cpu().tolist()
    shuffle.check_counts(cnt_h)
    ok_h, ov_h = ok.cpu().numpy(), ov.cpu().numpy()
    raw = data.tobytes()
    offs_l = offsets
    is_str = key_kind == columnar.KEY_STR
    for p in range(P):
        ids = ok_h[off_h[p]:off_h[p] + cnt_h[p]]
        keys = []
        for r in ids.tolist():
            if key_objs is not None:
                keys.append(key_objs[r])
                continue
            b = raw[offs_l[r]:offs_l[r + 1]]
            keys.append(b.decode("utf-8", "surrogatepass") if is_str else b)
        res.parts[p] = (keys, ov_h[off_h[p]:off_h[p] + cnt_h[p]].tolist())
    return res
```

### dpark_b200/textingest.py

```python
import os
import types

import numpy as np
import torch

from . import _native as nv
from . import shuffle


def _t_gen_strip_split(x):
    for w in x.strip().split():
        yield (w, 1)


def _t_gen_split(x):
    for w in x.split():
        yield (w, 1)


_t_list_strip_split = lambda x: [(w, 1) for w in x.strip().split()]
_t_list_split = lambda x: [(w, 1) for w in x.split()]
_t_split = lambda x: x.split()
_t_strip_split = lambda x: x.strip().split()
_t_pair_one = lambda x: (x, 1)
# ... 30 lines not shown
    def line_start_at_or_after(pos):
        if pos <= 0:
            return 0
        if pos >= size:
            return size
        with open(path, "rb") as f:
            f.seek(pos - 1)
            at = pos - 1
            while True:
                chunk = f.read(1 << 16)
                if not chunk:
                    return size
                i = chunk.find(b"\n")
                if i >= 0:
                    return at + i + 1
                at += len(chunk)
    return line_start_at_or_after(begin), line_start_at_or_after(end)


MAX_PIECE_BYTES = 1 << 30


def cut_pieces(path, a, b, size, max_bytes=None):
    max_bytes = max_bytes or MAX_PIECE_BYTES
    out = []
    while b - a > max_bytes:
        cut = owned_range(path, a + max_bytes, a + max_bytes, size)[0]
        if cut >= b:
            break
        out.append([a, cut])
        a = cut
    if b > a:
        out.append([a, b])
    return out


def reduce_tokens(text_rdd, split_indices, P, thresholds, op, dev, res, local_only=True):
    path = text_rdd.path
    size = os.path.getsize(path)
    splits = text_rdd.splits
    ranges = []
    for i in sorted(split_indices):
        a, b = owned_range(path, splits[i].begin, splits[i].end, size)
        if b > a:
            if ranges and ranges[-1][1] == a:
                ranges[-1][1] = b
            else:
                ranges.append([a, b])
    pieces = []
    for a, b in [piece for r in ranges for piece in cut_pieces(path, r[0], r[1], size)]:
        host = np.fromfile(path, dtype=np.uint8, count=b - a, offset=a)
        d_text = torch.from_numpy(host).to(dev)
        starts, lens, ascii_ok = nv.tokenize(d_text)
        if not ascii_ok:
            return None
        if starts.numel():
            pieces.append(nv.gather_bytes(d_text, starts, lens))
        del d_text
    if not pieces:
        for p in range(P):
            res.parts[p] = ([], [])
        return res
    if len(pieces) == 1:
        tok, off = pieces[0]
    else:
        tok = torch.cat([t for t, _ in pieces])
        offs, base = [pieces[0][1]], int(pieces[0][0].numel())
        for t, o in pieces[1:]:
            offs.append(o[1:] + base)
            base += int(t.numel())
        off = torch.cat(offs)
    n = int(off.numel()) - 1
    if n >= (1 << 31):
        raise nv.NativeError("more than 2^31 tokens in one shuffle")
    ones = torch.ones(n, dtype=torch.int64, device=dev)
    h = nv.hash_bytes(tok, off, nv.STR_UTF8)
    rep = nv.dict_encode(tok, off, h)
    sb = shuffle.choose_sub_bits(n, P)
    ctx = shuffle.local_only() if local_only else _Null()
    with ctx:
        mo = shuffle.map_side([rep], [ones], P, thresholds, False, sb, row_hash=h, unordered=True)
        rx = shuffle.exchange(mo)
        ok, ov, poff, cnt = nv.combine(rx.keys, rx.vals, op, P, rx.seg.contiguous(), rx.part_first, rx.nparts,
                                       thresholds, sb, row_hash=h)
    off_h, cnt_h = poff.cpu().tolist(), cnt.cpu().tolist()
    shuffle.check_counts(cnt_h)
    sel = torch.cat([ok[off_h[p]:off_h[p] + cnt_h[p]] for p in range(P)]) if P else ok[:0]
    lens_all = off[1:] - off[:-1]
    kb, ko = nv.gather_bytes(tok, off[:-1].contiguous(), lens_all.contiguous(), sel.contiguous())
    raw, ko_h = kb.cpu().numpy().tobytes(), ko.cpu().tolist()
    vals = torch.cat([ov[off_h[p]:off_h[p] + cnt_h[p]] for p in range(P)]).cpu().tolist() if P else []
    at = 0
    for p in range(P):
        c = cnt_h[p]
        keys = [raw[ko_h[i]:ko_h[i + 1]].decode("ascii") for i in range(at, at + c)]
        res.parts[p] = (keys, vals[at:at + c])
        at += c
    return res


class _Null(object):
    def __enter__(self):
        return self

    def __exit__(self, *a):
        return False
```

### include/dpark_b200.h

```cpp
#ifndef DPARK_B200_H
#define DPARK_B200_H

#include <stddef.h>
#include <stdint.h>

#ifdef __cplusplus
extern "C" {
#endif

#define DPK_ABI_VERSION 1

typedef void *dpk_stream_t;

enum {
    DPK_OK = 0,
    DPK_ERR_INVALID = -1,
    DPK_ERR_UNSUPPORTED = -2,
    DPK_ERR_WORKSPACE = -3,
    DPK_ERR_CUDA = -4
};

enum { DPK_K_I64 = 0, DPK_K_I32 = 1, DPK_K_F64 = 2, DPK_K_U64 = 3, DPK_K_F32 = 4,
       DPK_K_ROWID = 5  };
#define DPK_K_UNORDERED 0x100
enum { DPK_V_I64 = 0, DPK_V_F64 = 1, DPK_V_I32 = 2, DPK_V_F32 = 3 };
enum { DPK_OP_SUM = 0, DPK_OP_MIN = 1, DPK_OP_MAX = 2, DPK_OP_PROD = 3,
       DPK_OP_AND = 4, DPK_OP_OR = 5, DPK_OP_XOR = 6 };
enum { DPK_BYTES_SIGNED = 0,
       DPK_STR_UTF8 = 1 };

int dpk_abi_version(void);
const char *dpk_last_error(void);
int dpk_device_info(int32_t *h_info);

int dpk_hash_keys(const void *keys, int key_kind, int64_t n, int64_t *out_hash,
                  dpk_stream_t stream);
int dpk_hash_bytes(const uint8_t *data, const int64_t *offsets, int64_t n, int mode,
                   int64_t *out_hash, dpk_stream_t stream);

int dpk_hash_tuple(const int64_t *item_hash, int64_t n, int32_t arity, int64_t *out_hash, dpk_stream_t stream);
int dpk_partition_ids(const int64_t *hash, int64_t n, int32_t P, const int64_t *thresholds,
                      int32_t nthr, int32_t *out_pid, dpk_stream_t stream);

#define DPK_MAX_PARTITIONS 4096
int64_t dpk_partition_workspace_bytes(int64_t n, int32_t nbuckets);
int dpk_partition_count(const void *keys, int key_kind, const int64_t *key_aux, int64_t n, int32_t P,
                        const int64_t *thresholds, int32_t nthr, int32_t sub_bits,
                        int64_t *out_counts, void *ws, int64_t ws_bytes, dpk_stream_t stream);
int dpk_partition_scatter(const void *keys, int key_kind, const int64_t *key_aux, const void *vals,
                          int32_t val_bytes, int64_t n, int32_t P, const int64_t *thresholds,
                          int32_t nthr, int32_t sub_bits, const int64_t *bucket_base,
                          void *out_keys, void *out_vals, void *ws, int64_t ws_bytes,
                          dpk_stream_t stream);
int dpk_partition(const void *keys, int key_kind, const int64_t *key_aux, const void *vals,
                  int32_t val_bytes, int64_t n, int32_t P, const int64_t *thresholds, int32_t nthr,
                  int32_t sub_bits, void *out_keys, void *out_vals, int64_t *out_offsets, void *ws,
                  int64_t ws_bytes, dpk_stream_t stream);
int dpk_partition_scatter_ptrs(const void *keys, int key_kind, const int64_t *key_aux,
                               const void *vals, int32_t val_bytes, int64_t n, int32_t P,
                               const int64_t *thresholds, int32_t nthr, int32_t sub_bits,
                               const uint64_t *key_dst_ptrs, const uint64_t *val_dst_ptrs, void *ws,
                               int64_t ws_bytes, dpk_stream_t stream);
int dpk_copy_segments(const uint64_t *src_ptrs, const uint64_t *dst_ptrs, const int64_t *nbytes,
                      int32_t nseg, dpk_stream_t stream);
int dpk_memcpy_batch(const uint64_t *h_dst_ptrs, const uint64_t *h_src_ptrs, const int64_t *h_nbytes, int32_t count,
                     dpk_stream_t stream);
int dpk_push_plan(const int64_t *all_counts, int32_t nsrc, int32_t nranks, int32_t nbuckets, int32_t per_block,
                  int32_t my_src, int32_t my_rank, int32_t ncols, uint64_t src_keys, uint64_t src_vals,
                  const uint64_t *dst_base, int32_t key_bytes, int32_t val_bytes, int64_t capacity, uint64_t *src_ptrs,
                  uint64_t *dst_ptrs, int64_t *nbytes, int64_t *need_over, int64_t *seg_out, dpk_stream_t stream);
int dpk_push_plan_part(const int64_t *all_counts, int32_t nsrc, int32_t nranks, int32_t nbuckets, int32_t per_block,
                       int32_t blk_lo, int32_t blk_hi, int64_t dst_row0, int32_t my_src, int32_t my_rank, int32_t ncols,
                       uint64_t src_keys, uint64_t src_vals, const uint64_t *dst_base, int32_t key_bytes, int32_t val_bytes,
                       int64_t capacity, uint64_t *src_ptrs, uint64_t *dst_ptrs, int64_t *nbytes, int64_t *need_over,
                       int64_t *seg_out, dpk_stream_t stream);
int dpk_pipe_plan(const int64_t *all_counts, int32_t nsrc, int32_t nranks, int32_t nbuckets, int32_t per_block,
                  int32_t nparts, int64_t region_rows, int32_t my_src, int32_t my_rank, int32_t ncols, uint64_t src_keys,
                  uint64_t src_vals, const uint64_t *dst_base, int32_t key_bytes, int32_t val_bytes, int64_t *bucket_base,
                  uint64_t *src_ptrs, uint64_t *dst_ptrs, int64_t *nbytes, int64_t *need_over, int64_t *seg_out,
                  dpk_stream_t stream);
int dpk_fused_plan(const int64_t *all_counts, int32_t nranks, int32_t nbuckets, int32_t per_block, int32_t my_rank,
                   int32_t ncols, const uint64_t *dst_base, int32_t key_bytes, int32_t val_bytes, int64_t capacity,
                   uint64_t dump_keys, uint64_t dump_vals, uint64_t *key_ptrs, uint64_t *val_ptrs, int64_t *need_over,
                   int64_t *seg_out, dpk_stream_t stream);

int64_t dpk_combine_workspace_bytes(int64_t n, int32_t nbuckets, int32_t nsrc);
int dpk_combine(const void *keys, int key_kind, const int64_t *key_aux, const void *vals,
                int val_kind, int64_t n, int op, int32_t P, const int64_t *thresholds, int32_t nthr,
                int32_t sub_bits, int32_t part_first, int32_t nparts, int32_t nsrc,
                const int64_t *seg_rows, void *out_keys, void *out_vals, int64_t *out_offsets,
                int64_t *out_counts, void *ws, int64_t ws_bytes, dpk_stream_t stream);
int dpk_set_option(const char *name, int64_t value);

int dpk_key_or(const int64_t *keys, int64_t n, uint64_t *out_or, dpk_stream_t stream);
int dpk_gather_i64(const int64_t *src, const int64_t *idx, int64_t n, int64_t *out,
                   dpk_stream_t stream);
int dpk_radix_pass(const int64_t *keys, const void *vals, int32_t val_bytes, int64_t n, int32_t shift,
                   int32_t bits, int64_t *out_keys, void *out_vals, void *ws, int64_t ws_bytes,
                   dpk_stream_t stream);
int64_t dpk_radix_pass_seg_workspace_bytes(int64_t n, int32_t nbuckets, int32_t nsrc, int32_t bits);
int dpk_radix_pass_seg(const int64_t *keys, const void *vals, int32_t val_bytes, int64_t n, int32_t shift,
                       int32_t bits, int32_t nbuckets, int32_t nsrc, const int64_t *seg_rows, int64_t *out_keys,
                       void *out_vals, int64_t *out_fine_off, void *ws, int64_t ws_bytes, dpk_stream_t stream);
int64_t dpk_group_heads_workspace_bytes(int64_t n);
int dpk_group_heads(const int64_t *sorted_keys, int64_t n, int64_t *out_keys, int64_t *out_starts,
                    int64_t *out_ngroups, void *ws, int64_t ws_bytes, dpk_stream_t stream);

// ... 35 lines not shown
```

Before: 15.42 billion.

## Pack key/value pairs into interleaved rows through partition, multisplit and aggregate

```diff
diff --git a/dpark_b200/_native.py b/dpark_b200/_native.py
--- a/dpark_b200/_native.py
+++ b/dpark_b200/_native.py
@@ -205,6 +205,29 @@
 
 
 K_UNORDERED = 0x100
+K_PACKED = 0x200
+
+
+def packable(keys, vals, prehashed=False):
+    return vals is not None and not prehashed and keys.element_size() == vals.element_size()
+
+
+def packed_views(rows, key_dtype, val_dtype):
+    return rows[:, 0], (rows if val_dtype == rows.dtype else rows.view(val_dtype))[:, 1]
+
+
+def packed_source(keys, vals):
+    if keys is None or vals is None or keys.dim() != 1 or vals.dim() != 1 or keys.numel() != vals.numel():
+        return None
+    es = keys.element_size()
+    if (vals.element_size() != es or keys.stride() != (2,) or vals.stride() != (2,)
+            or vals.data_ptr() != keys.data_ptr() + es or keys.untyped_storage().data_ptr() != vals.untyped_storage().data_ptr()):
+        return None
+    return keys.as_strided((keys.numel(), 2), (2, 1))
+
+
+def packed_rows(n, key_dtype, device):
+    return torch.empty((n, 2), dtype=key_dtype, device=device)
 
 
 def _kk(keys, prehashed, row_hash, unordered=False):
@@ -230,7 +253,10 @@
     _need_cuda(keys, vals, bucket_base, out_keys, out_vals, ws, row_hash)
     thr, nthr = _thr(thresholds, keys.device)
     vb = 0 if vals is None else vals.element_size()
-    _check(lib().dpk_partition_scatter(_ptr(keys), _kk(keys, prehashed, row_hash, unordered), _ptr(row_hash), _ptr(vals), vb,
+    kk = _kk(keys, prehashed, row_hash, unordered)
+    if vals is not None and out_vals is None:
+        kk |= K_PACKED
+    _check(lib().dpk_partition_scatter(_ptr(keys), kk, _ptr(row_hash), _ptr(vals), vb,
                                        keys.numel(), P,
                                        _ptr(thr), nthr, sub_bits, _ptr(bucket_base), _ptr(out_keys),
                                        _ptr(out_vals), _ptr(ws), ws.numel(), _stream()))
@@ -329,7 +355,8 @@
     return kp, vp_, seg
 
 
-def partition(keys, vals, P, thresholds=None, prehashed=False, sub_bits=0, row_hash=None, unordered=False):
+def partition(keys, vals, P, thresholds=None, prehashed=False, sub_bits=0, row_hash=None, unordered=False,
+              packed=False):
     _need_cuda(keys, vals, row_hash)
     if vals is not None and vals.numel() != keys.numel():
         from .errors import DparkUserFatalError
@@ -337,11 +364,18 @@
     F = P << sub_bits
     thr, nthr = _thr(thresholds, keys.device)
     ws = partition_workspace(F, keys.device)
-    out_keys = torch.empty_like(keys)
-    out_vals = None if vals is None else torch.empty_like(vals)
+    kk = _kk(keys, prehashed, row_hash, unordered)
+    if packed:
+        if not packable(keys, vals, prehashed):
+            raise TypeError("packed rows need hashed keys and values of the same width")
+        out_keys, out_vals = packed_rows(keys.numel(), keys.dtype, keys.device), None
+        kk |= K_PACKED
+    else:
+        out_keys = torch.empty_like(keys)
+        out_vals = None if vals is None else torch.empty_like(vals)
     offsets = torch.empty(F + 1, dtype=torch.int64, device=keys.device)
     vb = 0 if vals is None else vals.element_size()
-    _check(lib().dpk_partition(_ptr(keys), _kk(keys, prehashed, row_hash, unordered), _ptr(row_hash), _ptr(vals), vb,
+    _check(lib().dpk_partition(_ptr(keys), kk, _ptr(row_hash), _ptr(vals), vb,
                                keys.numel(), P,
                                _ptr(thr), nthr, sub_bits, _ptr(out_keys), _ptr(out_vals), _ptr(offsets),
                                _ptr(ws), ws.numel(), _stream()))
@@ -353,8 +387,12 @@
 
 
 def combine(keys, vals, op, P, seg_rows, part_first=0, nparts=None, thresholds=None, sub_bits=0,
-            row_hash=None):
-    _need_cuda(keys, vals, seg_rows, row_hash)
+            row_hash=None, rows=None):
+    _need_cuda(seg_rows, row_hash, rows)
+    if rows is None:
+        rows = packed_source(keys, vals)
+    if rows is None:
+        _need_cuda(keys, vals)
     if nparts is None:
         nparts = P
     n = keys.numel()
@@ -368,12 +406,18 @@
     thr, nthr = _thr(thresholds, keys.device)
     ws_bytes = lib().dpk_combine_workspace_bytes(n, F, nsrc)
     ws = torch.empty(ws_bytes, dtype=torch.uint8, device=keys.device)
-    out_keys = torch.empty_like(keys)
+    out_keys = torch.empty(n, dtype=keys.dtype, device=keys.device)
     out_vals = torch.empty(n, dtype=acc_dtype(vals.dtype), device=keys.device)
     out_offsets = torch.empty(nparts + 1, dtype=torch.int64, device=keys.device)
     out_counts = torch.empty(nparts, dtype=torch.int64, device=keys.device)
     kk = key_kind(keys) if row_hash is None else K_ROWID
-    _check(lib().dpk_combine(_ptr(keys), kk, _ptr(row_hash), _ptr(vals), val_kind(vals), n, OPS[op], P,
+    src_k, src_v = keys, vals
+    if rows is not None:
+        if rows.dim() != 2 or rows.shape[1] != 2 or rows.shape[0] != n or keys.element_size() != vals.element_size():
+            raise ValueError("rows must be the packed [n, 2] buffer of the key and value columns")
+        kk |= K_PACKED
+        src_k, src_v = rows, None
+    _check(lib().dpk_combine(_ptr(src_k), kk, _ptr(row_hash), _ptr(src_v), val_kind(vals), n, OPS[op], P,
                              _ptr(thr), nthr, sub_bits, part_first, nparts, nsrc, _ptr(bucket_rows), _ptr(out_keys),
                              _ptr(out_vals), _ptr(out_offsets), _ptr(out_counts), _ptr(ws), ws_bytes,
                              _stream()))
diff --git a/dpark_b200/csrc/dpk_aggregate2.cuh b/dpark_b200/csrc/dpk_aggregate2.cuh
--- a/dpark_b200/csrc/dpk_aggregate2.cuh
+++ b/dpark_b200/csrc/dpk_aggregate2.cuh
@@ -180,7 +180,8 @@
     return v & 0xfffu;
 }
 
-template <typename KeyT, typename ValT, typename AccT, int MINB, bool CURSOR, bool BATCHED, bool FAST_ONLY = false>
+template <typename KeyT, typename ValT, typename AccT, int MINB, bool CURSOR, bool BATCHED, bool FAST_ONLY = false,
+          bool PACKED = false>
 __global__ void __launch_bounds__(AG2_THREADS, MINB)
 k_smem_aggregate2(const KeyT *__restrict__ keys, const ValT *__restrict__ vals, int op,
                   const int64_t *__restrict__ fine_off, int32_t nfine, int32_t fine_per_part,
@@ -220,7 +221,16 @@
 #pragma unroll
         for (int j = 0; j < NI; j++) {
             const int i = j * AG2_THREADS + (int)threadIdx.x;
-            if (i < w) { kr[j] = keys[g0 + i]; vr[j] = vals[g0 + i]; }
+            if (i < w) {
+                if constexpr (PACKED) {
+                    const PackedRow<KeyT, ValT> r = reinterpret_cast<const PackedRow<KeyT, ValT> *>(keys)[g0 + i];
+                    kr[j] = r.k;
+                    vr[j] = r.v;
+                } else {
+                    kr[j] = keys[g0 + i];
+                    vr[j] = vals[g0 + i];
+                }
+            }
         }
         between();
 #pragma unroll
diff --git a/dpark_b200/csrc/dpk_combine.cu b/dpark_b200/csrc/dpk_combine.cu
--- a/dpark_b200/csrc/dpk_combine.cu
+++ b/dpark_b200/csrc/dpk_combine.cu
@@ -185,14 +185,14 @@
 k_tbl_insert(const KeyT *__restrict__ keys, const int64_t *__restrict__ aux, const ValT *__restrict__ vals,
              int64_t n, const int64_t *__restrict__ rows_total, int op, PartFn f, int32_t bucket_first, int32_t F,
              const int64_t *__restrict__ tbl_off, Slot *__restrict__ table, Slot *__restrict__ side,
-             int32_t *__restrict__ side_used) {
+             int32_t *__restrict__ side_used, int64_t row_stride) {
     int64_t i = (int64_t)blockIdx.x * blockDim.x + threadIdx.x;
     int64_t stride = (int64_t)gridDim.x * blockDim.x;
     const int64_t rows = min(n, *rows_total);
     for (; i < rows; i += stride) {
-        const KeyT key = keys[i];
+        const KeyT key = keys[i * row_stride];
         const int64_t kb = key_bits<KeyT>(key);
-        const AccT v = (AccT)vals[i];
+        const AccT v = (AccT)vals[i * row_stride];
         Slot *s;
         if (kb == kEmpty) {
             s = side;
@@ -274,7 +274,7 @@
                 const int64_t *__restrict__ tbl_off, Slot *__restrict__ table, Slot *__restrict__ side,
                 int32_t *__restrict__ side_used, const int64_t *__restrict__ part_offsets,
                 KeyT *__restrict__ out_keys, int64_t *__restrict__ out_vals,
-                unsigned long long *__restrict__ out_counts, int *__restrict__ bucket_counter) {
+                unsigned long long *__restrict__ out_counts, int *__restrict__ bucket_counter, int64_t row_stride) {
     cg::cluster_group cluster = cg::this_cluster();
     const unsigned crank = cluster.block_rank();
     __shared__ int s_bucket;
@@ -299,8 +299,8 @@
             const int64_t r0 = seg_start[(int64_t)s * F + b];
             const int64_t rn = seg_rows[(int64_t)s * F + b];
             for (int64_t i = tid_c; i < rn; i += nth_c) {
-                const int64_t kb = key_bits<KeyT>(keys[r0 + i]);
-                const AccT v = (AccT)vals[r0 + i];
+                const int64_t kb = key_bits<KeyT>(keys[(r0 + i) * row_stride]);
+                const AccT v = (AccT)vals[(r0 + i) * row_stride];
                 Slot *sl;
                 if (kb == kEmpty) {
                     sl = side;
@@ -406,6 +406,7 @@
 
 struct Ctx {
     int key_kind, val_bytes;
+    bool packed;
     int64_t *fine_off;
     unsigned long long *fb_state;
     int *part_err;
@@ -439,8 +440,11 @@
         fine.row_hash = c.aux;
         KeyT *rekeys = (KeyT *)c.table;
         ValT *revals = (ValT *)((char *)c.table + (size_t)c.n * 8);
+        constexpr bool same_width = sizeof(KeyT) == sizeof(ValT);
+        const bool pack_fine = same_width && g_agg_impl == 1 && !g_agg_pipe && g_agg_cursor && !g_agg_batched && g_agg_split;
+        const int pack = (c.packed ? PK_IN : 0) | (pack_fine ? PK_OUT : 0);
         int rc = seg_multisplit(c.keys, c.key_kind, c.vals, (int32_t)sizeof(ValT), c.n, fine, c.F, c.nsrc, c.seg_start,
-                                c.seg_rows, rekeys, revals, c.fine_off, c.seg_ws, c.seg_ws_bytes, c.st);
+                                c.seg_rows, rekeys, revals, c.fine_off, c.seg_ws, c.seg_ws_bytes, c.st, false, pack);
         if (rc) return rc;
         const int32_t nfine = c.F * S2;
         int grid = sm_count() * 8;
@@ -485,6 +489,14 @@
             } else if (g_agg_cursor && !g_agg_batched && g_agg_split) {
                 auto fast = g_agg_ctas == 4 ? k_smem_aggregate2<KeyT, ValT, AccT, 4, true, false, true>
                                             : k_smem_aggregate2<KeyT, ValT, AccT, 3, true, false, true>;
+                auto aggb = k_smem_aggregate2<KeyT, ValT, AccT, 3, true, false>;
+                if constexpr (same_width) {
+                    if (pack_fine) {
+                        fast = g_agg_ctas == 4 ? k_smem_aggregate2<KeyT, ValT, AccT, 4, true, false, true, true>
+                                               : k_smem_aggregate2<KeyT, ValT, AccT, 3, true, false, true, true>;
+                        aggb = k_smem_aggregate2<KeyT, ValT, AccT, 3, true, false, false, true>;
+                    }
+                }
                 DPK_CUDA_TRY(cudaFuncSetAttribute(fast, cudaFuncAttributeMaxDynamicSharedMemorySize, smem2));
                 int *big_count = c.part_err + c.nparts, *list_counter = c.part_err + c.nparts + 1;
                 int *big_list = reinterpret_cast<int *>(c.fb_state);
@@ -492,7 +504,6 @@
                     rekeys, revals, c.op, c.fine_off, nfine, (1 << c.f.sub_bits) * S2, c.part_off,
                     (KeyT *)c.out_keys, c.out_vals, (long long *)c.out_counts, c.fb_state, c.bucket_counter, c.part_err,
                     nullptr, nullptr, timing, big_list, big_count));
-                auto aggb = k_smem_aggregate2<KeyT, ValT, AccT, 3, true, false>;
                 DPK_CUDA_TRY(cudaFuncSetAttribute(aggb, cudaFuncAttributeMaxDynamicSharedMemorySize, smem2));
                 DPK_LAUNCH("smem_aggregate_big", c.st, aggb<<<sm_count() * 2, AG2_THREADS, smem2, c.st>>>(
                     rekeys, revals, c.op, c.fine_off, nfine, (1 << c.f.sub_bits) * S2, c.part_off,
@@ -530,7 +541,7 @@
         DPK_LAUNCH("bucket_reduce", c.st, kern<<<nclusters * BR_CLUSTER, BR_THREADS, 0, c.st>>>(
             (const KeyT *)c.keys, c.aux, (const ValT *)c.vals, c.op, ident, c.f.sub_bits, c.F, c.nsrc,
             c.seg_start, c.seg_rows, c.tbl_off, c.table, c.side, c.side_used, c.part_off, (KeyT *)c.out_keys,
-            c.out_vals, c.out_counts, c.bucket_counter));
+            c.out_vals, c.out_counts, c.bucket_counter, c.packed ? 2 : 1));
     } else {
         DPK_LAUNCH("tbl_init", c.st, k_tbl_init<<<grid_cap(c.max_slots, CB_THREADS, 16), CB_THREADS, 0, c.st>>>(
             c.table, c.tbl_off + c.F, ident));
@@ -538,7 +549,7 @@
             DPK_LAUNCH("tbl_insert", c.st, k_tbl_insert<KeyT, ValT, AccT><<<grid_cap(c.n, CB_THREADS, 16), CB_THREADS, 0, c.st>>>(
                 (const KeyT *)c.keys, c.aux, (const ValT *)c.vals, c.n, c.part_off + c.nparts, c.op, c.f,
                 c.part_first << c.f.sub_bits,
-                c.F, c.tbl_off, c.table, c.side, c.side_used));
+                c.F, c.tbl_off, c.table, c.side, c.side_used, c.packed ? 2 : 1));
         }
         size_t sh = (size_t)((c.nparts + 1) & ~1) * 4 + (size_t)c.nparts * 8;
         DPK_LAUNCH("tbl_compact", c.st, k_tbl_compact<KeyT><<<grid_cap(c.max_slots, CB_THREADS * 4, 8), CB_THREADS, sh, c.st>>>(
@@ -717,6 +728,16 @@
         return fail(DPK_ERR_INVALID, "bad partition range first=%d n=%d P=%d", part_first, nparts, P);
     if (nsrc < 1) return fail(DPK_ERR_INVALID, "nsrc must be >= 1");
     if (!seg_rows || !out_counts || !out_offsets || !ws) return fail(DPK_ERR_INVALID, "NULL pointer");
+    const bool packed = key_kind >= 0 && (key_kind & DPK_K_PACKED);
+    if (packed) {
+        key_kind &= ~DPK_K_PACKED;
+        const int kw = (key_kind == DPK_K_I32 || key_kind == DPK_K_F32) ? 4 : 8;
+        const int vw = (val_kind == DPK_V_I32 || val_kind == DPK_V_F32) ? 4 : 8;
+        if (vals) return fail(DPK_ERR_INVALID, "packed rows: vals must be NULL");
+        if (kw != vw) return fail(DPK_ERR_UNSUPPORTED, "packed rows need values as wide as the keys");
+        if ((uintptr_t)keys % (2 * kw)) return fail(DPK_ERR_INVALID, "packed rows must be aligned to their %d-byte size", 2 * kw);
+        vals = keys ? (const char *)keys + kw : nullptr;
+    }
     if (n > 0 && (!keys || !vals || !out_keys || !out_vals)) return fail(DPK_ERR_INVALID, "NULL pointer");
     Ctx c;
     int rc = make_partfn(P, thresholds, nthr, sub_bits, &c.f);
@@ -727,6 +748,7 @@
     if (ws_bytes < dpk_combine_workspace_bytes(n, c.F, nsrc))
         return fail(DPK_ERR_WORKSPACE, "workspace needs %lld B, got %lld", (long long)dpk_combine_workspace_bytes(n, c.F, nsrc), (long long)ws_bytes);
     c.keys = keys; c.vals = vals; c.n = n; c.op = op; c.aux = key_aux; c.key_kind = key_kind; c.val_bytes = 0;
+    c.packed = packed;
     if (key_kind == DPK_K_ROWID && n > 0 && !key_aux) return fail(DPK_ERR_INVALID, "DPK_K_ROWID needs key_aux (the per-row hash column)");
     c.part_first = part_first; c.nparts = nparts; c.nsrc = nsrc; c.seg_rows = seg_rows;
     c.max_slots = max_slots_for(n, c.F);
diff --git a/dpark_b200/csrc/dpk_common.cuh b/dpark_b200/csrc/dpk_common.cuh
--- a/dpark_b200/csrc/dpk_common.cuh
+++ b/dpark_b200/csrc/dpk_common.cuh
@@ -190,7 +190,14 @@
 int seg_multisplit(const void *keys, int key_kind, const void *vals, int32_t val_bytes, int64_t n,
                    const PartFn &fine, int32_t F1, int32_t nsrc, const int64_t *seg_start,
                    const int64_t *seg_rows, void *out_keys, void *out_vals, int64_t *fine_off, void *ws,
-                   int64_t ws_bytes, cudaStream_t st, bool stable = false);
+                   int64_t ws_bytes, cudaStream_t st, bool stable = false, int pack = 0);
+
+constexpr int PK_OUT = 1, PK_IN = 2;
+template <typename KeyT, typename ValT>
+struct __align__(2 * sizeof(KeyT)) PackedRow {
+    KeyT k;
+    ValT v;
+};
 
 DPK_HD uint64_t mix64(uint64_t x) {
     x ^= x >> 33; x *= 0xff51afd7ed558ccdull; x ^= x >> 33; x *= 0xc4ceb9fe1a85ec53ull;
diff --git a/dpark_b200/csrc/dpk_partition.cu b/dpark_b200/csrc/dpk_partition.cu
--- a/dpark_b200/csrc/dpk_partition.cu
+++ b/dpark_b200/csrc/dpk_partition.cu
@@ -33,6 +33,7 @@
     int64_t L;
     SegTab seg;
     const char *label_count = nullptr, *label_scatter = nullptr;
+    int pack = 0;
 };
 
 static Plan make_plan(int64_t n) {
@@ -95,7 +96,7 @@
     return base + inc - v;
 }
 
-template <typename KeyT, int PRE>
+template <typename KeyT, int PRE, bool PIN = false>
 __global__ void __launch_bounds__(PT_THREADS)
 k_part_count(const KeyT *__restrict__ keys, int64_t n, int64_t L, PartFn f,
              int32_t *__restrict__ tile_counts, int32_t T, SegTab seg, int count_mode) {
@@ -116,7 +117,7 @@
         for (; i0 + (int64_t)PT_THREADS * U <= end; i0 += (int64_t)PT_THREADS * U) {
             KeyT k[U];
 #pragma unroll
-            for (int u = 0; u < U; u++) k[u] = keys[i0 + (int64_t)u * PT_THREADS + threadIdx.x];
+            for (int u = 0; u < U; u++) k[u] = keys[(i0 + (int64_t)u * PT_THREADS + threadIdx.x) * (PIN ? 2 : 1)];
 #pragma unroll
             for (int u = 0; u < U; u++) atomicAdd(&wh[f.bucket(key_hash<KeyT, PRE>(k[u], f))], 1);
         }
@@ -128,7 +129,7 @@
         for (int u = 0; u < U; u++) {
             int64_t i = i0 + (int64_t)u * PT_THREADS + threadIdx.x;
             ok[u] = i < end;
-            k[u] = ok[u] ? keys[i] : KeyT(0);
+            k[u] = ok[u] ? keys[i * (PIN ? 2 : 1)] : KeyT(0);
         }
 #pragma unroll
         for (int u = 0; u < U; u++) {
@@ -219,13 +220,14 @@
     return s;
 }
 
-template <typename KeyT, typename ValT, int PRE, int ITEMS>
+template <typename KeyT, typename ValT, int PRE, int ITEMS, int PK = 0>
 __global__ void __launch_bounds__(PT_THREADS, ITEMS == 16 ? 2 : 4)
 k_part_scatter(const KeyT *__restrict__ keys, const ValT *__restrict__ vals, int64_t n, int64_t L,
                PartFn f, const int32_t *__restrict__ tile_off, int32_t T,
                const int64_t *__restrict__ bucket_base, KeyT *__restrict__ out_keys,
                ValT *__restrict__ out_vals, ScatterSmem lay, SegTab seg) {
     constexpr bool HAS_VAL = !std::is_same<ValT, NoVal>::value;
+    using Rec = PackedRow<KeyT, ValT>;
     constexpr int TILE = PT_THREADS * ITEMS;
     extern __shared__ __align__(16) unsigned char smem[];
     __shared__ int s_warp[PT_WARPS];
@@ -268,12 +270,25 @@
         KeyT k[ITEMS];
         ValT v[ITEMS];
         const int64_t wbase = tile + (int64_t)warp * (32 * ITEMS) + lane;
-#pragma unroll
-        for (int j = 0; j < ITEMS; j++) {
-            int64_t idx = wbase + j * 32;
-            k[j] = idx < end ? keys[idx] : KeyT(0);
-        }
-        if constexpr (HAS_VAL) {
+        if constexpr ((PK & PK_IN) != 0) {
+#pragma unroll
+            for (int j = 0; j < ITEMS; j++) {
+                int64_t idx = wbase + j * 32;
+                k[j] = KeyT(0);
+                if (idx < end) {
+                    const Rec r = reinterpret_cast<const Rec *>(keys)[idx];
+                    k[j] = r.k;
+                    v[j] = r.v;
+                }
+            }
+        } else {
+#pragma unroll
+            for (int j = 0; j < ITEMS; j++) {
+                int64_t idx = wbase + j * 32;
+                k[j] = idx < end ? keys[idx] : KeyT(0);
+            }
+        }
+        if constexpr (HAS_VAL && (PK & PK_IN) == 0) {
 #pragma unroll
             for (int j = 0; j < ITEMS; j++) {
                 int64_t idx = wbase + j * 32;
@@ -346,7 +361,9 @@
         for (int i = threadIdx.x; i < rows; i += PT_THREADS) {
             const int p = s_pid[i];
             const int64_t dst = s_gpos[p] + (int64_t)(i - s_tstart[p]);
-            if (seg.key_ptrs) {
+            if constexpr ((PK & PK_OUT) != 0) {
+                reinterpret_cast<Rec *>(out_keys)[dst] = Rec{s_key[i], s_val[i]};
+            } else if (seg.key_ptrs) {
                 reinterpret_cast<KeyT *>(s_kptr[p])[dst] = s_key[i];
                 if constexpr (HAS_VAL) reinterpret_cast<ValT *>(s_vptr[p])[dst] = s_val[i];
             } else {
@@ -409,7 +426,7 @@
     }
 }
 
-template <typename KeyT, typename ValT, int PRE, int NT, int FMODE, bool PTRS = false>
+template <typename KeyT, typename ValT, int PRE, int NT, int FMODE, bool PTRS = false, int PK = 0>
 __global__ void __launch_bounds__(NT, NT == 1024 ? 1 : 2)
 k_part_scatter_bulk(const KeyT *__restrict__ keys, const ValT *__restrict__ vals, int64_t n, int64_t L,
                     PartFn f, const int32_t *__restrict__ tile_off, int32_t T,
@@ -421,11 +438,17 @@
     constexpr int NW = NT / 32;
     constexpr int AK = 16 / (int)sizeof(KeyT);
     constexpr int AV = HAS_VAL ? 16 / (int)sizeof(typename std::conditional<HAS_VAL, ValT, int64_t>::type) : 1;
+    constexpr bool PIN = (PK & PK_IN) != 0, POUT = (PK & PK_OUT) != 0;
+    using Rec = PackedRow<KeyT, ValT>;
+    constexpr int AR = 16 / (int)sizeof(Rec);
+    static_assert(PK == 0 || (HAS_VAL && !PTRS && sizeof(KeyT) == sizeof(ValT)), "packed rows: same-width key and value, plain or segmented mode");
     extern __shared__ __align__(128) unsigned char smem_bulk[];
     unsigned char *smem = smem_bulk;
     __shared__ int s_warp[NW];
     KeyT *s_key = reinterpret_cast<KeyT *>(smem + lay.key_off);
     ValT *s_val = reinterpret_cast<ValT *>(smem + lay.val_off);
+    Rec *s_rec = reinterpret_cast<Rec *>(smem + lay.key_off);
+    Rec *out_rec = reinterpret_cast<Rec *>(out_keys);
     int64_t *s_gpos = reinterpret_cast<int64_t *>(smem + lay.gpos_off);
     uint32_t *s_cnt = reinterpret_cast<uint32_t *>(smem + lay.cnt_off);
     int32_t *s_sk = reinterpret_cast<int32_t *>(smem + lay.sk_off);
@@ -458,6 +481,20 @@
     KeyT k[ITEMS];
     ValT v[ITEMS];
     auto load_tile = [&](int64_t tile) {
+        if constexpr (PIN) {
+            const Rec *rp = reinterpret_cast<const Rec *>(keys) + tile + warp * (32 * ITEMS) + lane;
+            const int left = (int)min((int64_t)TILE, end - tile) - warp * (32 * ITEMS) - lane;
+#pragma unroll
+            for (int j = 0; j < ITEMS; j++) {
+                k[j] = KeyT(0);
+                if (j * 32 < left) {
+                    const Rec r = rp[j * 32];
+                    k[j] = r.k;
+                    v[j] = r.v;
+                }
+            }
+            return;
+        }
         const KeyT *kp = keys + tile + warp * (32 * ITEMS) + lane;
         if (tile + TILE <= end) {
 #pragma unroll
@@ -514,6 +551,13 @@
             int run = block_excl_scan<NW>(sum, s_warp, &tot);
             for (int i = b; i < min(b + E, P); i++) {
                 const int64_t g = s_gpos[i];
+                if constexpr (POUT) {
+                    const uint32_t gr = (uint32_t)(((uintptr_t)(out_rec + g)) / sizeof(Rec));
+                    const int baser = run + i * (AR - 1);
+                    s_sk[i] = baser + (int)((gr - (uint32_t)baser) & (uint32_t)(AR - 1));
+                    run += (int)cnt[i];
+                    continue;
+                }
                 const uint32_t gk = (uint32_t)(((uintptr_t)(out_keys + g)) / sizeof(KeyT));
                 const int basek = run + i * (AK - 1);
                 s_sk[i] = basek + (int)((gk - (uint32_t)basek) & (uint32_t)(AK - 1));
@@ -531,15 +575,30 @@
         for (int j = 0; j < ITEMS; j++) {
             const int p = (int)(pr[j] >> 16), r = (int)(pr[j] & 0xffffu);
             if (p != 0xffff) {
-                s_key[s_sk[p] + r] = k[j];
-                if constexpr (HAS_VAL) s_val[s_sv[p] + r] = v[j];
+                if constexpr (POUT) {
+                    s_rec[s_sk[p] + r] = Rec{k[j], v[j]};
+                } else {
+                    s_key[s_sk[p] + r] = k[j];
+                    if constexpr (HAS_VAL) s_val[s_sv[p] + r] = v[j];
+                }
             }
         }
         if (tile + TILE < end) load_tile(tile + TILE);
         asm volatile("fence.proxy.async.shared::cta;" ::: "memory");
         __syncthreads();
 
-        if constexpr (HAS_VAL) {
+        if constexpr (POUT) {
+            const uint32_t rec_addr = key_addr;
+            for (int p = threadIdx.x; p < P; p += NT) {
+                const int c = (int)cnt[p];
+                if (c) {
+                    const int64_t g = s_gpos[p];
+                    flush_run<Rec>(out_rec, g, s_rec, rec_addr, s_sk[p], c);
+                    s_gpos[p] = g + c;
+                    cnt[p] = 0;
+                }
+            }
+        } else if constexpr (HAS_VAL) {
             for (int q0 = 0; q0 < 2 * P; q0 += NT) {
                 const int q = q0 + (int)threadIdx.x;
                 const int p = q >> 1;
@@ -576,12 +635,14 @@
 static int launch_count(const void *keys, int64_t n, const Plan &pl, const PartFn &f,
                         int32_t *tile_counts, cudaStream_t st) {
     size_t sh = (size_t)f.nbuckets() * sizeof(int32_t) * (f.nbuckets() <= PT_COUNT_PRIV ? PT_WARPS : 1);
-    DPK_LAUNCH(pl.label_count ? pl.label_count : (pl.seg.cbeg ? "seg_count" : "part_count"), st, k_part_count<KeyT, PRE><<<pl.T, PT_THREADS, sh, st>>>((const KeyT *)keys, n, pl.L, f, tile_counts, pl.T, pl.seg, g_count_mode));
+    auto kern = (pl.pack & PK_IN) ? k_part_count<KeyT, PRE, true> : k_part_count<KeyT, PRE, false>;
+    DPK_LAUNCH(pl.label_count ? pl.label_count : (pl.seg.cbeg ? "seg_count" : "part_count"), st, kern<<<pl.T, PT_THREADS, sh, st>>>((const KeyT *)keys, n, pl.L, f, tile_counts, pl.T, pl.seg, g_count_mode));
     return DPK_OK;
 }
 
 static int dispatch_count(const void *keys, int key_kind, int64_t n, const Plan &pl, const PartFn &f,
                           int32_t *tile_counts, cudaStream_t st) {
+    if (key_kind >= 0) key_kind &= ~DPK_K_PACKED;
     if (key_kind >= DPK_K_UNORDERED) key_kind -= DPK_K_UNORDERED;
     switch (key_kind) {
     case -1: return launch_count<int64_t, true>(keys, n, pl, f, tile_counts, st);
@@ -604,6 +665,11 @@
     constexpr int vb = std::is_same<ValT, NoVal>::value ? 0 : (int)sizeof(ValT);
     ScatterSmem lay = scatter_smem((int)sizeof(KeyT), vb, f.nbuckets(), pl.seg.key_ptrs != nullptr, PT_THREADS * ITEMS);
     auto kern = k_part_scatter<KeyT, ValT, PRE, ITEMS>;
+    if constexpr (vb == (int)sizeof(KeyT) && ITEMS == 16) {
+        if (pl.pack == PK_OUT) kern = k_part_scatter<KeyT, ValT, PRE, ITEMS, PK_OUT>;
+        else if (pl.pack == PK_IN) kern = k_part_scatter<KeyT, ValT, PRE, ITEMS, PK_IN>;
+        else if (pl.pack == (PK_IN | PK_OUT)) kern = k_part_scatter<KeyT, ValT, PRE, ITEMS, PK_IN | PK_OUT>;
+    }
     if (lay.total > 227 * 1024)
         return fail(DPK_ERR_UNSUPPORTED, "%d buckets need %lld B of shared memory", f.nbuckets(), (long long)lay.total);
     DPK_CUDA_TRY(cudaFuncSetAttribute(kern, cudaFuncAttributeMaxDynamicSharedMemorySize, (int)lay.total));
@@ -619,6 +685,27 @@
                                const int32_t *tile_off, const int64_t *bucket_base, void *out_keys,
                                void *out_vals, cudaStream_t st) {
     constexpr int vb = std::is_same<ValT, NoVal>::value ? 0 : (int)sizeof(ValT);
+    if constexpr (vb == (int)sizeof(KeyT)) {
+        if (pl.pack) {
+            const int fmode = f.mode == 5 ? 2 : ((f.mode == 0 || f.mode == 1) ? 1 : 0);
+            BulkSmem lay = bulk_smem(2 * (int)sizeof(KeyT), 0, f.nbuckets(), 8192);
+            auto kern = fmode == 2 ? k_part_scatter_bulk<KeyT, ValT, PRE, 1024, 2, false, PK_OUT>
+                      : fmode == 1 ? k_part_scatter_bulk<KeyT, ValT, PRE, 1024, 1, false, PK_OUT>
+                                   : k_part_scatter_bulk<KeyT, ValT, PRE, 1024, 0, false, PK_OUT>;
+            if (pl.pack & PK_IN) {
+                if (fmode != 2) return fail(DPK_ERR_UNSUPPORTED, "packed input needs the second-level split");
+                kern = (pl.pack & PK_OUT) ? k_part_scatter_bulk<KeyT, ValT, PRE, 1024, 2, false, PK_IN | PK_OUT>
+                                          : k_part_scatter_bulk<KeyT, ValT, PRE, 1024, 2, false, PK_IN>;
+                if (!(pl.pack & PK_OUT)) lay = bulk_smem((int)sizeof(KeyT), vb, f.nbuckets(), 8192);
+            }
+            DPK_CUDA_TRY(cudaFuncSetAttribute(kern, cudaFuncAttributeMaxDynamicSharedMemorySize, (int)lay.total));
+            DPK_LAUNCH(pl.label_scatter ? pl.label_scatter : (pl.seg.cbeg ? "seg_scatter" : "part_scatter"), st,
+                       kern<<<pl.T, 1024, (size_t)lay.total, st>>>((const KeyT *)keys, (const ValT *)vals, n, pl.L, f,
+                                                                  tile_off, pl.T, bucket_base, (KeyT *)out_keys,
+                                                                  (ValT *)out_vals, lay, pl.seg));
+            return DPK_OK;
+        }
+    }
     int nt = g_scatter_threads;
     if (nt == 512 && pl.seg.cbeg != nullptr && g_scatter_seg_wide) nt = 1024;
     if (nt == 512 && g_scatter_seg_wide && sizeof(KeyT) <= 4 && (vb == 0 || vb <= 4)) nt = 1024;
@@ -658,11 +745,14 @@
     Plan pl = pl_in;
     if (pl.seg.unordered == 2) {
         constexpr int vb = std::is_same<ValT, NoVal>::value ? 0 : (int)sizeof(ValT);
-        if (bulk_smem((int)sizeof(KeyT), vb, f.nbuckets(), PT_TILE, pl.seg.key_ptrs != nullptr).total <= 110 * 1024)
+        const bool fits = (pl.pack & PK_OUT) ? bulk_smem(2 * (int)sizeof(KeyT), 0, f.nbuckets(), 8192).total <= 220 * 1024
+                        : pl.pack ? bulk_smem((int)sizeof(KeyT), vb, f.nbuckets(), 8192).total <= 220 * 1024
+                                  : bulk_smem((int)sizeof(KeyT), vb, f.nbuckets(), PT_TILE, pl.seg.key_ptrs != nullptr).total <= 110 * 1024;
+        if (fits)
             return launch_scatter_bulk<KeyT, ValT, PRE>(keys, vals, n, pl, f, tile_off, bucket_base, out_keys, out_vals, st);
         pl.seg.unordered = (f.nbuckets() % 2 == 0) ? 1 : 0;
     }
-    if (g_scatter_items == 8)
+    if (g_scatter_items == 8 && !pl.pack)
         return launch_scatter_items<KeyT, ValT, PRE, 8>(keys, vals, n, pl, f, tile_off, bucket_base, out_keys, out_vals, st);
     return launch_scatter_items<KeyT, ValT, PRE, 16>(keys, vals, n, pl, f, tile_off, bucket_base, out_keys, out_vals, st);
 }
@@ -671,7 +761,14 @@
 static int dispatch_val(const void *keys, const void *vals, int32_t val_bytes, int64_t n, const Plan &pl,
                         const PartFn &f, const int32_t *tile_off, const int64_t *bucket_base,
                         void *out_keys, void *out_vals, cudaStream_t st) {
-    if (vals == nullptr || val_bytes == 0)
+    if (pl.pack) {
+        if (vals == nullptr && !(pl.pack & PK_IN)) return fail(DPK_ERR_INVALID, "packed rows need a value column");
+        if (val_bytes != (int)sizeof(KeyT)) return fail(DPK_ERR_UNSUPPORTED, "packed rows need values as wide as the keys (%d B), got %d B", (int)sizeof(KeyT), val_bytes);
+        if (pl.seg.key_ptrs) return fail(DPK_ERR_UNSUPPORTED, "packed rows are not written through pointer tables");
+        if (((pl.pack & PK_OUT) && ((uintptr_t)out_keys % (2 * sizeof(KeyT)))) || ((pl.pack & PK_IN) && ((uintptr_t)keys % (2 * sizeof(KeyT)))))
+            return fail(DPK_ERR_INVALID, "packed rows must be aligned to their %d-byte size", 2 * (int)sizeof(KeyT));
+    }
+    if ((vals == nullptr && !(pl.pack & PK_IN)) || val_bytes == 0)
         return launch_scatter<KeyT, NoVal, PRE>(keys, nullptr, n, pl, f, tile_off, bucket_base, out_keys, nullptr, st);
     if (val_bytes == 8)
         return launch_scatter<KeyT, int64_t, PRE>(keys, vals, n, pl, f, tile_off, bucket_base, out_keys, out_vals, st);
@@ -684,6 +781,10 @@
                             const Plan &pl_in, const PartFn &f, const int32_t *tile_off,
                             const int64_t *bucket_base, void *out_keys, void *out_vals, cudaStream_t st) {
     Plan pl = pl_in;
+    if (key_kind >= 0 && (key_kind & DPK_K_PACKED)) {
+        key_kind &= ~DPK_K_PACKED;
+        pl.pack |= PK_OUT;
+    }
     if (key_kind >= DPK_K_UNORDERED) {
         key_kind -= DPK_K_UNORDERED;
         if (f.nbuckets() % 2 == 0) pl.seg.unordered = 1;
@@ -805,7 +906,7 @@
 int seg_multisplit(const void *keys, int key_kind, const void *vals, int32_t val_bytes, int64_t n,
                    const PartFn &fine, int32_t F1, int32_t nsrc, const int64_t *seg_start,
                    const int64_t *seg_rows, void *out_keys, void *out_vals, int64_t *fine_off, void *ws,
-                   int64_t ws_bytes, cudaStream_t st, bool stable) {
+                   int64_t ws_bytes, cudaStream_t st, bool stable, int pack) {
     const int32_t S2 = fine.nbuckets();
     if (ws_bytes < seg_multisplit_ws_bytes(n, F1, S2, nsrc)) return fail(DPK_ERR_WORKSPACE, "segmented multisplit workspace too small");
     const int64_t maxc = seg_max_chunks(n, F1, nsrc);
@@ -822,6 +923,7 @@
     pl.T = (int32_t)maxc;
     pl.L = 0;
     pl.seg = SegTab{cbeg, cend, ctotal, chunk_counts, chunk_off, nullptr, nullptr, (S2 % 2 == 0) ? 1 : (g_scatter_bulk ? 2 : 0)};
+    pl.pack = pack;
     if (stable) {
         pl.seg.unordered = 0;
         pl.label_count = "radix_count";
diff --git a/dpark_b200/peer.py b/dpark_b200/peer.py
--- a/dpark_b200/peer.py
+++ b/dpark_b200/peer.py
@@ -115,6 +115,7 @@
 
 def exchange_push(px, mo, need_host_count=False):
     G, rank, dev = px.world, px.rank, px.device
+    mo = mo.unpacked()
     P, sb = mo.P, mo.sub_bits
     F = P << sb
     if mo.keys.dtype != px.keys.dtype or (mo.vals is not None and mo.vals.dtype != px.vals.dtype):
diff --git a/dpark_b200/shuffle.py b/dpark_b200/shuffle.py
--- a/dpark_b200/shuffle.py
+++ b/dpark_b200/shuffle.py
@@ -55,10 +55,16 @@
 
 
 class MapOutput(object):
-    __slots__ = ("keys", "vals", "offsets", "P", "sub_bits")
-
-    def __init__(self, keys, vals, offsets, P, sub_bits):
+    __slots__ = ("keys", "vals", "offsets", "P", "sub_bits", "rows")
+
+    def __init__(self, keys, vals, offsets, P, sub_bits, rows=None):
         self.keys, self.vals, self.offsets, self.P, self.sub_bits = keys, vals, offsets, P, sub_bits
+        self.rows = rows
+
+    def unpacked(self):
+        if self.rows is None:
+            return self
+        return MapOutput(self.keys.contiguous(), self.vals.contiguous(), self.offsets, self.P, self.sub_bits)
 
 
 def _as_one(chunks):
@@ -79,12 +85,17 @@
 def map_side(key_chunks, val_chunks, P, thresholds=None, prehashed=False, sub_bits=0, row_hash=None,
              unordered=False):
     F = P << sub_bits
+    packed = (unordered and val_chunks[0] is not None and _world() == 1
+              and nv.packable(key_chunks[0], val_chunks[0], prehashed))
     if len(key_chunks) > 1:
         whole_k, whole_v = _as_one(key_chunks), (_as_one(val_chunks) if val_chunks[0] is not None else None)
         if whole_k is not None and (val_chunks[0] is None or whole_v is not None) and whole_k.numel() < (1 << 31):
             key_chunks, val_chunks = [whole_k], [whole_v]
     if len(key_chunks) == 1:
-        k, v, off = nv.partition(key_chunks[0], val_chunks[0], P, thresholds, prehashed, sub_bits, row_hash, unordered)
+        k, v, off = nv.partition(key_chunks[0], val_chunks[0], P, thresholds, prehashed, sub_bits, row_hash, unordered,
+                                 packed)
+        if packed:
+            return MapOutput(*nv.packed_views(k, key_chunks[0].dtype, val_chunks[0].dtype), off, P, sub_bits, rows=k)
         return MapOutput(k, v, off, P, sub_bits)
     dev = key_chunks[0].device
     counts, wss = [], []
@@ -98,20 +109,28 @@
     torch.cumsum(tot, 0, out=offsets[1:])
     base = offsets[:-1].unsqueeze(0) + (torch.cumsum(cm, 0) - cm)
     n = sum(int(k.numel()) for k in key_chunks)
-    out_k = torch.empty(n, dtype=key_chunks[0].dtype, device=dev)
     has_v = val_chunks[0] is not None
-    out_v = torch.empty(n, dtype=val_chunks[0].dtype, device=dev) if has_v else None
+    if packed:
+        rows = nv.packed_rows(n, key_chunks[0].dtype, dev)
+        out_k, out_v = rows, None
+    else:
+        out_k = torch.empty(n, dtype=key_chunks[0].dtype, device=dev)
+        out_v = torch.empty(n, dtype=val_chunks[0].dtype, device=dev) if has_v else None
     for m, (k, v) in enumerate(zip(key_chunks, val_chunks)):
         nv.partition_scatter(k, v, P, base[m].contiguous(), out_k, out_v, wss[m], thresholds, prehashed, sub_bits,
                              row_hash, unordered)
+    if packed:
+        return MapOutput(*nv.packed_views(rows, key_chunks[0].dtype, val_chunks[0].dtype), offsets, P, sub_bits,
+                         rows=rows)
     return MapOutput(out_k, out_v, offsets, P, sub_bits)
 
 
 class Received(object):
-    __slots__ = ("keys", "vals", "seg", "part_first", "nparts", "sub_bits", "bound")
-
-    def __init__(self, keys, vals, seg, part_first, nparts, sub_bits, bound=False):
+    __slots__ = ("keys", "vals", "seg", "part_first", "nparts", "sub_bits", "bound", "rows")
+
+    def __init__(self, keys, vals, seg, part_first, nparts, sub_bits, bound=False, rows=None):
         self.keys, self.vals, self.seg = keys, vals, seg
+        self.rows = rows
         self.part_first, self.nparts, self.sub_bits = part_first, nparts, sub_bits
         self.bound = bound
 
@@ -134,7 +153,8 @@
     P, sb = mo.P, mo.sub_bits
     if G == 1:
         seg = (mo.offsets[1:] - mo.offsets[:-1]).unsqueeze(0)
-        return Received(mo.keys, mo.vals, seg, 0, P, sb)
+        return Received(mo.keys, mo.vals, seg, 0, P, sb, rows=mo.rows)
+    mo = mo.unpacked()
     rank = dist.get_rank(group)
     F = P << sb
     blocks = [b << sb for b in owner_blocks(P, G)]
@@ -163,7 +183,7 @@
         z = torch.zeros(1, dtype=torch.int64, device=dev)
         return rx.keys[:0], (rx.vals[:0] if rx.vals is not None else None), z, z[:0]
     return nv.combine(rx.keys, rx.vals, op, P, rx.seg.contiguous(), rx.part_first, rx.nparts, thresholds,
-                      rx.sub_bits)
+                      rx.sub_bits, rows=rx.rows)
 
 
 RADIX_BITS = 8
@@ -421,7 +441,7 @@
 def combine_map_output(mo, op, thresholds=None):
     P, sb = mo.P, mo.sub_bits
     seg = (mo.offsets[1:] - mo.offsets[:-1]).unsqueeze(0)
-    ok, ov, po, cnt = reduce_side(Received(mo.keys, mo.vals, seg, 0, P, sb), op, P, thresholds)
+    ok, ov, po, cnt = reduce_side(Received(mo.keys, mo.vals, seg, 0, P, sb, rows=mo.rows), op, P, thresholds)
     po_h, cnt_h = po.cpu().tolist(), cnt.cpu().tolist()
     check_counts(cnt_h)
     keys = torch.cat([ok[a:a + c] for a, c in zip(po_h, cnt_h)])
diff --git a/dpark_b200/strings.py b/dpark_b200/strings.py
--- a/dpark_b200/strings.py
+++ b/dpark_b200/strings.py
@@ -44,7 +44,7 @@
     mo = shuffle.map_side([rep], [d_vals], P, thresholds, False, sb, row_hash=h, unordered=True)
     rx = shuffle.exchange(mo)
     ok, ov, off, cnt = nv.combine(rx.keys, rx.vals, op, P, rx.seg.contiguous(), rx.part_first, rx.nparts,
-                                  thresholds, sb, row_hash=h)
+                                  thresholds, sb, row_hash=h, rows=rx.rows)
     off_h, cnt_h = off.cpu().tolist(), cnt.cpu().tolist()
     shuffle.check_counts(cnt_h)
     ok_h, ov_h = ok.cpu().numpy(), ov.cpu().numpy()
diff --git a/dpark_b200/textingest.py b/dpark_b200/textingest.py
--- a/dpark_b200/textingest.py
+++ b/dpark_b200/textingest.py
@@ -136,7 +136,7 @@
         mo = shuffle.map_side([rep], [ones], P, thresholds, False, sb, row_hash=h, unordered=True)
         rx = shuffle.exchange(mo)
         ok, ov, poff, cnt = nv.combine(rx.keys, rx.vals, op, P, rx.seg.contiguous(), rx.part_first, rx.nparts,
-                                       thresholds, sb, row_hash=h)
+                                       thresholds, sb, row_hash=h, rows=rx.rows)
     off_h, cnt_h = poff.cpu().tolist(), cnt.cpu().tolist()
     shuffle.check_counts(cnt_h)
     sel = torch.cat([ok[off_h[p]:off_h[p] + cnt_h[p]] for p in range(P)]) if P else ok[:0]
diff --git a/include/dpark_b200.h b/include/dpark_b200.h
--- a/include/dpark_b200.h
+++ b/include/dpark_b200.h
@@ -23,6 +23,7 @@
 enum { DPK_K_I64 = 0, DPK_K_I32 = 1, DPK_K_F64 = 2, DPK_K_U64 = 3, DPK_K_F32 = 4,
        DPK_K_ROWID = 5  };
 #define DPK_K_UNORDERED 0x100
+#define DPK_K_PACKED 0x200
 enum { DPK_V_I64 = 0, DPK_V_F64 = 1, DPK_V_I32 = 2, DPK_V_F32 = 3 };
 enum { DPK_OP_SUM = 0, DPK_OP_MIN = 1, DPK_OP_MAX = 2, DPK_OP_PROD = 3,
        DPK_OP_AND = 4, DPK_OP_OR = 5, DPK_OP_XOR = 6 };
```

Result: faster. 17.81 billion (median of 6 runs) (+15.5%).
